# bxh1/VIDO-SLAM

Hardware: AMD Instinct MI355X
Metric: frames/sec end-to-end (flow+depth+track+local-BA) at 640x480; BA iters/sec (higher is better)
Workload: dtype f32

## Files before the change

include/vido_c.h:

```cpp
#ifndef VIDO_C_H
#define VIDO_C_H
#include <stdint.h>
#include <stddef.h>
#ifdef __cplusplus
extern "C" {
#endif

#define VIDO_OK              0
#define VIDO_E_INVALID      -1
#define VIDO_E_NO_DEVICE    -2
#define VIDO_E_HIP          -3
#define VIDO_E_CAPACITY     -4
#define VIDO_E_NOMEM        -5

#define VIDO_MAX_LEVELS 16

typedef struct vido_ctx vido_ctx;

typedef struct vido_keypoint { float x, y, size, angle, response; int32_t octave; } vido_keypoint;

typedef struct vido_config {
    int32_t device;
    int32_t width, height;
    int32_t max_batch;
// ... 44 lines not shown
} vido_track_params;

typedef struct vido_frame_lists {
    int32_t max_stat, max_obj;
    int32_t* n_stat; int32_t* stat_idx; float* stat_corr; float* stat_flow; float* stat_depth;
    int32_t* n_obj; float* obj_keys; float* obj_corr; float* obj_depth; int32_t* obj_label; float* obj_flow;
} vido_frame_lists;

int vido_track_slots(vido_ctx* ctx);
int vido_debug_first_op(vido_ctx* ctx, int rounds);
int vido_frame_upload(vido_ctx* ctx, int slot0, int n_frames, float* depth, const float* flow, const int32_t* mask,
                      int on_device, const vido_track_params* p);
int vido_frame_features(vido_ctx* ctx, int slot0, int n_frames, const vido_keypoint* kps, const int32_t* n_kps, int max_kp,
                        const vido_track_params* p, vido_frame_lists* out);
typedef struct vido_frontend_view {
    int32_t n_frames, kp_pitch, stat_pitch, obj_pitch;
    const vido_keypoint* kps; const uint8_t* desc; const int32_t* frame_beg;
    const int32_t* n_stat; const int32_t* stat_idx; const float* stat_corr; const float* stat_flow; const float* stat_depth;
    const int32_t* n_obj; const float* obj_keys; const float* obj_corr; const float* obj_depth; const int32_t* obj_label; const float* obj_flow;
} vido_frontend_view;
int vido_frontend_batch(vido_ctx* ctx, const uint8_t* imgs, int imgs_on_device, int n_frames, size_t frame_stride, int stride, int width, int height,
                        float* depth, const float* flow, const int32_t* mask, int maps_on_device, int slot0, const vido_track_params* p,
                        vido_frontend_view* view);
int vido_gather_static_depth(vido_ctx* ctx, int slot, const float* keys_xy, int n, float* depth_out);
int vido_gather_object_depth_label(vido_ctx* ctx, int slot, const float* keys_xy, int n, float th_depth_obj,
                                   float* depth_out, int32_t* label_out);
int vido_update_mask(vido_ctx* ctx, int slot_last, int slot_cur, const int32_t* last_label, const float* last_corr_xy, int n,
                     int32_t* recovered_out, int cap, int32_t* n_recovered);
int vido_read_maps(vido_ctx* ctx, int slot, float* depth_out, float* flow_out, int32_t* mask_out);
int vido_mask_propagate(vido_ctx* ctx, const int32_t* mask_prev, const float* flow, const float* depth_prev , int H, int W, int32_t* out,
                        int32_t* stats_out );
int vido_frame_propagate_mask(vido_ctx* ctx, int slot_last, int slot_cur, int32_t* stats_out );
int vido_mask_associate(vido_ctx* ctx, const int32_t* prev , const int32_t* cur, int H, int W, const int64_t* classes , int n, int hold,
                        int32_t* state , int32_t* out, int32_t* lut_out , int32_t* stats_out );
int vido_mask_components(vido_ctx* ctx, const int32_t* mask, int H, int W, int connectivity, int min_area, int id_base, int cap, int32_t* out,
                         int64_t* classes_out , int32_t* area_out , int32_t* stats_out );
int vido_frame_split_mask(vido_ctx* ctx, int slot, int connectivity, int min_area, int id_base, int cap, int32_t* stats_out );
int vido_gather_point_samples(vido_ctx* ctx, int slot, const float* xy, int n, int32_t* mask_out, float* depth_out, float* flow_out);
int vido_unproject_world(vido_ctx* ctx, const float* keys_xy, const float* z, int n, const vido_track_params* p,
                         const float* Tcw, float* xyz_out);
int vido_scene_flow(vido_ctx* ctx, const float* xyz_last, const float* xyz_cur, const int32_t* sem_last, const int32_t* sem_cur,
                    int n, float* flow3d_out, int32_t* obj_label_inout);

typedef struct vido_pose_problem {
    int32_t mode, n;
    const double* Xw;
    const double* obs;
    const double* flow0;
    const double* depth;
    double Twl[16];
    double P[12];
    double fx, fy, cx, cy;
    double T_init[16];
    double info_edge, info_prior, huber_delta;
    int32_t use_huber, rounds, drop_kernel_after_round;
    int32_t iters[4];
    float chi2_th[4];
} vido_pose_problem;

typedef struct vido_pose_result { double T[16]; int32_t n_inliers, lm_iterations; double chi2_final; } vido_pose_result;

int vido_pose_optimize(vido_ctx* ctx, const vido_pose_problem* prob, vido_pose_result* result, uint8_t* outlier_out, double* flow_out);
int vido_pose_optimize_batch(vido_ctx* ctx, const vido_pose_problem* probs, int n_prob, vido_pose_result* results,
                             uint8_t* const* outlier_out, double* const* flow_out);

typedef struct vido_ba_problem {
    int32_t n_cam, n_pt, n_obs, n_odo, prior_cam, use_huber, max_iters, pad;
    double* cam_T; double* pt_xyz;
    const int32_t* obs_cam; const int32_t* obs_pt; const double* obs_meas;
    const int32_t* odo_i; const int32_t* odo_j; const double* odo_T;
    double prior_T[12];
    double info_obs, info_odo, info_prior, huber_obs, huber_odo, gain_threshold;
    int32_t pt_lo, pt_hi;
    int32_t rank, world;
} vido_ba_problem;

typedef struct vido_ba_result { int32_t iterations, lm_trials; double chi2_initial, chi2_final, lambda_final;
                                double ms_setup;
                                double ms_solve_loop;
                                double ms_linearize_kernel;
                                double ms_schur_kernel;
} vido_ba_result;

typedef int (*vido_allreduce_fn)(void* user, void* dev_ptr, size_t count, int op);

int vido_ba_optimize(vido_ctx* ctx, vido_ba_problem* prob, vido_ba_result* result, vido_allreduce_fn allreduce, void* user);
int vido_rccl_unique_id(uint8_t id_out[128]);
int vido_rccl_init(vido_ctx* ctx, const uint8_t id[128], int rank, int world);
int vido_rccl_allreduce(void* user_ctx, void* dev_ptr, size_t count, int op);
int vido_rccl_destroy(vido_ctx* ctx);

typedef struct vido_ba_dynamic {
    int32_t n_H, n_dyn, n_tern, n_smooth;
    double* H_T;
    double* dyn_xyz;
    const int32_t* dyn_cam; const double* dyn_meas;
    const int32_t* tern_prev; const int32_t* tern_cur; const int32_t* tern_H;
    const int32_t* sm_i; const int32_t* sm_j;
    double info_dyn, info_tern, info_smooth, huber_dyn, huber_tern, huber_smooth;
} vido_ba_dynamic;
int vido_ba_optimize_dynamic(vido_ctx* ctx, vido_ba_problem* prob, vido_ba_dynamic* dyn, vido_ba_result* result,
                             vido_allreduce_fn allreduce, void* user);

int vido_correlation(vido_ctx* ctx, const float* first, const float* second, int B, int C, int H, int W, int stride,
                     float* out, int on_device);
int vido_det_order(vido_ctx* ctx, const float* scores, const long long* labels, const int* n_det, float confidence, int cap, long long* order, long long* labels_out, long long* n_live);
int vido_det_order_n(vido_ctx* ctx, const float* scores, const long long* labels, const int* n_det, float confidence, int cap, long long* order, long long* labels_out, long long* n_live,
                     int32_t* n_live32);
int vido_roi_levels(vido_ctx* ctx, const float* boxes, int n, float k_min, float k_max, int* out);
int vido_mask_logit_select(vido_ctx* ctx, const float* feat, const float* w, const float* b, const long long* labels, float* out, int n, int c, int hw, int classes);
int vido_mask_logit_select_n(vido_ctx* ctx, const float* feat, const float* w, const float* b, const long long* labels, float* out, int n, int c, int hw, int classes, const int32_t* n_live);
int vido_bias_act(vido_ctx* ctx, float* x, const float* bias, int N, int C, int H, int W, float slope);
int vido_bias_unary(vido_ctx* ctx, float* x, const float* bias, int N, int C, int H, int W, int kind);
int vido_upcat_reflect(vido_ctx* ctx, const float* x, const float* skip, int C1, int C2, int h, int w, float* out);
int vido_minmax_norm_u16(vido_ctx* ctx, const float* d, const float* mm, int64_t n, int32_t* out);
int vido_bias_res_act(vido_ctx* ctx, float* x, const float* bias, const float* res, int N, int C, int H, int W, float slope);
int vido_area_feed(vido_ctx* ctx, const uint8_t* bgr, int H, int W, float* out, int OH, int OW, float div);
int vido_backwarp(vido_ctx* ctx, const float* x, const float* flow, int B, int C, int H, int W, float* out);
int vido_deconv4s2_depthwise(vido_ctx* ctx, const float* x, const float* weight, int B, int C, int H, int W, float input_slope, float* out);

int vido_conv1x1_supported(int cin, int cout, int hw);
int vido_conv1x1_layout(int cin, int cout, int hw);
int vido_conv1x1_set_arith(int arith);
int vido_conv1x1_range_flag(vido_ctx* ctx, int reset);
int vido_range_latch(vido_ctx* ctx, unsigned* dst);
int vido_conv1x1_bias_act(vido_ctx* ctx, const float* x, const float* w_packed, const float* bias, const float* residual, float* y, int cin, int cout, int hw, float slope);
int vido_deconv2x2_supported(int n, int cin, int cout, int h, int w);
int vido_deconv2x2_bias_act(vido_ctx* ctx, const float* x, const float* w_packed, const float* bias, float* y, int n, int cin, int cout, int h, int w, float slope);
int vido_deconv2x2_bias_act_n(vido_ctx* ctx, const float* x, const float* w_packed, const float* bias, float* y, int n, int cin, int cout, int h, int w, float slope, const int32_t* n_live);
int vido_conv1x1_bias_up2_act(vido_ctx* ctx, const float* x, const float* w_packed, const float* bias, const float* residual_half, float* y, int cin, int cout, int h, int w, float slope);

int vido_conv_kxk_c2(vido_ctx* ctx, const float* x, const float* w, const float* bias, const float* residual, float* y, int cin, int k, int h, int w_);
int vido_conv1x1_skinny(vido_ctx* ctx, const float* x, const float* w_packed, const float* bias, const float* residual, float* y, int cin, int cout, long long hw, float slope);
int vido_stem7x7s2_pool(vido_ctx* ctx, const float* x, const float* w_packed, const float* bias, float* y, int h, int w);

int vido_conv_direct_supported(int cin, int cout, int h, int w, int kh, int kw, int sh, int sw, int ph, int pw);
long long vido_conv_direct_packed_floats(int cin, int cout, int kh, int kw);
int vido_conv_direct_pack(const float* w, int cin, int cout, int kh, int kw, float* w_packed);
int vido_conv_direct_bias_act(vido_ctx* ctx, const float* x, const float* w_packed, const float* bias, float* y, int n, int cin, int cout, int h, int w,
                              int kh, int kw, int sh, int sw, int ph, int pw, float slope);

int vido_wino3x3_supported(int cin, int cout, int h, int w);
int vido_wino3x3_fills_chip(int n, int cout, int h, int w, int min_wgs);
long long vido_wino3x3_packed_floats(int cin, int cout);
int vido_wino3x3_pack(const float* w, int cin, int cout, float* u_packed);
int vido_wino3x3_bias_act(vido_ctx* ctx, const float* x, const float* u_packed, const float* bias, float* y, int n, int cin, int cout, int h, int w, float slope);
int vido_wino3x3_form(int n, int cin, int cout, int h, int w);
int vido_fc_h_splitk(int rows, int k, int outs);
int vido_fc_h(vido_ctx* ctx, const float* x, const void* w_packed, const float* bias, float* part, float* y, int rows, int k, int outs, float slope);
int vido_conv3x3_h_supported(int n, int cin, int cout, int h, int w);
int vido_conv3x3_h_workgroups(int n, int cout, int h, int w);
int vido_conv3x3_h_bias_act(vido_ctx* ctx, const float* x, const void* w_packed, const float* bias, float* y, int n, int cin, int cout, int h, int w, float slope);
int vido_conv3x3_h_bias_act_n(vido_ctx* ctx, const float* x, const void* w_packed, const float* bias, float* y, int n, int cin, int cout, int h, int w, float slope, const int32_t* n_live);
long long vido_wino3x3_packed_floats_form(int cin, int cout, int form);
int vido_wino3x3_pack_form(const float* w, int cin, int cout, int form, float* u_packed);
int vido_wino3x3_bias_act_form(vido_ctx* ctx, const float* x, const float* u_packed, const float* bias, float* y, int n, int cin, int cout, int h, int w, float slope, int form);
int vido_gconv3x3_supported(int H, int W, int cpg_in, int cpg_out);
int64_t vido_gconv3x3_packed_size(int groups, int cpg_in, int cpg_out);
int vido_gconv3x3_bias_act(vido_ctx* ctx, const float* x, const float* in_bias, const float* w_packed, const float* bias, float* y, int groups, int cpg_in, int cpg_out, int H, int W, float slope);
int vido_gconv3x3_s2_supported(int H, int W, int cpg_in, int cpg_out);
int vido_gconv3x3_s2_bias_act(vido_ctx* ctx, const float* x, const float* w_packed, const float* bias, float* y, int groups, int cpg_in, int cpg_out, int H, int W, float slope);
int vido_lfn_reg_front(vido_ctx* ctx, const float* im1, const float* im2, const float* flow, const float* mean, float scale, int B, int C, int H, int W, float* out, int out_channels);
int vido_lfn_reg_tail(vido_ctx* ctx, const float* dist, const float* flow, const float* wx, const float* bx, const float* wy, const float* by, int B, int K, int H, int W, float* out);
int vido_roi_align(vido_ctx* ctx, const float* feat, int B, int C, int H, int W, const float* rois, int n_rois,
                   float spatial_scale, int pooled_h, int pooled_w, int sampling_ratio, float* out, int on_device);
int vido_nms(vido_ctx* ctx, const float* boxes_xyxy, const float* scores, int n, float thresh, int32_t* keep_out,
             int32_t* n_keep, int on_device);
int vido_nms_grouped(vido_ctx* ctx, const float* boxes_xyxy, const float* scores, const int32_t* groups, int n, float thresh,
                     int32_t* keep_out, int32_t* n_keep, int on_device);
int vido_nms_segments(vido_ctx* ctx, const float* boxes_xyxy, const int32_t* groups, const int32_t* seg_off, const int32_t* seg_n, int n_seg, int max_n, int total,
                      float thresh, int32_t* keep_out, int32_t* n_keep);
int vido_roi_align_fpn(vido_ctx* ctx, const float* const feat[4], const int H[4], const int W[4], const float scale[4], int C, const float* boxes, const int32_t* level,
                       int n, int pooled_h, int pooled_w, int sampling_ratio, float* out);
int vido_nchw_to_nhwc(vido_ctx* ctx, const float* src, int B, int C, int H, int W, float* dst);
int vido_roi_align_fpn_nhwc(vido_ctx* ctx, const float* const feat[4], const int H[4], const int W[4], const float scale[4], int C, const float* boxes, const int32_t* level,
                            int n, int pooled_h, int pooled_w, int sampling_ratio, float* out);
int vido_roi_align_fpn_nhwc_n(vido_ctx* ctx, const float* const feat[4], const int H[4], const int W[4], const float scale[4], int C, const float* boxes, const int32_t* level,
                              int n, int pooled_h, int pooled_w, int sampling_ratio, float* out, const int32_t* n_live);
int vido_bawin_create(vido_ctx* ctx, int cap_frames, int cap_features);
int vido_bawin_push_frame(vido_ctx* ctx, int frame, int n, const double* meas, const float* xyz, const int32_t* asso);
int vido_bawin_set_labels(vido_ctx* ctx, int n, const int32_t* quads);
int vido_bawin_solve(vido_ctx* ctx, int start, int N, vido_ba_problem* prob, vido_ba_result* res, int32_t* n_obs_out, int32_t* n_pt_out);
int vido_bawin_read_points(vido_ctx* ctx, int frame, int n, float* xyz_out);
int vido_rpn_select(vido_ctx* ctx, int n_levels, const float* const* logits, const float* const* deltas, const int* h, const int* w, const int* stride, const float* cell_anchors,
                    int A, int K, int img_w, int img_h, float* boxes_out, float* scores_out, int32_t* n_out);
int vido_rpn_merge(vido_ctx* ctx, const float* boxes, const float* scores, const int32_t* keep, const int32_t* cnt, int n_levels, int K, int post_nms_top_n, int n_final,
                   float* out_boxes, float* out_scores, int32_t* n_valid);
int vido_det_class_sort(vido_ctx* ctx, const float* prob, const float* deltas, const float* proposals, const float* objectness, int N, int nc, float thresh, const float weights[4],
                        int img_w, int img_h, float* seg_boxes, int32_t* order, int32_t* seg_n);
int vido_det_select(vido_ctx* ctx, const float* prob, const float* seg_boxes, const int32_t* order, const int32_t* keep, const int32_t* cnt, int N, int nc, int detections_per_img, int cap,
                    int32_t* scratch, float* out_boxes, float* out_scores, int64_t* out_labels, int32_t* n_det);
int vido_mask_label_image(vido_ctx* ctx, const float* masks, const float* boxes, const int64_t* labels, int n, int M, int padding, float thresh, int H, int W, uint8_t* out);
int vido_mask_instance_image(vido_ctx* ctx, const float* masks, const float* boxes, const int64_t* labels, int n, int M, int padding, float thresh, int H, int W,
                             const int32_t* id_base_dev, uint8_t* out, int32_t* area_out);
int vido_box_decode(vido_ctx* ctx, const float* deltas, const float* boxes, int n, int k, const float weights[4],
                    float* out, int on_device);

int vido_pnp_ransac(vido_ctx* ctx, const float* pts3d, const float* pts2d, int n, double fx, double fy, double cx, double cy,
                    int max_iters, double reproj_err, double confidence, uint64_t seed, double T_out[16], uint8_t* inlier_mask,
                    int32_t* n_inliers);

int vido_pnp_ransac_batch(vido_ctx* ctx, int n_prob, const float* const* pts3d, const float* const* pts2d, const int32_t* n, double fx, double fy, double cx, double cy,
                          int max_iters, double reproj_err, double confidence, const uint64_t* seeds, double* T_out, uint8_t* const* inlier_mask, int32_t* n_inliers);

typedef struct vido_host_maps { const int32_t* mask; const float* depth; const float* flow; int32_t width, height; } vido_host_maps;
float vido_depth_noise(float z, unsigned seed);
int vido_undistort_points(const float* xy, int n, const float K[4], const float dist[5], float* xy_out);
int vido_renew_static(const vido_host_maps* maps, const float* stat_xy, int n_stat, const int32_t* TM_sta, int n_tm, const float* sample_xy, int n_sample,
                      int max_num, int32_t* src_out, int32_t* inlier_out, float* flow_out, int cap, int32_t* n_out);
int vido_renew_objects(const vido_host_maps* maps, const float* obj_xy, const int32_t* obj_label, int n_obj_pts,
                       int n_objects, const int32_t* inl_off, const int32_t* inl_ids, const uint8_t* obj_stat, const int32_t* sem_position, const int32_t* mod_label,
                       const float* tmp_xy, const float* tmp_depth, const int32_t* tmp_sem, const float* tmp_flow, const float* tmp_corr, int n_tmp, int max_num_obj,
                       float* keys_out, float* depth_out, int32_t* sem_out, float* flow_out, float* corr_out, int32_t* inlier_out, int32_t* label_out, int cap, int32_t* n_out);
typedef struct vido_point_samples { const int32_t* mask; const float* depth; const float* flow; } vido_point_samples;
int vido_renew_static_sampled(int width, int height, const float* stat_xy, int n_stat, const vido_point_samples* stat_samples, const int32_t* TM_sta, int n_tm,
                              const float* sample_xy, int n_sample, const vido_point_samples* sample_samples, int max_num,
                              int32_t* src_out, int32_t* inlier_out, float* flow_out, int cap, int32_t* n_out);
int vido_renew_objects_sampled(int width, int height, const float* obj_xy, const int32_t* obj_label, int n_obj_pts, const vido_point_samples* obj_samples,
                               int n_objects, const int32_t* inl_off, const int32_t* inl_ids, const uint8_t* obj_stat, const int32_t* sem_position, const int32_t* mod_label,
                               const float* tmp_xy, const float* tmp_depth, const int32_t* tmp_sem, const float* tmp_flow, const float* tmp_corr, int n_tmp, int max_num_obj,
                               float* keys_out, float* depth_out, int32_t* sem_out, float* flow_out, float* corr_out, int32_t* inlier_out, int32_t* label_out, int cap, int32_t* n_out);
int vido_dyn_obj_tracking(const int32_t* sem_label, int32_t* obj_label, const float* obj_xy, const float* obj_depth, const float* flow3d, const int32_t* last_sem_label, int n,
                          const int32_t* last_sem_position, const uint8_t* last_obj_stat, const int32_t* last_mod_label, int n_last, int rows, int cols,
                          float sf_mg_thres, float sf_ds_thres, float th_depth_obj, int f_id, int32_t* max_id,
                          int32_t* obj_off, int32_t* obj_ids, int32_t* mod_label_out, int32_t* sem_position_out, int max_objects, int32_t* n_objects);

int vido_tracklets_incremental(int n_rows, const int32_t* row_off, const int32_t* row_n, const int32_t* TM, const int32_t* labels, int n_feat0,
                               int32_t* trk_off, int32_t* pairs, int32_t* obj_id, int32_t* owner_trk, int32_t* owner_pos, int cap_trk, int cap_pairs, int32_t* n_trk);

typedef struct vido_system vido_system;
typedef struct vido_system_stats {
    int32_t frame_id, n_keypoints, n_static, n_static_inliers, n_objects, n_object_points, ba_window;
    int32_t mask_propagated;
    float ms_total;
    float ms_update_mask, ms_frame;
    float ms_cam_pose, ms_obj_tracking, ms_obj_motion, ms_renew;
    float ms_local_ba;
    float ms_wait_inputs;
    float ms_orb, ms_lists;
} vido_system_stats;
int         vido_system_create(const char* settings_yaml, vido_system** out);
void        vido_system_destroy(vido_system* sys);
const char* vido_system_last_error(const vido_system* sys);
int         vido_system_track_rgbd(vido_system* sys, const uint8_t* im, int channels, int width, int height, float* depth, const float* flow,
                                   const int32_t* mask, double timestamp, int n_image, float Tcw_out[16]);
int         vido_system_set_zero_copy_maps(vido_system* sys, int zero_copy);
int         vido_system_prefetch_image_device(vido_system* sys, const void* im_dev, int channels, int width, int height, void* image_ready_event);
int         vido_system_track_rgbd_device(vido_system* sys, const void* im_dev, int channels, int width, int height, float* depth_dev, const float* flow_dev,
                                          const int32_t* mask_dev, void* ready_event, double timestamp, int n_image, float Tcw_out[16]);
int         vido_system_get_stats(const vido_system* sys, vido_system_stats* out);
int         vido_system_get_verify_stats(const vido_system* sys, int* n_checked, int* n_rejected);
int         vido_system_mask_split_stats(const vido_system* sys, int32_t out[4]);
int         vido_system_get_verify_points(const vido_system* sys, float* xy, float* prev_xy, int32_t* xyl, int32_t* dist, uint8_t* rejected, uint8_t* seed_desc, int cap, int* n_out);
int         vido_system_save_results(vido_system* sys, const char* prefix);
vido_ctx*   vido_system_context(vido_system* sys);
int         vido_system_set_depth_noise_seed(vido_system* sys, unsigned seed);

#ifdef __cplusplus
}
#endif
#endif
```

vido-slam_amd/csrc/conv3x3h.hip:

```cpp
#include "common.hpp"
#include <type_traits>

namespace {
typedef float f32x16 __attribute__((ext_vector_type(16)));
typedef float f32x2 __attribute__((ext_vector_type(2)));
typedef _Float16 f16x8 __attribute__((ext_vector_type(8)));
typedef _Float16 f16x2 __attribute__((ext_vector_type(2)));
typedef unsigned u32x4 __attribute__((ext_vector_type(4)));

#define C3_OOB 0x40000000u
#define C3_WSLOT 24576
#define C3_RBW 3
#define C3_WPIX(BR) (((BR) + 2) * 18)
#define C3_XP(BR) ((16 * C3_WPIX(BR) + 511) / 512)
#define C3_RAW(BR) (C3_XP(BR) * 8 * 256)
#define C3_PLANE(BR) (C3_WPIX(BR) * 32)
#define C3_PBUF(BR) (2 * C3_PLANE(BR))
#define C3_LDS(BR) (C3_RBW * C3_WSLOT + C3_RAW(BR) + 2 * C3_PBUF(BR))

struct C3Args { const float* x; const void* wp; const float* bias; float* y; int N, Cin, Cout, H, W, nby, nbx, mt, total, nchunk; float slope; unsigned wbytes; unsigned* range_flag; const int* n_live; };

template <int RPW, int CG>
__global__ __launch_bounds__(512) void k_conv3x3_h(C3Args A)
{
    constexpr int BR = 16 / CG, MT = 32 * RPW * CG, WPIX = C3_WPIX(BR), XP = C3_XP(BR), RAWB = C3_RAW(BR), PLANE = C3_PLANE(BR), PBUF = C3_PBUF(BR), CK = (WPIX * 8 + 511) / 512, NMM = 9 * RPW, NRD = 2 * RPW + 2;
    extern __shared__ __attribute__((aligned(16))) char c3_lds[];
    char* L = c3_lds;
    const int tid = threadIdx.x, lane = tid & 63, w = __builtin_amdgcn_readfirstlane(tid >> 6);
    int total = A.total, per = gridDim.x >> 3;
    if (A.n_live) { const int nl = min(max(*A.n_live, 0), A.N); total = nl * A.nby * A.nbx * A.mt; per = (total + 7) >> 3; }
    const int q8 = blockIdx.x >> 3, item = (blockIdx.x & 7) * per + q8;
    if (q8 >= per || item >= total) return;
    const int nt = item / A.mt, mtile = item - nt * A.mt, m0 = mtile * MT;
    const int bpi = A.nby * A.nbx, n = nt / bpi, brem = nt - n * bpi, by = brem / A.nbx, bx = brem - by * A.nbx, Y0 = by * BR, X0 = bx * 16;
    const int rp = CG == 1 ? w : (w & 3), rb0 = CG == 1 ? 0 : RPW * (w >> 2);
    const int hw = A.H * A.W, nsteps = A.nchunk * 3;

    const __amdgpu_buffer_rsrc_t wr = __builtin_amdgcn_make_buffer_rsrc((void*)A.wp, 0, A.wbytes, 0x00020000);
    const unsigned avo = 16u * (unsigned)lane;
    unsigned abase[3], avq[3];
#pragma unroll
    for (int q = 0; q < 3; q++) { const int i = w + 8 * q, rb = i / 6, rem = i - 6 * rb; abase[q] = 1024u * (unsigned)(((m0 >> 5) + rb) * A.nchunk * 18 + rem); avq[q] = rb < RPW * CG ? avo : 0x80000000u; }
    unsigned xvo[11];
#pragma unroll
    for (int j = 0; j < XP; j++) {
        const int e = 64 * (8 * j + w) + lane, ch = e / WPIX, rem = e - ch * WPIX, row = rem / 18, col = rem - row * 18, gy = Y0 - 1 + row, gx = X0 - 1 + col;
        xvo[j] = (e < 16 * WPIX && gy >= 0 && gy < A.H && gx >= 0 && gx < A.W) ? 4u * (unsigned)(ch * hw + gy * A.W + gx) : C3_OOB;
    }
    const unsigned ximg = 4u * (unsigned)n * (unsigned)A.Cin * (unsigned)hw, ximg_end = ximg + 4u * (unsigned)A.Cin * (unsigned)hw, xchunk = 64u * (unsigned)hw;
    char* const RAW = L + C3_RBW * C3_WSLOT;
    char* const PL = RAW + RAWB;
    auto issue_w = [&](int s, int slot) {
        char* S = L + slot * C3_WSLOT + w * 1024;
        const unsigned so = 6144u * (unsigned)s;
#pragma unroll
        for (int q = 0; q < 3; q++) __builtin_amdgcn_raw_ptr_buffer_load_lds(wr, (__attribute__((address_space(3))) void*)(S + q * 8192), 16, avq[q], abase[q] + so, 0, 0);
    };
    auto issue_x = [&](int c) {
        const unsigned so = ximg + xchunk * (unsigned)c;
        const __amdgpu_buffer_rsrc_t xc = __builtin_amdgcn_make_buffer_rsrc((void*)((const char*)A.x + so), 0, ximg_end - so, 0x00020000);
#pragma unroll
        for (int j = 0; j < XP; j++) __builtin_amdgcn_raw_ptr_buffer_load_lds(xc, (__attribute__((address_space(3))) void*)(RAW + (8 * j + w) * 256), 4, xvo[j], 0, 0, 0);
    };
    float xmax = 0.f;
    const f32x2 k2048 = {2048.f, 2048.f};
    auto convert = [&](int buf) {
        const float* R = (const float*)RAW;
        unsigned* P = (unsigned*)(PL + buf * PBUF);
#pragma unroll
        for (int k = 0; k < CK; k++) {
            const int idx = tid + 512 * k;
            if (k < CK - 1 || idx < WPIX * 8) {
                const int q = idx / WPIX, pix = idx - q * WPIX;
                const f32x2 v = {R[(2 * q) * WPIX + pix], R[(2 * q + 1) * WPIX + pix]};
                const f16x2 h = __builtin_convertvector(v, f16x2);
                f32x2 vs, r;
                asm("v_pk_mul_f32 %0, %1, %2" : "=v"(vs) : "v"(v), "v"(k2048));
                asm("v_fma_mix_f32 %0, %1, %2, %3 op_sel_hi:[1,0,0]" : "=v"(r.x) : "v"(h), "s"(-2048.f), "v"(vs.x));
                asm("v_fma_mix_f32 %0, %1, %2, %3 op_sel:[1,0,0] op_sel_hi:[1,0,0]" : "=v"(r.y) : "v"(h), "s"(-2048.f), "v"(vs.y));
                const f16x2 l = __builtin_convertvector(r, f16x2);
                P[pix * 8 + q] = __builtin_bit_cast(unsigned, h); P[PLANE / 4 + pix * 8 + q] = __builtin_bit_cast(unsigned, l);
                xmax = __builtin_elementwise_maximum(__builtin_elementwise_maximum(xmax, __builtin_fabsf(v.x)), __builtin_fabsf(v.y));
            }
        }
    };

    f32x16 acc[RPW], acl[RPW];
#pragma unroll
    for (int rb = 0; rb < RPW; rb++)
#pragma unroll
        for (int r = 0; r < 16; r++) { acc[rb][r] = 0.f; acl[rb][r] = 0.f; }
    typedef const __attribute__((address_space(3))) char* lds_c;
    const unsigned a_lane = 16u * (unsigned)lane;
    const unsigned b_lane = (unsigned)(C3_RBW * C3_WSLOT + RAWB) + 32u * (unsigned)((2 * rp + ((lane & 31) >> 4)) * 18 + (lane & 15)) + 16u * (unsigned)(lane >> 5);

    issue_x(0); issue_w(0, 0); issue_w(min(1, nsteps - 1), 1);
    asm volatile("s_waitcnt vmcnt(6) lgkmcnt(0)\n\ts_barrier" ::: "memory");
    convert(0);
    int slot = 0;
    u32x4 a[2][RPW][2], b[2][2];
    auto step = [&](auto dy_c, auto nbuf_c, int pbuf, auto&& copies) {
        constexpr int dy = decltype(dy_c)::value, NBUF = decltype(nbuf_c)::value;
        lds_c Ab = (lds_c)(L + slot * C3_WSLOT) + a_lane;
        lds_c Bb = (lds_c)L + b_lane + pbuf * PBUF + dy * (18 * 32);
        auto ld = [&](int dx, int set) {
#pragma unroll
            for (int rb = 0; rb < RPW; rb++)
#pragma unroll
                for (int pl = 0; pl < 2; pl++) a[set][rb][pl] = *(const __attribute__((address_space(3))) u32x4*)(Ab + (((rb0 + rb) * 3 + dx) * 2 + pl) * 1024);
#pragma unroll
            for (int pl = 0; pl < 2; pl++) b[set][pl] = *(const __attribute__((address_space(3))) u32x4*)(Bb + dx * 32 + pl * PLANE);
        };
        __builtin_amdgcn_sched_barrier(0);
        ld(0, 0);
        copies();
#pragma unroll
        for (int dx = 0; dx < 3; dx++) {
            if (dx < 2) ld(dx + 1, (dx + 1) & 1);
#pragma unroll
            for (int term = 0; term < 3; term++) {
                constexpr int PA[3] = {0, 1, 0}, PB[3] = {1, 0, 0};
#pragma unroll
                for (int rb = 0; rb < RPW; rb++) {
                    f32x16& d = term == 2 ? acc[rb] : acl[rb];
                    d = __builtin_amdgcn_mfma_f32_32x32x16_f16(__builtin_bit_cast(f16x8, a[dx & 1][rb][PA[term]]), __builtin_bit_cast(f16x8, b[dx & 1][PB[term]]), d, 0, 0, 0);
                }
            }
        }
        __builtin_amdgcn_sched_group_barrier(0x100, NRD, 0);
#pragma unroll
        for (int i = 0; i < NMM; i++) {
            __builtin_amdgcn_sched_group_barrier(0x008, 1, 0);
            if (i < 2 * NRD) __builtin_amdgcn_sched_group_barrier(0x100, 1, 0);
            if (i >= 1 && i < 1 + NBUF) __builtin_amdgcn_sched_group_barrier(0x020, 1, 0);
        }
        __builtin_amdgcn_sched_barrier(0);
    };
    for (int c = 0; c < A.nchunk; c++) {
        const int pbuf = c & 1, cn = min(c + 1, A.nchunk - 1);
        asm volatile("s_waitcnt vmcnt(3) lgkmcnt(0)\n\ts_barrier" ::: "memory");
        step(std::integral_constant<int, 0>{}, std::integral_constant<int, 3 + XP>{}, pbuf, [&] { const int sf = slot == 0 ? C3_RBW - 1 : slot - 1; issue_w(min(3 * c + 2, nsteps - 1), sf); issue_x(cn); });
        slot = slot + 1 == C3_RBW ? 0 : slot + 1;
        asm volatile("s_waitcnt vmcnt(%0) lgkmcnt(0)\n\ts_barrier" :: "n"(3 + XP) : "memory");
        step(std::integral_constant<int, 1>{}, std::integral_constant<int, 3>{}, pbuf, [&] { const int sf = slot == 0 ? C3_RBW - 1 : slot - 1; issue_w(min(3 * c + 3, nsteps - 1), sf); });
        slot = slot + 1 == C3_RBW ? 0 : slot + 1;
        asm volatile("s_waitcnt vmcnt(3) lgkmcnt(0)\n\ts_barrier" ::: "memory");
        step(std::integral_constant<int, 2>{}, std::integral_constant<int, 3>{}, pbuf, [&] { const int sf = slot == 0 ? C3_RBW - 1 : slot - 1; issue_w(min(3 * c + 4, nsteps - 1), sf); });
        convert(pbuf ^ 1);
        slot = slot + 1 == C3_RBW ? 0 : slot + 1;
    }
    asm volatile("s_waitcnt vmcnt(0) lgkmcnt(0)" ::: "memory");
#pragma unroll
    for (int rb = 0; rb < RPW; rb++) acc[rb] += acl[rb] * 0x1p-11f;
    if (!(xmax < 65504.f) && A.range_flag) atomicOr(A.range_flag, 1u);

    const float* wsc = (const float*)((const char*)A.wp + (size_t)A.nchunk * 16 * 18 * A.Cout * 2);
    const int p = lane & 31, Y = Y0 + 2 * rp + (p >> 4), X = X0 + (p & 15);
    const bool inside = Y < A.H && X < A.W;
    float* yb = A.y + (size_t)n * A.Cout * hw + (size_t)Y * A.W + X;
#pragma unroll
    for (int rb = 0; rb < RPW; rb++) {
        float bv[16], sv[16];
#pragma unroll
        for (int r = 0; r < 16; r++) { const int co = m0 + 32 * (rb0 + rb) + 8 * (r >> 2) + 4 * (lane >> 5) + (r & 3); bv[r] = A.bias ? A.bias[co] : 0.f; sv[r] = wsc[co]; }
        if (inside) {
#pragma unroll
            for (int r = 0; r < 16; r++) {
                const int co = m0 + 32 * (rb0 + rb) + 8 * (r >> 2) + 4 * (lane >> 5) + (r & 3);
                const float v = acc[rb][r] * sv[r] + bv[r];
                yb[(size_t)co * hw] = fmaxf(v, v * A.slope);
            }
        }
    }
}
}

extern "C" {

int vido_conv3x3_h_supported(int n, int cin, int cout, int h, int w)
{
    const long long cp = (cin + 15) / 16 * 16;
    return n >= 1 && cin >= 1 && (cout == 32 || cout == 64 || (cout >= 128 && cout % 128 == 0)) && h >= 1 && w >= 1 && 4ll * n * cin * h * w < (1ll << 30) && 4ll * n * cout * h * w < (1ll << 30)
           && 36ll * cp * cout < (1ll << 31);
}

#define C3_MIN16 190
static int c3_block_rows(int n, int cout, int h, int w)
{
    static const int force = [] { const char* e = getenv("VIDO_CONV3X3_H_ROWS"); return e ? atoi(e) : 0; }();
    if (cout == 32) return 16;
    if (force == 16 || force == 8) return force;
    const int mt = cout >= 128 ? cout / 128 : 1;
    return n * ((h + 15) / 16) * ((w + 15) / 16) * mt >= C3_MIN16 ? 16 : 8;
}
int vido_conv3x3_h_workgroups(int n, int cout, int h, int w) { const int br = c3_block_rows(n, cout, h, w); return n * ((h + br - 1) / br) * ((w + 15) / 16) * (cout >= 128 ? cout / 128 : 1); }

int vido_conv3x3_h_bias_act(vido_ctx* ctx, const float* x, const void* w_packed, const float* bias, float* y, int n, int cin, int cout, int h, int w, float slope)
{
    return vido_conv3x3_h_bias_act_n(ctx, x, w_packed, bias, y, n, cin, cout, h, w, slope, nullptr);
}

int vido_conv3x3_h_bias_act_n(vido_ctx* ctx, const float* x, const void* w_packed, const float* bias, float* y, int n, int cin, int cout, int h, int w, float slope, const int32_t* n_live)
{
    if (!ctx) return VIDO_E_INVALID;
    if (!x || !w_packed || !y || x == y || !vido_conv3x3_h_supported(n, cin, cout, h, w) || slope < 0.f || slope > 1.f || (((uintptr_t)x | (uintptr_t)y | (uintptr_t)n_live) & 3) || ((uintptr_t)w_packed & 15))
        return vido_set_error(ctx, VIDO_E_INVALID, "conv3x3_h: no kernel for %d x %d -> %d channels at %d x %d (or a pointer is misaligned, or slope outside [0, 1])", n, cin, cout, h, w);
    HIP_TRY(ctx, hipSetDevice(ctx->device));
    hipStream_t st = ctx->has_ext_stream ? ctx->ext_stream : ctx->stream;
    const int br = c3_block_rows(n, cout, h, w);
    const int nby = (h + br - 1) / br, nbx = (w + 15) / 16, mt = cout >= 128 ? cout / 128 : 1, total = n * nby * nbx * mt;
    const int nchunk = (cin + 15) / 16;
    C3Args A{x, w_packed, bias, y, n, cin, cout, h, w, nby, nbx, mt, total, nchunk, slope, (unsigned)(36ll * 16 * nchunk * cout), ctx->c1_range_flag, n_live};
    static bool attr[64] = {};
    if (!attr[ctx->device & 63]) {
#define C3_ATTR(RPW_, CG_) HIP_TRY(ctx, hipFuncSetAttribute((const void*)k_conv3x3_h<RPW_, CG_>, hipFuncAttributeMaxDynamicSharedMemorySize, (int)C3_LDS(16 / CG_)))
        C3_ATTR(4, 1); C3_ATTR(2, 2); C3_ATTR(2, 1); C3_ATTR(1, 2); C3_ATTR(1, 1);
#undef C3_ATTR
        attr[ctx->device & 63] = true;
    }
    const dim3 grid(8 * ((total + 7) / 8));
#define C3_LAUNCH(RPW_, CG_) hipLaunchKernelGGL((k_conv3x3_h<RPW_, CG_>), grid, dim3(512), C3_LDS(16 / CG_), st, A)
    if (cout >= 128) { if (br == 16) C3_LAUNCH(4, 1); else C3_LAUNCH(2, 2); }
    else if (cout == 64) { if (br == 16) C3_LAUNCH(2, 1); else C3_LAUNCH(1, 2); }
    else C3_LAUNCH(1, 1);
#undef C3_LAUNCH
    HIP_TRY(ctx, hipGetLastError());
    return VIDO_OK;
}

}
```

vido-slam_amd/csrc/nets.hip:

```cpp
#include "common.hpp"
#include <numeric>

#define CORR_CH 8
__global__ __launch_bounds__(256) void k_correlation(const float* __restrict__ f1, const float* __restrict__ f2, int C, int H, int W, int s,
                                                     int Ho, int Wo, float* __restrict__ out, int nsplit, int cper)
{
    __shared__ float t2[CORR_CH][22][23];
    const int tx = threadIdx.x & 15, ty = threadIdx.x >> 4, b = blockIdx.z / nsplit, split = blockIdx.z - b * nsplit;
    const int c_lo = split * cper, c_hi = min(C, c_lo + cper);
    const int x = blockIdx.x * 16 + tx, y = blockIdx.y * 16 + ty;
    const bool valid = x < Wo && y < Ho;
    float acc[49];
#pragma unroll
    for (int k = 0; k < 49; k++) acc[k] = 0.f;
    const size_t plane = (size_t)H * W;
    for (int c0 = c_lo; c0 < c_hi; c0 += CORR_CH) {
        const int nc = min(CORR_CH, c_hi - c0);
        for (int i = threadIdx.x; i < nc * 22 * 22; i += 256) {
            const int cc = i / (22 * 22), r = (i / 22) % 22, q = i % 22;
            const int yy = (blockIdx.y * 16 + r - 3), xx = (blockIdx.x * 16 + q - 3);
            float v = 0.f;
            if (yy >= 0 && yy < Ho && xx >= 0 && xx < Wo) v = f2[((size_t)b * C + c0 + cc) * plane + (size_t)(yy * s) * W + xx * s];
            t2[cc][r][q] = v;
        }
        float a[CORR_CH];
#pragma unroll
        for (int cc = 0; cc < CORR_CH; cc++) a[cc] = (valid && cc < nc) ? f1[((size_t)b * C + c0 + cc) * plane + (size_t)(y * s) * W + x * s] : 0.f;
        __syncthreads();
#pragma unroll
        for (int cc = 0; cc < CORR_CH; cc++) {
            if (cc < nc) {
#pragma unroll
                for (int p = 0; p < 7; p++)
#pragma unroll
                    for (int o = 0; o < 7; o++) acc[p * 7 + o] += a[cc] * t2[cc][ty + p][tx + o];
            }
        }
        __syncthreads();
    }
    if (valid) {
        float* o = out + (size_t)split * (gridDim.z / nsplit) * 49 * Ho * Wo;
#pragma unroll
        for (int k = 0; k < 49; k++) o[(((size_t)b * 49 + k) * Ho + y) * Wo + x] = nsplit == 1 ? acc[k] / (float)C : acc[k];
    }
}
__global__ __launch_bounds__(256) void k_correlation_reduce(const float* __restrict__ part, int nsplit, size_t n, float inv_c_dummy, int C, float* __restrict__ out)
{
    const size_t i = blockIdx.x * (size_t)blockDim.x + threadIdx.x;
    if (i >= n) return;
    float sum = 0.f;
    for (int k = 0; k < nsplit; k++) sum += part[(size_t)k * n + i];
    out[i] = sum / (float)C;
}

__global__ __launch_bounds__(1024) void k_det_order(const float* __restrict__ scores, const long long* __restrict__ labels, const int* __restrict__ n_det, float confidence, int cap,
                                                   long long* __restrict__ order, long long* __restrict__ labels_out, long long* __restrict__ n_live, int* __restrict__ n_live32)
{
    __shared__ float key[1024];
    __shared__ int cnt;
    const int i = threadIdx.x;
    if (i == 0) cnt = 0;
    const int nd = *n_det;
    bool live = false;
    if (i < cap) { live = scores[i] > confidence && i < nd; key[i] = live ? scores[i] : -1.0f; }
    __syncthreads();
    if (i < cap) {
        const float k = key[i]; int rank = 0;
        for (int j = 0; j < cap; j++) { const float kj = key[j]; rank += (kj > k) || (kj == k && j < i); }
        order[rank] = i; labels_out[rank] = live ? labels[i] : 0;
        if (live) atomicAdd(&cnt, 1);
    }
    __syncthreads();
    if (i == 0) { *n_live = cnt; if (n_live32) *n_live32 = cnt; }
}

__global__ void k_roi_levels(const float* __restrict__ boxes, int n, float k_min, float k_max, int* __restrict__ out)
{
    const int i = blockIdx.x * blockDim.x + threadIdx.x;
    if (i >= n) return;
    const float x1 = boxes[4 * i], y1 = boxes[4 * i + 1], x2 = boxes[4 * i + 2], y2 = boxes[4 * i + 3];
    const float area = __fmul_rn(__fadd_rn(__fsub_rn(x2, x1), 1.f), __fadd_rn(__fsub_rn(y2, y1), 1.f));
    const float t = __fadd_rn(__fdiv_rn(__fsqrt_rn(area), 224.f), 1e-6f);
    float l = floorf(__fadd_rn(4.f, log2f(t)));
    l = fminf(fmaxf(l, k_min), k_max);
    out[i] = (int)l - (int)k_min;
}

__global__ __launch_bounds__(256) void k_mask_logit_select(const float* __restrict__ feat, const float* __restrict__ w, const float* __restrict__ b, const long long* __restrict__ labels,
                                                           float* __restrict__ out, int c, int hw, int classes, const int* __restrict__ n_live)
{
    __shared__ float wl[1024];
    const int n = blockIdx.y, p = blockIdx.x * 256 + threadIdx.x;
    if (n_live && n >= *n_live) {
        if (p < hw) out[(size_t)n * hw + p] = 0.f;
        return;
    }
    long long lab = labels[n]; lab = lab < 0 ? 0 : (lab >= classes ? classes - 1 : lab);
    for (int i = threadIdx.x; i < c; i += 256) wl[i] = w[(size_t)lab * c + i];
    __syncthreads();
    if (p >= hw) return;
    const float* f = feat + (size_t)n * c * hw + p;
    double a0 = 0, a1 = 0, a2 = 0, a3 = 0;
    int i = 0;
    for (; i + 4 <= c; i += 4) { a0 += (double)wl[i] * f[(size_t)i * hw]; a1 += (double)wl[i + 1] * f[(size_t)(i + 1) * hw]; a2 += (double)wl[i + 2] * f[(size_t)(i + 2) * hw]; a3 += (double)wl[i + 3] * f[(size_t)(i + 3) * hw]; }
    for (; i < c; i++) a0 += (double)wl[i] * f[(size_t)i * hw];
    const float v = (float)((a0 + a1) + (a2 + a3) + (b ? (double)b[lab] : 0.0));
    out[(size_t)n * hw + p] = 1.f / (1.f + expf(-v));
}

__global__ __launch_bounds__(256) void k_bias_act(float* __restrict__ x, const float* __restrict__ bias, int C, size_t hw, size_t total, float slope)
{
    const size_t i = (blockIdx.x * (size_t)blockDim.x + threadIdx.x) * 4;
    if (i >= total) return;
    if ((hw & 3) == 0) {
        const float b = bias[(i / hw) % C];
        float4 v = *(float4*)(x + i);
        v.x += b; v.y += b; v.z += b; v.w += b;
        v.x = v.x > 0.f ? v.x : v.x * slope; v.y = v.y > 0.f ? v.y : v.y * slope; v.z = v.z > 0.f ? v.z : v.z * slope; v.w = v.w > 0.f ? v.w : v.w * slope;
        *(float4*)(x + i) = v;
    } else {
        for (size_t k = i; k < min(i + 4, total); k++) { float v = x[k] + bias[(k / hw) % C]; x[k] = v > 0.f ? v : v * slope; }
    }
}

template <int KIND>
__global__ __launch_bounds__(256) void k_bias_unary(float* __restrict__ x, const float* __restrict__ bias, int C, size_t hw, size_t total)
{
    const size_t i = blockIdx.x * (size_t)blockDim.x + threadIdx.x;
    if (i >= total) return;
    const float v = x[i] + bias[(i / hw) % C];
    x[i] = KIND == 1 ? (v > 0.f ? v : expf(v) - 1.f) : 1.f / (1.f + expf(-v));
}

__global__ __launch_bounds__(256) void k_upcat_reflect(const float* __restrict__ x, const float* __restrict__ skip, int C1, int C2, int h, int w, float* __restrict__ out)
{
    const int H2 = 2 * h, W2 = 2 * w, OW = W2 + 2, OH = H2 + 2;
    const size_t i = blockIdx.x * (size_t)blockDim.x + threadIdx.x, total = (size_t)(C1 + C2) * OH * OW;
    if (i >= total) return;
    const int X = (int)(i % OW), Y = (int)((i / OW) % OH), c = (int)(i / ((size_t)OW * OH));
    int yy = Y - 1, xx = X - 1;
    yy = yy < 0 ? -yy : (yy >= H2 ? 2 * H2 - 2 - yy : yy); xx = xx < 0 ? -xx : (xx >= W2 ? 2 * W2 - 2 - xx : xx);
    out[i] = c < C1 ? x[((size_t)c * h + (yy >> 1)) * w + (xx >> 1)] : skip[((size_t)(c - C1) * H2 + yy) * W2 + xx];
}

__global__ __launch_bounds__(256) void k_minmax_norm_u16(const float* __restrict__ d, const float* __restrict__ mm, size_t n, int* __restrict__ out)
{
    const size_t i = blockIdx.x * (size_t)blockDim.x + threadIdx.x;
    if (i >= n) return;
    const float lo = mm[0], hi = mm[1];
    float v = (d[i] - lo) / (hi - lo + 1e-12f) * 65536.0f;
    v = fminf(fmaxf(v, 0.f), 65535.f);
    out[i] = (int)v;
}

__global__ __launch_bounds__(256) void k_bias_res_act(float* __restrict__ x, const float* __restrict__ bias, const float* __restrict__ res, int C, size_t hw, size_t total, float slope)
{
    const size_t i = (blockIdx.x * (size_t)blockDim.x + threadIdx.x) * 4;
    if (i >= total) return;
    if ((hw & 3) == 0) {
        const float b = bias[(i / hw) % C];
        float4 v = *(float4*)(x + i); const float4 r = *(const float4*)(res + i);
        v.x += b + r.x; v.y += b + r.y; v.z += b + r.z; v.w += b + r.w;
        v.x = v.x > 0.f ? v.x : v.x * slope; v.y = v.y > 0.f ? v.y : v.y * slope; v.z = v.z > 0.f ? v.z : v.z * slope; v.w = v.w > 0.f ? v.w : v.w * slope;
        *(float4*)(x + i) = v;
    } else {
        for (size_t k = i; k < min(i + 4, total); k++) { float v = x[k] + bias[(k / hw) % C] + res[k]; x[k] = v > 0.f ? v : v * slope; }
    }
}

struct RoiLevels { const float* feat[4]; int H[4], W[4]; float scale[4]; };
template <int SR >
__global__ __launch_bounds__(256) void k_roi_align_nhwc(RoiLevels L, int C, const float* __restrict__ rois, int roi_stride ,
                                                        const int* __restrict__ level , int PH, int PW, int sampling, float* __restrict__ out, const int* __restrict__ n_live )
{
    extern __shared__ __attribute__((aligned(16))) float rl_tile[];
    if (n_live && (int)blockIdx.x >= *n_live) return;
    const int i = blockIdx.x, c0 = blockIdx.y * 64, lane = threadIdx.x & 63, wave = threadIdx.x >> 6;
    const int nbin = PH * PW, pitch = nbin | 1;
    const float* r = rois + (size_t)roi_stride * i;
    const int l = level ? level[i] : 0, bi = roi_stride == 5 ? (int)r[0] : 0;
    const float* box = r + (roi_stride == 5 ? 1 : 0);
    const float scale = L.scale[l]; const int H = L.H[l], W = L.W[l];
    const float sw = box[0] * scale, sh = box[1] * scale, ew = box[2] * scale, eh = box[3] * scale;
    const float rw = fmaxf(ew - sw, 1.f), rh = fmaxf(eh - sh, 1.f);
    const float bh = rh / (float)PH, bw = rw / (float)PW;
    const int gh = SR > 0 ? SR : (sampling > 0 ? sampling : (int)ceilf(rh / PH)), gw = SR > 0 ? SR : (sampling > 0 ? sampling : (int)ceilf(rw / PW));
    const float count = (float)(gh * gw);
    const int c = min(c0 + lane, C - 1);
    const float* d = L.feat[l] + (size_t)bi * H * W * C + c;
    auto taps = [&](float y, float x, int& o1, int& o2, int& o3, int& o4, float& w1, float& w2, float& w3, float& w4) {
        const bool out = y < -1.0 || y > H || x < -1.0 || x > W;
        if (y <= 0) y = 0;
        if (x <= 0) x = 0;
        int yl = out ? 0 : (int)y, xl = out ? 0 : (int)x, yh, xh;
        if (yl >= H - 1) { yh = yl = H - 1; y = (float)yl; } else yh = yl + 1;
        if (xl >= W - 1) { xh = xl = W - 1; x = (float)xl; } else xh = xl + 1;
        const float ly = y - yl, lx = x - xl, hy = 1.f - ly, hx = 1.f - lx;
        o1 = yl * W + xl; o2 = yl * W + xh; o3 = yh * W + xl; o4 = yh * W + xh;
        w1 = hy * hx; w2 = hy * lx; w3 = ly * hx; w4 = ly * lx;
        return out;
    };
    for (int bin = wave; bin < nbin; bin += 4) {
        const int ph = bin / PW, pw = bin - ph * PW;
        float acc = 0.f;
        if (SR == 2) {
            int o[4][4]; float w[4][4], v[4][4]; bool out[4];
#pragma unroll
            for (int s2 = 0; s2 < 4; s2++) {
                const int iy = s2 >> 1, ix = s2 & 1;
                const float y = sh + ph * bh + (float)(iy + .5f) * bh / (float)gh, x = sw + pw * bw + (float)(ix + .5f) * bw / (float)gw;
                out[s2] = taps(y, x, o[s2][0], o[s2][1], o[s2][2], o[s2][3], w[s2][0], w[s2][1], w[s2][2], w[s2][3]);
            }
#pragma unroll
            for (int s2 = 0; s2 < 4; s2++)
#pragma unroll
                for (int t = 0; t < 4; t++) v[s2][t] = d[(size_t)o[s2][t] * C];
#pragma unroll
            for (int s2 = 0; s2 < 4; s2++) acc += out[s2] ? 0.f : (w[s2][0] * v[s2][0] + w[s2][1] * v[s2][1] + w[s2][2] * v[s2][2] + w[s2][3] * v[s2][3]);
        } else {
            for (int iy = 0; iy < gh; iy++) {
                const float y = sh + ph * bh + (float)(iy + .5f) * bh / (float)gh;
                for (int ix = 0; ix < gw; ix++) {
                    const float x = sw + pw * bw + (float)(ix + .5f) * bw / (float)gw;
                    int o1, o2, o3, o4; float w1, w2, w3, w4;
                    if (taps(y, x, o1, o2, o3, o4, w1, w2, w3, w4)) { acc += 0.f; continue; }
                    const float v1 = d[(size_t)o1 * C], v2 = d[(size_t)o2 * C], v3 = d[(size_t)o3 * C], v4 = d[(size_t)o4 * C];
                    acc += (w1 * v1 + w2 * v2 + w3 * v3 + w4 * v4);
                }
            }
        }
        rl_tile[lane * pitch + bin] = acc / count;
    }
    __syncthreads();
    const int nc = min(64, C - c0), total = nc * nbin;
    float* o = out + ((size_t)i * C + c0) * nbin;
    for (int e = threadIdx.x; e < total; e += 256) { const int cc = e / nbin; o[e] = rl_tile[cc * pitch + (e - cc * nbin)]; }
}
__global__ __launch_bounds__(256) void k_nchw_to_nhwc(const float* __restrict__ src, int C, int HW, float* __restrict__ dst)
{
    __shared__ float t[64][65];
    const int p0 = blockIdx.x * 64, c0 = blockIdx.y * 64, b = blockIdx.z, lane = threadIdx.x & 63, q = threadIdx.x >> 6;
    const float* s = src + (size_t)b * C * HW; float* d = dst + (size_t)b * HW * C;
    for (int k = q; k < 64; k += 4) if (c0 + k < C && p0 + lane < HW) t[k][lane] = s[(size_t)(c0 + k) * HW + p0 + lane];
    __syncthreads();
    for (int k = q; k < 64; k += 4) if (p0 + k < HW && c0 + lane < C) d[(size_t)(p0 + k) * C + c0 + lane] = t[lane][k];
}

__device__ __forceinline__ void tile_of(int t, int nb, int& rb, int& cb)
{
    int r = (int)((2.0f * nb + 1.0f - sqrtf((2.0f * nb + 1.0f) * (2.0f * nb + 1.0f) - 8.0f * (float)t)) * 0.5f);
    r = max(0, min(r, nb - 1));
    while (r > 0 && r * nb - r * (r - 1) / 2 > t) r--;
    while ((r + 1) * nb - (r + 1) * r / 2 <= t) r++;
    rb = r; cb = r + (t - (r * nb - r * (r - 1) / 2));
}
__device__ __forceinline__ void nms_tile(const float* __restrict__ boxes, const int* __restrict__ group, int n, float thresh, unsigned long long* __restrict__ mask, int col_blocks, int rb, int cb, int lane)
{
    const int col = cb * 64 + lane; const bool cv = col < n;
    const float4 b = cv ? *(const float4*)(boxes + 4 * (size_t)col) : make_float4(0.f, 0.f, 0.f, 0.f);
    const float Sb = (b.z - b.x + 1) * (b.w - b.y + 1);
    const int gb = (group && cv) ? group[col] : 0;
    const int rows = min(n - rb * 64, 64);
    unsigned long long mine = 0;
    for (int i = 0; i < rows; i++) {
        const float* a = boxes + 4 * (size_t)(rb * 64 + i);
        const float a0 = a[0], a1 = a[1], a2 = a[2], a3 = a[3];
        const int ga = group ? group[rb * 64 + i] : 0;
        const float left = fmaxf(a0, b.x), right = fminf(a2, b.z), top = fmaxf(a1, b.y), bottom = fminf(a3, b.w);
        const float w = fmaxf(right - left + 1, 0.f), h = fmaxf(bottom - top + 1, 0.f), inter = w * h;
        const float Sa = (a2 - a0 + 1) * (a3 - a1 + 1);
        const bool hit = cv && ga == gb && inter / (Sa + Sb - inter) > thresh;
        unsigned long long word = __ballot(hit);
        if (rb == cb) word &= i >= 63 ? 0ull : ~((2ull << i) - 1ull);
        if (lane == i) mine = word;
    }
    if (lane < rows) mask[(size_t)(rb * 64 + lane) * col_blocks + cb] = mine;
}
__global__ __launch_bounds__(256) void k_nms_mask(const float* __restrict__ boxes, const int* __restrict__ group , int n, float thresh,
                                                 unsigned long long* __restrict__ mask, int col_blocks)
{
    const int t = __builtin_amdgcn_readfirstlane(blockIdx.x * 4 + (threadIdx.x >> 6)), nb = col_blocks;
    if (t >= nb * (nb + 1) / 2) return;
    int rb, cb; tile_of(t, nb, rb, cb);
    nms_tile(boxes, group, n, thresh, mask, col_blocks, rb, cb, threadIdx.x & 63);
}
__global__ __launch_bounds__(64) void k_nms_sweep(const unsigned long long* __restrict__ mask, int n, int col_blocks, int* __restrict__ keep, int* __restrict__ n_keep)
{
    const int lane = threadIdx.x;
    int cnt = 0;
    unsigned long long remv[16];
    const int wpl = (col_blocks + 63) / 64;
    for (int k = 0; k < 16; k++) remv[k] = 0;
    for (int i = 0; i < n; i++) {
        const int nblock = i >> 6, inblock = i & 63;
        const int owner = nblock & 63, slot = nblock >> 6;
        unsigned long long word = 0;
#pragma unroll
        for (int k = 0; k < 16; k++) if (k == slot) word = remv[k];
        word = __shfl(word, owner, 64);
        if (!(word & (1ULL << inblock))) {
            if (lane == 0) keep[cnt] = i;
            cnt++;
            const unsigned long long* p = mask + (size_t)i * col_blocks;
#pragma unroll
            for (int k = 0; k < 16; k++) if (k < wpl) { const int w = k * 64 + lane; if (w >= nblock && w < col_blocks) remv[k] |= p[w]; }
        }
    }
    if (lane == 0) *n_keep = cnt;
}

__global__ __launch_bounds__(64) void k_nms_sweep_seg(const unsigned long long* __restrict__ mask, const int* __restrict__ seg_off, const int* __restrict__ seg_n, int col_blocks,
                                                      int* __restrict__ keep, int* __restrict__ n_keep, int keep_stride)
{
    const int g = blockIdx.x, lane = threadIdx.x;
    const int n = seg_n[g];
    const unsigned long long* M = mask + (size_t)seg_off[g] * col_blocks;
    int* kp = keep + (size_t)g * keep_stride;
    const int cb = (n + 63) >> 6;
    unsigned long long remv[16];
#pragma unroll
    for (int k = 0; k < 16; k++) remv[k] = 0;
    int cnt = 0;
    for (int blk = 0; blk < cb; blk++) {
        const int owner = blk & 63, slot = blk >> 6, rows = min(n - blk * 64, 64);
        unsigned long long word = 0;
#pragma unroll
        for (int k = 0; k < 16; k++) if (k == slot) word = remv[k];
        word = __shfl(word, owner, 64);
        const unsigned long long diag = lane < rows ? M[(size_t)(blk * 64 + lane) * col_blocks + blk] : 0ull;
        const uint32_t dlo = (uint32_t)diag, dhi = (uint32_t)(diag >> 32);
        unsigned long long alive = ~word;
        if (rows < 64) alive &= (1ull << rows) - 1ull;
        unsigned long long keepmask = 0;
        while (alive) {
            const int j = __builtin_ctzll(alive);
            keepmask |= 1ull << j;
            const unsigned long long dj = (unsigned long long)(uint32_t)__builtin_amdgcn_readlane((int)dlo, j) | ((unsigned long long)(uint32_t)__builtin_amdgcn_readlane((int)dhi, j) << 32);
            alive &= ~dj; alive &= ~(1ull << j);
        }
        if ((keepmask >> lane) & 1ull) kp[cnt + __popcll(keepmask & ((1ull << lane) - 1ull))] = blk * 64 + lane;
        cnt += __popcll(keepmask);
        const bool mine = (keepmask >> lane) & 1ull;
        const unsigned long long* prow = M + (size_t)(blk * 64 + lane) * col_blocks;
        for (int w0 = blk + 1; w0 < cb; w0 += 4) {
            unsigned long long v[4];
#pragma unroll
            for (int u = 0; u < 4; u++) v[u] = (mine && w0 + u < cb) ? prow[w0 + u] : 0ull;
#pragma unroll
            for (int u = 0; u < 4; u++) {
                uint32_t lo = (uint32_t)v[u], hi = (uint32_t)(v[u] >> 32);
#pragma unroll
                for (int o = 32; o >= 1; o >>= 1) { lo |= (uint32_t)__shfl_xor((int)lo, o, 64); hi |= (uint32_t)__shfl_xor((int)hi, o, 64); }
                const int w = w0 + u;
                if (w < cb && lane == (w & 63)) {
                    const unsigned long long r = (unsigned long long)lo | ((unsigned long long)hi << 32);
#pragma unroll
                    for (int k = 0; k < 16; k++) if (k == (w >> 6)) remv[k] |= r;
                }
            }
        }
    }
    for (int i = cnt + lane; i < keep_stride; i += 64) kp[i] = -1;
    if (lane == 0) n_keep[g] = cnt;
}
__global__ __launch_bounds__(256) void k_nms_mask_seg(const float* __restrict__ boxes, const int* __restrict__ group, const int* __restrict__ seg_off, const int* __restrict__ seg_n,
                                                     float thresh, unsigned long long* __restrict__ mask, int col_blocks)
{
    const int g = blockIdx.y, n = seg_n[g], off = seg_off[g];
    const int nb = (n + 63) >> 6, t = __builtin_amdgcn_readfirstlane(blockIdx.x * 4 + (threadIdx.x >> 6));
    if (t >= nb * (nb + 1) / 2) return;
    int rb, cb; tile_of(t, nb, rb, cb);
    nms_tile(boxes + 4 * (size_t)off, group ? group + off : nullptr, n, thresh, mask + (size_t)off * col_blocks, col_blocks, rb, cb, threadIdx.x & 63);
}

struct PasteDet { int x0, y0, w, h, label; float rw, rh; };
__global__ __launch_bounds__(256) void k_paste_prepare(const float* __restrict__ boxes, const int64_t* __restrict__ labels, int n, int M, int padding, PasteDet* __restrict__ det)
{
    const int i = blockIdx.x * blockDim.x + threadIdx.x;
    if (i >= n) return;
    const float scale = (float)((double)(M + 2 * padding) / (double)M);
    const float* b = boxes + 4 * (size_t)i;
    const float wh = (b[2] - b[0]) * 0.5f * scale, hh = (b[3] - b[1]) * 0.5f * scale;
    const float xc = (b[2] + b[0]) * 0.5f, yc = (b[3] + b[1]) * 0.5f;
    const int x0 = (int)(xc - wh), y0 = (int)(yc - hh), x1 = (int)(xc + wh), y1 = (int)(yc + hh);
    PasteDet d; d.x0 = x0; d.y0 = y0; d.w = max(x1 - x0 + 1, 1); d.h = max(y1 - y0 + 1, 1); d.label = (int)labels[i];
    const int Mp = M + 2 * padding;
    d.rw = (float)Mp / (float)d.w; d.rh = (float)Mp / (float)d.h;
    det[i] = d;
}
__global__ __launch_bounds__(256) void k_paste_label(const float* __restrict__ masks , const PasteDet* __restrict__ det, int n, int M, int padding, float thresh,
                                                     int H, int W, uint8_t* __restrict__ out)
{
    __shared__ PasteDet sd[128];
    const int x = blockIdx.x * 32 + (threadIdx.x & 31), y = blockIdx.y * 8 + (threadIdx.x >> 5);
    const int Mp = M + 2 * padding;
    unsigned acc = 0;
    for (int d0 = 0; d0 < n; d0 += 128) {
        __syncthreads();
        if ((int)threadIdx.x < min(128, n - d0)) sd[threadIdx.x] = det[d0 + threadIdx.x];
        __syncthreads();
        if (x < W && y < H) {
            for (int k = 0; k < min(128, n - d0); k++) {
                const PasteDet d = sd[k];
                const int u = x - d.x0, v = y - d.y0;
                if (u < 0 || v < 0 || u >= d.w || v >= d.h) continue;
                float sy = d.rh * ((float)v + 0.5f) - 0.5f; if (sy < 0.f) sy = 0.f;
                float sx = d.rw * ((float)u + 0.5f) - 0.5f; if (sx < 0.f) sx = 0.f;
                const int iy = (int)sy, ix = (int)sx; const int iyp = iy < Mp - 1 ? 1 : 0, ixp = ix < Mp - 1 ? 1 : 0;
                const float ly = sy - (float)iy, lx = sx - (float)ix, hy = 1.f - ly, hx = 1.f - lx;
                const float* m = masks + (size_t)(d0 + k) * M * M;
                auto at = [&](int yy, int xx) -> float { yy -= padding; xx -= padding; return (yy < 0 || xx < 0 || yy >= M || xx >= M) ? 0.f : m[yy * M + xx]; };
                const float val = hy * (hx * at(iy, ix) + lx * at(iy, ix + ixp)) + ly * (hx * at(iy + iyp, ix) + lx * at(iy + iyp, ix + ixp));
                if (val > thresh) acc += (unsigned)d.label;
            }
        }
    }
    if (x < W && y < H) out[(size_t)y * W + x] = (uint8_t)acc;
}

__global__ void k_zero_i32(int32_t* __restrict__ p, int n)
{
    const int i = blockIdx.x * blockDim.x + threadIdx.x;
    if (i < n) p[i] = 0;
}
__global__ __launch_bounds__(256) void k_paste_instance(const float* __restrict__ masks , const PasteDet* __restrict__ det, int n, int M, int padding, float thresh,
                                                        int H, int W, const int32_t* __restrict__ id_base, uint8_t* __restrict__ out, int32_t* __restrict__ area)
{
    __shared__ PasteDet sd[128];
    __shared__ unsigned char slot[128];
    __shared__ int cnt[256], nlive[2];
    const int t = threadIdx.x, bx0 = blockIdx.x * 32, by0 = blockIdx.y * 8;
    const int x = bx0 + (t & 31), y = by0 + (t >> 5);
    const int Mp = M + 2 * padding;
    const bool inside = x < W && y < H;
    if (area) cnt[t] = 0;
    int hit = -1;
    for (int d0 = 0; d0 < n; d0 += 128) {
        PasteDet mine; bool live = false; int pos = 0;
        if (t < 128) {
            if (t < n - d0) {
                mine = det[d0 + t];
                const int u_lo = (int)((unsigned)bx0 - (unsigned)mine.x0), u_hi = (int)((unsigned)(bx0 + 31) - (unsigned)mine.x0);
                const int v_lo = (int)((unsigned)by0 - (unsigned)mine.y0), v_hi = (int)((unsigned)(by0 + 7) - (unsigned)mine.y0);
                live = mine.label != 0 && (u_lo > u_hi || (u_hi >= 0 && u_lo < mine.w)) && (v_lo > v_hi || (v_hi >= 0 && v_lo < mine.h));
            }
            const unsigned long long b = __ballot(live);
            pos = __popcll(b & ((1ull << (t & 63)) - 1ull));
            if ((t & 63) == 0) nlive[t >> 6] = __popcll(b);
        }
        __syncthreads();
        if (live) { const int p = pos + (t >= 64 ? nlive[0] : 0); sd[p] = mine; slot[p] = (unsigned char)t; }
        __syncthreads();
        const int m = nlive[0] + nlive[1];
        if (inside && hit < 0) {
            for (int k = 0; k < m; k++) {
                const PasteDet d = sd[k];
                const int u = x - d.x0, v = y - d.y0;
                if (u < 0 || v < 0 || u >= d.w || v >= d.h) continue;
                float sy = d.rh * ((float)v + 0.5f) - 0.5f; if (sy < 0.f) sy = 0.f;
                float sx = d.rw * ((float)u + 0.5f) - 0.5f; if (sx < 0.f) sx = 0.f;
                const int iy = (int)sy, ix = (int)sx; const int iyp = iy < Mp - 1 ? 1 : 0, ixp = ix < Mp - 1 ? 1 : 0;
                const float ly = sy - (float)iy, lx = sx - (float)ix, hy = 1.f - ly, hx = 1.f - lx;
                const float* m_ = masks + (size_t)(d0 + slot[k]) * M * M;
                auto at = [&](int yy, int xx) -> float { yy -= padding; xx -= padding; return (yy < 0 || xx < 0 || yy >= M || xx >= M) ? 0.f : m_[yy * M + xx]; };
                const float val = hy * (hx * at(iy, ix) + lx * at(iy, ix + ixp)) + ly * (hx * at(iy + iyp, ix) + lx * at(iy + iyp, ix + ixp));
                if (val > thresh) { hit = d0 + slot[k]; break; }
            }
        }
        __syncthreads();
    }
    if (inside) out[(size_t)y * W + x] = hit < 0 ? (uint8_t)0 : (uint8_t)((id_base ? *id_base : 0) + 1 + hit);
    if (area) {
        if (hit >= 0) atomicAdd(&cnt[hit], 1);
        __syncthreads();
        if (t < n && cnt[t]) atomicAdd(&area[t], cnt[t]);
    }
}

__global__ void k_box_decode(const float* __restrict__ deltas, const float* __restrict__ boxes, int n, int k, float wx, float wy, float ww, float wh, float* __restrict__ out)
{
    const int t = blockIdx.x * blockDim.x + threadIdx.x;
    if (t >= n * k) return;
    const int i = t / k;
    const float clip = (float)log(1000. / 16);
    const float* b = boxes + 4 * (size_t)i; const float* d = deltas + 4 * (size_t)t; float* o = out + 4 * (size_t)t;
    const float w = b[2] - b[0] + 1, h = b[3] - b[1] + 1, cx = b[0] + 0.5f * w, cy = b[1] + 0.5f * h;
    float dx = d[0] / wx, dy = d[1] / wy, dw = d[2] / ww, dh = d[3] / wh;
    if (dw > clip) dw = clip;
    if (dh > clip) dh = clip;
    const float pcx = dx * w + cx, pcy = dy * h + cy, pw = expf(dw) * w, phh = expf(dh) * h;
    o[0] = pcx - 0.5f * pw; o[1] = pcy - 0.5f * phh; o[2] = pcx + 0.5f * pw - 1; o[3] = pcy + 0.5f * phh - 1;
}

struct NetState { char* d = nullptr; char* h = nullptr; size_t cap = 0; };
void net_state_destroy(vido_ctx* ctx)
{
    NetState* S = ctx->net; if (!S) return;
    hipFree(S->d); hipHostFree(S->h); delete S; ctx->net = nullptr;
}
static int net_scratch(vido_ctx* ctx, size_t bytes, NetState** out)
{
    if (!ctx->net) ctx->net = new NetState();
    NetState* S = ctx->net;
    if (bytes > S->cap) {
        HIP_TRY(ctx, hipStreamSynchronize(ctx->stream));
        if (S->d) { hipFree(S->d); hipHostFree(S->h); S->d = nullptr; S->h = nullptr; }
        S->cap = bytes + bytes / 4 + 4096;
        HIP_TRY(ctx, hipMalloc((void**)&S->d, S->cap)); HIP_TRY(ctx, hipHostMalloc((void**)&S->h, S->cap));
    }
    *out = S;
    return VIDO_OK;
}
static inline size_t al256(size_t x) { return (x + 255) & ~(size_t)255; }

__global__ __launch_bounds__(256) void k_area_feed(const uint8_t* __restrict__ src, int H, int W, float* __restrict__ dst, int OH, int OW, float div)
{
    const int ow = blockIdx.x * 64 + (threadIdx.x & 63), oh = blockIdx.y * 4 + (threadIdx.x >> 6);
    if (ow >= OW || oh >= OH) return;
    const int h0 = (int)floorf((float)(oh * H) / OH), h1 = (int)ceilf((float)((oh + 1) * H) / OH);
    const int w0 = (int)floorf((float)(ow * W) / OW), w1 = (int)ceilf((float)((ow + 1) * W) / OW);
    float s0 = 0.f, s1 = 0.f, s2 = 0.f;
    for (int ih = h0; ih < h1; ih++) {
        const uint8_t* row = src + ((size_t)ih * W + w0) * 3;
        for (int iw = w0; iw < w1; iw++, row += 3) { s0 += (float)row[2]; s1 += (float)row[1]; s2 += (float)row[0]; }
    }
    const float kh = (float)(h1 - h0), kw = (float)(w1 - w0);
    float o0 = s0 / kh / kw, o1 = s1 / kh / kw, o2 = s2 / kh / kw;
    if (div != 1.0f) { const float inv = 1.0f / div; o0 *= inv; o1 *= inv; o2 *= inv; }
    const size_t plane = (size_t)OH * OW, o = (size_t)oh * OW + ow;
    dst[o] = o0; dst[plane + o] = o1; dst[2 * plane + o] = o2;
}
#define BW_CG 8
__global__ __launch_bounds__(256) void k_backwarp(const float* __restrict__ x, const float* __restrict__ flow, int B, int C, int H, int W, float* __restrict__ out)
{
    const int w = blockIdx.x * 64 + (threadIdx.x & 63), h = blockIdx.y * 4 + (threadIdx.x >> 6);
    const int ncg = (C + BW_CG - 1) / BW_CG, b = blockIdx.z / ncg, c0 = (blockIdx.z - b * ncg) * BW_CG, c1 = min(C, c0 + BW_CG);
    if (w >= W || h >= H) return;
    const size_t hw = (size_t)H * W, o = (size_t)h * W + w;
    const float u = flow[(size_t)b * 2 * hw + o], v = flow[(size_t)b * 2 * hw + hw + o];
    const float stepx = ((1.0f - 1.0f / W) - (-1.0f + 1.0f / W)) / (float)(W - 1), stepy = ((1.0f - 1.0f / H) - (-1.0f + 1.0f / H)) / (float)(H - 1);
    const float gx = ((-1.0f + 1.0f / W) + stepx * (float)w) + u / (((float)W - 1.0f) / 2.0f);
    const float gy = ((-1.0f + 1.0f / H) + stepy * (float)h) + v / (((float)H - 1.0f) / 2.0f);
    const float ix = ((gx + 1.0f) * (float)W - 1.0f) / 2.0f, iy = ((gy + 1.0f) * (float)H - 1.0f) / 2.0f;
    const float fx = floorf(ix), fy = floorf(iy);
    const int x0 = (int)fx, y0 = (int)fy, x1 = x0 + 1, y1 = y0 + 1;
    const float ax = ix - fx, ay = iy - fy;
    const float wnw = (1.0f - ax) * (1.0f - ay), wne = ax * (1.0f - ay), wsw = (1.0f - ax) * ay, wse = ax * ay;
    const bool vx0 = x0 >= 0 && x0 < W, vx1 = x1 >= 0 && x1 < W, vy0 = y0 >= 0 && y0 < H, vy1 = y1 >= 0 && y1 < H;
    const float* xb = x + (size_t)b * C * hw; float* ob = out + (size_t)b * C * hw + o;
    const size_t inw = (size_t)(vy0 ? y0 : 0) * W + (vx0 ? x0 : 0), ine = (size_t)(vy0 ? y0 : 0) * W + (vx1 ? x1 : 0);
    const size_t isw = (size_t)(vy1 ? y1 : 0) * W + (vx0 ? x0 : 0), ise = (size_t)(vy1 ? y1 : 0) * W + (vx1 ? x1 : 0);
    const float mnw = (vy0 && vx0) ? wnw : 0.f, mne = (vy0 && vx1) ? wne : 0.f, msw = (vy1 && vx0) ? wsw : 0.f, mse = (vy1 && vx1) ? wse : 0.f;
#pragma unroll 4
    for (int c = c0; c < c1; c++) {
        const float* xc = xb + (size_t)c * hw;
        float acc = 0.f;
        acc += xc[inw] * mnw; acc += xc[ine] * mne; acc += xc[isw] * msw; acc += xc[ise] * mse;
        ob[(size_t)c * hw] = acc;
    }
}

__global__ __launch_bounds__(256) void k_lfn_reg_front(const float* __restrict__ im1, const float* __restrict__ im2, const float* __restrict__ flow, const float* __restrict__ mean ,
                                                       float scale, int B, int C, int H, int W, float* __restrict__ out, int out_ch)
{
    const int w = blockIdx.x * 64 + (threadIdx.x & 63), h = blockIdx.y * 4 + (threadIdx.x >> 6), b = blockIdx.z;
    if (w >= W || h >= H) return;
    const size_t hw = (size_t)H * W, o = (size_t)h * W + w;
    const float fu = flow[(size_t)b * 2 * hw + o], fv = flow[(size_t)b * 2 * hw + hw + o];
    const float u = fu * scale, v = fv * scale;
    const float stepx = ((1.0f - 1.0f / W) - (-1.0f + 1.0f / W)) / (float)(W - 1), stepy = ((1.0f - 1.0f / H) - (-1.0f + 1.0f / H)) / (float)(H - 1);
    const float gx = ((-1.0f + 1.0f / W) + stepx * (float)w) + u / (((float)W - 1.0f) / 2.0f);
    const float gy = ((-1.0f + 1.0f / H) + stepy * (float)h) + v / (((float)H - 1.0f) / 2.0f);
    const float ix = ((gx + 1.0f) * (float)W - 1.0f) / 2.0f, iy = ((gy + 1.0f) * (float)H - 1.0f) / 2.0f;
    const float fx = floorf(ix), fy = floorf(iy);
    const int x0 = (int)fx, y0 = (int)fy, x1 = x0 + 1, y1 = y0 + 1;
    const float ax = ix - fx, ay = iy - fy;
    const float wnw = (1.0f - ax) * (1.0f - ay), wne = ax * (1.0f - ay), wsw = (1.0f - ax) * ay, wse = ax * ay;
    const bool vx0 = x0 >= 0 && x0 < W, vx1 = x1 >= 0 && x1 < W, vy0 = y0 >= 0 && y0 < H, vy1 = y1 >= 0 && y1 < H;
    const size_t inw = (size_t)(vy0 ? y0 : 0) * W + (vx0 ? x0 : 0), ine = (size_t)(vy0 ? y0 : 0) * W + (vx1 ? x1 : 0);
    const size_t isw = (size_t)(vy1 ? y1 : 0) * W + (vx0 ? x0 : 0), ise = (size_t)(vy1 ? y1 : 0) * W + (vx1 ? x1 : 0);
    const float mnw = (vy0 && vx0) ? wnw : 0.f, mne = (vy0 && vx1) ? wne : 0.f, msw = (vy1 && vx0) ? wsw : 0.f, mse = (vy1 && vx1) ? wse : 0.f;
    float acc2 = 0.f;
    for (int c = 0; c < C; c++) {
        const float* xc = im2 + ((size_t)b * C + c) * hw;
        float wv = 0.f;
        wv += xc[inw] * mnw; wv += xc[ine] * mne; wv += xc[isw] * msw; wv += xc[ise] * mse;
        const float dlt = im1[((size_t)b * C + c) * hw + o] - wv;
        acc2 += dlt * dlt;
    }
    float* ob = out + (size_t)b * out_ch * hw + o;
    ob[0] = sqrtf(acc2); ob[hw] = fu - mean[2 * b]; ob[2 * hw] = fv - mean[2 * b + 1];
}
template <int K>
__global__ __launch_bounds__(256) void k_lfn_reg_tail(const float* __restrict__ dist, const float* __restrict__ flow, const float* __restrict__ wx, const float* __restrict__ bx,
                                                      const float* __restrict__ wy, const float* __restrict__ by, int B, int H, int W, float* __restrict__ out)
{
    constexpr int ND = K * K, PAD = (K - 1) / 2;
    const int w = blockIdx.x * 64 + (threadIdx.x & 63), h = blockIdx.y * 4 + (threadIdx.x >> 6), b = blockIdx.z;
    if (w >= W || h >= H) return;
    const size_t hw = (size_t)H * W, o = (size_t)h * W + w;
    const float* dp = dist + (size_t)b * ND * hw + o;
    float e[ND]; float m = -INFINITY;
#pragma unroll
    for (int c = 0; c < ND; c++) { const float v = dp[(size_t)c * hw]; e[c] = -(v * v); m = fmaxf(m, e[c]); }
    const float* fxp = flow + (size_t)b * 2 * hw; const float* fyp = fxp + hw;
    float s = 0.f, ax = 0.f, ay = 0.f;
#pragma unroll
    for (int c = 0; c < ND; c++) {
        const float p = expf(e[c] - m);
        s += p;
        const int yy = h + c / K - PAD, xx = w + c % K - PAD;
        const bool in = yy >= 0 && yy < H && xx >= 0 && xx < W;
        const size_t q = in ? (size_t)yy * W + xx : 0;
        const float ux = in ? fxp[q] : 0.f, uy = in ? fyp[q] : 0.f;
        ax += wx[c] * (p * ux); ay += wy[c] * (p * uy);
    }
    const float div = 1.0f / s;
    out[(size_t)b * 2 * hw + o] = (ax + bx[0]) * div;
    out[(size_t)b * 2 * hw + hw + o] = (ay + by[0]) * div;
}

__global__ __launch_bounds__(256) void k_deconv4s2_dw(const float* __restrict__ in, const float* __restrict__ wgt , int C, int H, int W, float slope, float* __restrict__ out)
{
    const int OW = 2 * W, OH = 2 * H;
    const int ox = blockIdx.x * 64 + (threadIdx.x & 63), oy = blockIdx.y * 4 + (threadIdx.x >> 6), bc = blockIdx.z, c = bc % C;
    if (ox >= OW || oy >= OH) return;
    const float* ip = in + (size_t)bc * H * W; const float* wp = wgt + 16 * c;
    const int ky0 = (oy + 1) & 1, kx0 = (ox + 1) & 1, iy0 = (oy + 1 - ky0) >> 1, ix0 = (ox + 1 - kx0) >> 1;
    float acc = 0.f;
#pragma unroll
    for (int a = 0; a < 2; a++) {
        const int iy = iy0 - a, ky = ky0 + 2 * a;
#pragma unroll
        for (int b = 0; b < 2; b++) {
            const int ix = ix0 - b, kx = kx0 + 2 * b;
            if (iy >= 0 && iy < H && ix >= 0 && ix < W) { float v = ip[(size_t)iy * W + ix]; v = v > 0.f ? v : v * slope; acc += v * wp[ky * 4 + kx]; }
        }
    }
    out[((size_t)bc * OH + oy) * OW + ox] = acc;
}

static int roi_lds_limit(vido_ctx* ctx, size_t lds)
{
    static size_t have = 48 * 1024;
    if (lds <= have) return VIDO_OK;
    HIP_TRY(ctx, hipFuncSetAttribute((const void*)k_roi_align_nhwc<2>, hipFuncAttributeMaxDynamicSharedMemorySize, (int)lds));
    HIP_TRY(ctx, hipFuncSetAttribute((const void*)k_roi_align_nhwc<0>, hipFuncAttributeMaxDynamicSharedMemorySize, (int)lds));
    have = lds;
    return VIDO_OK;
}

extern "C" {

int vido_correlation(vido_ctx* ctx, const float* first, const float* second, int B, int C, int H, int W, int stride, float* out, int on_device)
{
    if (!ctx) return VIDO_E_INVALID;
    if (!first || !second || !out || B < 1 || C < 1 || H < 1 || W < 1 || (stride != 1 && stride != 2)) return vido_set_error(ctx, VIDO_E_INVALID, "correlation: bad arguments");
    HIP_TRY(ctx, hipSetDevice(ctx->device));
    hipStream_t st = (on_device && ctx->has_ext_stream) ? ctx->ext_stream : ctx->stream;
    const int Ho = (H + stride - 1) / stride, Wo = (W + stride - 1) / stride;
    const size_t nin = (size_t)B * C * H * W * 4, nout = (size_t)B * 49 * Ho * Wo * 4;
    const float *d1 = first, *d2 = second; float* dout = out;
    const int tiles = ((Wo + 15) / 16) * ((Ho + 15) / 16) * B, nchunk = (C + CORR_CH - 1) / CORR_CH;
    int nsplit = std::max(1, std::min(nchunk, 512 / std::max(tiles, 1)));
    const int cper = ((nchunk + nsplit - 1) / nsplit) * CORR_CH; nsplit = (C + cper - 1) / cper;
    const size_t nel = (size_t)B * 49 * Ho * Wo, io_bytes = on_device ? 0 : 2 * al256(nin) + al256(nout), pbytes = nsplit > 1 ? al256(nel * 4 * nsplit) : 0;
    NetState* S = nullptr;
    if (io_bytes + pbytes) { int rc = net_scratch(ctx, io_bytes + pbytes, &S); if (rc) return rc; }
    if (!on_device) {
        memcpy(S->h, first, nin); memcpy(S->h + al256(nin), second, nin);
        HIP_TRY(ctx, hipMemcpyAsync(S->d, S->h, 2 * al256(nin), hipMemcpyHostToDevice, st));
        d1 = (float*)S->d; d2 = (float*)(S->d + al256(nin)); dout = (float*)(S->d + 2 * al256(nin));
    }
    if (nsplit == 1) hipLaunchKernelGGL(k_correlation, dim3((Wo + 15) / 16, (Ho + 15) / 16, B), dim3(256), 0, st, d1, d2, C, H, W, stride, Ho, Wo, dout, 1, C);
    else {
        float* part = (float*)(S->d + io_bytes);
        hipLaunchKernelGGL(k_correlation, dim3((Wo + 15) / 16, (Ho + 15) / 16, B * nsplit), dim3(256), 0, st, d1, d2, C, H, W, stride, Ho, Wo, part, nsplit, cper);
        hipLaunchKernelGGL(k_correlation_reduce, dim3((unsigned)((nel + 255) / 256)), dim3(256), 0, st, (const float*)part, nsplit, nel, 0.f, C, dout);
    }
    HIP_TRY(ctx, hipGetLastError());
    if (!on_device) {
        HIP_TRY(ctx, hipStreamSynchronize(st));
        HIP_TRY(ctx, hipMemcpyAsync(S->h, dout, nout, hipMemcpyDeviceToHost, st)); HIP_TRY(ctx, hipStreamSynchronize(st));
        memcpy(out, S->h, nout);
    }
    return VIDO_OK;
}

int vido_det_order(vido_ctx* ctx, const float* scores, const long long* labels, const int* n_det, float confidence, int cap, long long* order, long long* labels_out, long long* n_live)
{
    return vido_det_order_n(ctx, scores, labels, n_det, confidence, cap, order, labels_out, n_live, nullptr);
}
int vido_det_order_n(vido_ctx* ctx, const float* scores, const long long* labels, const int* n_det, float confidence, int cap, long long* order, long long* labels_out, long long* n_live,
                     int32_t* n_live32)
{
    if (!ctx) return VIDO_E_INVALID;
    if (!scores || !labels || !n_det || !order || !labels_out || !n_live || cap < 1 || cap > 1024) return vido_set_error(ctx, VIDO_E_INVALID, "det_order: bad arguments (cap 1 .. 1024)");
    HIP_TRY(ctx, hipSetDevice(ctx->device));
    hipStream_t st = ctx->has_ext_stream ? ctx->ext_stream : ctx->stream;
    hipLaunchKernelGGL(k_det_order, dim3(1), dim3(1024), 0, st, scores, labels, n_det, confidence, cap, order, labels_out, n_live, n_live32);
    HIP_TRY(ctx, hipGetLastError());
    return VIDO_OK;
}

int vido_roi_levels(vido_ctx* ctx, const float* boxes, int n, float k_min, float k_max, int* out)
{
    if (!ctx) return VIDO_E_INVALID;
    if (!boxes || !out || n < 0 || !(k_min <= k_max)) return vido_set_error(ctx, VIDO_E_INVALID, "roi_levels: bad arguments");
    if (n == 0) return VIDO_OK;
    HIP_TRY(ctx, hipSetDevice(ctx->device));
    hipStream_t st = ctx->has_ext_stream ? ctx->ext_stream : ctx->stream;
    hipLaunchKernelGGL(k_roi_levels, dim3((unsigned)((n + 255) / 256)), dim3(256), 0, st, boxes, n, k_min, k_max, out);
    HIP_TRY(ctx, hipGetLastError());
    return VIDO_OK;
}

int vido_mask_logit_select(vido_ctx* ctx, const float* feat, const float* w, const float* b, const long long* labels, float* out, int n, int c, int hw, int classes)
{
    return vido_mask_logit_select_n(ctx, feat, w, b, labels, out, n, c, hw, classes, nullptr);
}
int vido_mask_logit_select_n(vido_ctx* ctx, const float* feat, const float* w, const float* b, const long long* labels, float* out, int n, int c, int hw, int classes, const int32_t* n_live)
{
    if (!ctx) return VIDO_E_INVALID;
    if (!feat || !w || !labels || !out || n < 1 || c < 1 || c > 1024 || hw < 1 || classes < 1) return vido_set_error(ctx, VIDO_E_INVALID, "mask_logit_select: bad arguments");
    HIP_TRY(ctx, hipSetDevice(ctx->device));
    hipStream_t st = ctx->has_ext_stream ? ctx->ext_stream : ctx->stream;
    hipLaunchKernelGGL(k_mask_logit_select, dim3((unsigned)((hw + 255) / 256), (unsigned)n), dim3(256), 0, st, feat, w, b, labels, out, c, hw, classes, n_live);
    HIP_TRY(ctx, hipGetLastError());
    return VIDO_OK;
}

int vido_bias_act(vido_ctx* ctx, float* x, const float* bias, int N, int C, int H, int W, float slope)
{
    if (!ctx) return VIDO_E_INVALID;
    if (!x || !bias || N < 1 || C < 1 || H < 1 || W < 1) return vido_set_error(ctx, VIDO_E_INVALID, "bias_act: bad arguments");
    HIP_TRY(ctx, hipSetDevice(ctx->device));
    hipStream_t st = ctx->has_ext_stream ? ctx->ext_stream : ctx->stream;
    const size_t hw = (size_t)H * W, total = (size_t)N * C * hw;
    hipLaunchKernelGGL(k_bias_act, dim3((unsigned)((total / 4 + 256) / 256)), dim3(256), 0, st, x, bias, C, hw, total, slope);
    HIP_TRY(ctx, hipGetLastError());
    return VIDO_OK;
}

int vido_bias_unary(vido_ctx* ctx, float* x, const float* bias, int N, int C, int H, int W, int kind)
{
    if (!ctx) return VIDO_E_INVALID;
    if (!x || !bias || N < 1 || C < 1 || H < 1 || W < 1 || (kind != 1 && kind != 2)) return vido_set_error(ctx, VIDO_E_INVALID, "bias_unary: bad arguments");
    HIP_TRY(ctx, hipSetDevice(ctx->device));
    hipStream_t st = ctx->has_ext_stream ? ctx->ext_stream : ctx->stream;
    const size_t hw = (size_t)H * W, total = (size_t)N * C * hw;
    if (kind == 1) hipLaunchKernelGGL(k_bias_unary<1>, dim3((unsigned)((total + 255) / 256)), dim3(256), 0, st, x, bias, C, hw, total);
    else hipLaunchKernelGGL(k_bias_unary<2>, dim3((unsigned)((total + 255) / 256)), dim3(256), 0, st, x, bias, C, hw, total);
    HIP_TRY(ctx, hipGetLastError());
    return VIDO_OK;
}

int vido_upcat_reflect(vido_ctx* ctx, const float* x, const float* skip, int C1, int C2, int h, int w, float* out)
{
    if (!ctx) return VIDO_E_INVALID;
    if (!x || !out || C1 < 1 || C2 < 0 || (C2 && !skip) || h < 1 || w < 1) return vido_set_error(ctx, VIDO_E_INVALID, "upcat_reflect: bad arguments");
    HIP_TRY(ctx, hipSetDevice(ctx->device));
    hipStream_t st = ctx->has_ext_stream ? ctx->ext_stream : ctx->stream;
    const size_t total = (size_t)(C1 + C2) * (2 * h + 2) * (2 * w + 2);
    hipLaunchKernelGGL(k_upcat_reflect, dim3((unsigned)((total + 255) / 256)), dim3(256), 0, st, x, skip, C1, C2, h, w, out);
    HIP_TRY(ctx, hipGetLastError());
    return VIDO_OK;
}

int vido_minmax_norm_u16(vido_ctx* ctx, const float* d, const float* mm, int64_t n, int32_t* out)
{
    if (!ctx) return VIDO_E_INVALID;
    if (!d || !mm || !out || n < 1) return vido_set_error(ctx, VIDO_E_INVALID, "minmax_norm_u16: bad arguments");
    HIP_TRY(ctx, hipSetDevice(ctx->device));
    hipStream_t st = ctx->has_ext_stream ? ctx->ext_stream : ctx->stream;
    hipLaunchKernelGGL(k_minmax_norm_u16, dim3((unsigned)((n + 255) / 256)), dim3(256), 0, st, d, mm, (size_t)n, (int*)out);
    HIP_TRY(ctx, hipGetLastError());
    return VIDO_OK;
}

int vido_area_feed(vido_ctx* ctx, const uint8_t* bgr, int H, int W, float* out, int OH, int OW, float div)
{
    if (!ctx) return VIDO_E_INVALID;
    if (!bgr || !out || H < 1 || W < 1 || OH < 1 || OW < 1 || !(div > 0)) return vido_set_error(ctx, VIDO_E_INVALID, "area_feed: bad arguments");
    HIP_TRY(ctx, hipSetDevice(ctx->device));
    hipStream_t st = ctx->has_ext_stream ? ctx->ext_stream : ctx->stream;
    hipLaunchKernelGGL(k_area_feed, dim3((OW + 63) / 64, (OH + 3) / 4), dim3(256), 0, st, bgr, H, W, out, OH, OW, div);
    HIP_TRY(ctx, hipGetLastError());
    return VIDO_OK;
}

int vido_backwarp(vido_ctx* ctx, const float* x, const float* flow, int B, int C, int H, int W, float* out)
{
    if (!ctx) return VIDO_E_INVALID;
    if (!x || !flow || !out || B < 1 || C < 1 || H < 2 || W < 2 || (long long)B * ((C + 7) / 8) > 65535) return vido_set_error(ctx, VIDO_E_INVALID, "backwarp: bad arguments");
    HIP_TRY(ctx, hipSetDevice(ctx->device));
    hipStream_t st = ctx->has_ext_stream ? ctx->ext_stream : ctx->stream;
    hipLaunchKernelGGL(k_backwarp, dim3((W + 63) / 64, (H + 3) / 4, B * ((C + BW_CG - 1) / BW_CG)), dim3(256), 0, st, x, flow, B, C, H, W, out);
    HIP_TRY(ctx, hipGetLastError());
    return VIDO_OK;
}

int vido_deconv4s2_depthwise(vido_ctx* ctx, const float* x, const float* weight, int B, int C, int H, int W, float input_slope, float* out)
{
    if (!ctx) return VIDO_E_INVALID;
    if (!x || !weight || !out || B < 1 || C < 1 || H < 1 || W < 1 || (long long)B * C > 65535) return vido_set_error(ctx, VIDO_E_INVALID, "deconv4s2_depthwise: bad arguments");
    HIP_TRY(ctx, hipSetDevice(ctx->device));
    hipStream_t st = ctx->has_ext_stream ? ctx->ext_stream : ctx->stream;
    hipLaunchKernelGGL(k_deconv4s2_dw, dim3((2 * W + 63) / 64, (2 * H + 3) / 4, B * C), dim3(256), 0, st, x, weight, C, H, W, input_slope, out);
    HIP_TRY(ctx, hipGetLastError());
    return VIDO_OK;
}

int vido_lfn_reg_front(vido_ctx* ctx, const float* im1, const float* im2, const float* flow, const float* mean, float scale, int B, int C, int H, int W, float* out, int out_channels)
{
    if (!ctx) return VIDO_E_INVALID;
    if (!im1 || !im2 || !flow || !mean || !out || B < 1 || B > 65535 || C < 1 || H < 2 || W < 2 || out_channels < 3) return vido_set_error(ctx, VIDO_E_INVALID, "lfn_reg_front: bad arguments");
    HIP_TRY(ctx, hipSetDevice(ctx->device));
    hipStream_t st = ctx->has_ext_stream ? ctx->ext_stream : ctx->stream;
    hipLaunchKernelGGL(k_lfn_reg_front, dim3((W + 63) / 64, (H + 3) / 4, B), dim3(256), 0, st, im1, im2, flow, mean, scale, B, C, H, W, out, out_channels);
    HIP_TRY(ctx, hipGetLastError());
    return VIDO_OK;
}

int vido_lfn_reg_tail(vido_ctx* ctx, const float* dist, const float* flow, const float* wx, const float* bx, const float* wy, const float* by, int B, int K, int H, int W, float* out)
{
    if (!ctx) return VIDO_E_INVALID;
    if (!dist || !flow || !wx || !bx || !wy || !by || !out || B < 1 || B > 65535 || H < 1 || W < 1 || (K != 3 && K != 5 && K != 7)) return vido_set_error(ctx, VIDO_E_INVALID, "lfn_reg_tail: bad arguments (K must be 3, 5 or 7)");
    HIP_TRY(ctx, hipSetDevice(ctx->device));
    hipStream_t st = ctx->has_ext_stream ? ctx->ext_stream : ctx->stream;
    const dim3 grid((W + 63) / 64, (H + 3) / 4, B);
    if (K == 3) hipLaunchKernelGGL(k_lfn_reg_tail<3>, grid, dim3(256), 0, st, dist, flow, wx, bx, wy, by, B, H, W, out);
    else if (K == 5) hipLaunchKernelGGL(k_lfn_reg_tail<5>, grid, dim3(256), 0, st, dist, flow, wx, bx, wy, by, B, H, W, out);
    else hipLaunchKernelGGL(k_lfn_reg_tail<7>, grid, dim3(256), 0, st, dist, flow, wx, bx, wy, by, B, H, W, out);
    HIP_TRY(ctx, hipGetLastError());
    return VIDO_OK;
}

int vido_bias_res_act(vido_ctx* ctx, float* x, const float* bias, const float* res, int N, int C, int H, int W, float slope)
{
    if (!ctx) return VIDO_E_INVALID;
    if (!res) return vido_bias_act(ctx, x, bias, N, C, H, W, slope);
    if (!x || !bias || N < 1 || C < 1 || H < 1 || W < 1) return vido_set_error(ctx, VIDO_E_INVALID, "bias_res_act: bad arguments");
    HIP_TRY(ctx, hipSetDevice(ctx->device));
    hipStream_t st = ctx->has_ext_stream ? ctx->ext_stream : ctx->stream;
    const size_t hw = (size_t)H * W, total = (size_t)N * C * hw;
    hipLaunchKernelGGL(k_bias_res_act, dim3((unsigned)((total / 4 + 256) / 256)), dim3(256), 0, st, x, bias, res, C, hw, total, slope);
    HIP_TRY(ctx, hipGetLastError());
    return VIDO_OK;
}

int vido_nchw_to_nhwc(vido_ctx* ctx, const float* src, int B, int C, int H, int W, float* dst)
{
    if (!ctx) return VIDO_E_INVALID;
    if (!src || !dst || B < 1 || C < 1 || H < 1 || W < 1 || B > 65535) return vido_set_error(ctx, VIDO_E_INVALID, "nchw_to_nhwc: bad arguments");
    HIP_TRY(ctx, hipSetDevice(ctx->device));
    hipStream_t st = ctx->has_ext_stream ? ctx->ext_stream : ctx->stream;
    hipLaunchKernelGGL(k_nchw_to_nhwc, dim3((H * W + 63) / 64, (C + 63) / 64, B), dim3(256), 0, st, src, C, H * W, dst);
    HIP_TRY(ctx, hipGetLastError());
    return VIDO_OK;
}

int vido_roi_align(vido_ctx* ctx, const float* feat, int B, int C, int H, int W, const float* rois, int n_rois, float spatial_scale,
                   int pooled_h, int pooled_w, int sampling_ratio, float* out, int on_device)
{
    if (!ctx) return VIDO_E_INVALID;
    if (!feat || (n_rois && (!rois || !out)) || B < 1 || C < 1 || H < 1 || W < 1 || n_rois < 0 || pooled_h < 1 || pooled_w < 1) return vido_set_error(ctx, VIDO_E_INVALID, "roi_align: bad arguments");
    if (n_rois == 0) return VIDO_OK;
    HIP_TRY(ctx, hipSetDevice(ctx->device));
    hipStream_t st = (on_device && ctx->has_ext_stream) ? ctx->ext_stream : ctx->stream;
    const size_t nf = (size_t)B * C * H * W * 4, nr = (size_t)n_rois * 5 * 4, nout = (size_t)n_rois * C * pooled_h * pooled_w * 4;
    const float *df = feat, *dr = rois; float* dout = out; NetState* S = nullptr;
    const size_t base = on_device ? 0 : al256(nf) + al256(nr) + al256(nout);
    { int rc = net_scratch(ctx, base + al256(nf), &S); if (rc) return rc; }
    if (!on_device) {
        for (int i = 0; i < n_rois; i++) if (!(rois[5 * i] >= 0 && rois[5 * i] < B)) return vido_set_error(ctx, VIDO_E_INVALID, "roi_align: roi %d has batch index %g", i, rois[5 * i]);
        memcpy(S->h, feat, nf); memcpy(S->h + al256(nf), rois, nr);
        HIP_TRY(ctx, hipMemcpyAsync(S->d, S->h, al256(nf) + al256(nr), hipMemcpyHostToDevice, st));
        df = (float*)S->d; dr = (float*)(S->d + al256(nf)); dout = (float*)(S->d + al256(nf) + al256(nr));
    }
    float* nhwc = (float*)(S->d + base);
    hipLaunchKernelGGL(k_nchw_to_nhwc, dim3((H * W + 63) / 64, (C + 63) / 64, B), dim3(256), 0, st, df, C, H * W, nhwc);
    RoiLevels L{}; L.feat[0] = nhwc; L.H[0] = H; L.W[0] = W; L.scale[0] = spatial_scale;
    const size_t lds = (size_t)64 * ((pooled_h * pooled_w) | 1) * sizeof(float);
    if (lds > 150 * 1024) return vido_set_error(ctx, VIDO_E_CAPACITY, "roi_align: pooled size %d x %d too large", pooled_h, pooled_w);
    { int rc = roi_lds_limit(ctx, lds); if (rc) return rc; }
    if (sampling_ratio == 2) hipLaunchKernelGGL(k_roi_align_nhwc<2>, dim3(n_rois, (C + 63) / 64), dim3(256), lds, st, L, C, dr, 5, (const int*)nullptr, pooled_h, pooled_w, sampling_ratio, dout, (const int*)nullptr);
    else hipLaunchKernelGGL(k_roi_align_nhwc<0>, dim3(n_rois, (C + 63) / 64), dim3(256), lds, st, L, C, dr, 5, (const int*)nullptr, pooled_h, pooled_w, sampling_ratio, dout, (const int*)nullptr);
    HIP_TRY(ctx, hipGetLastError());
    if (!on_device) {
        HIP_TRY(ctx, hipStreamSynchronize(st));
        HIP_TRY(ctx, hipMemcpyAsync(S->h, dout, nout, hipMemcpyDeviceToHost, st)); HIP_TRY(ctx, hipStreamSynchronize(st));
        memcpy(out, S->h, nout);
    }
    return VIDO_OK;
}

static int nms_impl(vido_ctx* ctx, const float* boxes_xyxy, const float* scores, const int32_t* groups, int n, float thresh, int32_t* keep_out, int32_t* n_keep, int on_device)
{
    if (!ctx) return VIDO_E_INVALID;
    if (n < 0 || !n_keep || (n && (!boxes_xyxy || !keep_out)) || (!on_device && n && !scores)) return vido_set_error(ctx, VIDO_E_INVALID, "nms: bad arguments");
    if (n > 65536) return vido_set_error(ctx, VIDO_E_CAPACITY, "nms: %d boxes > 65536", n);
    HIP_TRY(ctx, hipSetDevice(ctx->device));
    hipStream_t st = (on_device && ctx->has_ext_stream) ? ctx->ext_stream : ctx->stream;
    if (n == 0) { if (on_device) HIP_TRY(ctx, hipMemsetAsync(n_keep, 0, 4, st)); else *n_keep = 0; return VIDO_OK; }
    const int cb = (n + 63) / 64;
    const size_t nb = (size_t)n * 16, nm = (size_t)n * cb * 8, nk = (size_t)n * 4 + 256, ng = (size_t)n * 4;
    NetState* S = nullptr;
    int rc = net_scratch(ctx, al256(nb) + al256(nm) + al256(nk) + al256(ng), &S); if (rc) return rc;
    const int* dgroups = groups;
    const float* dboxes = boxes_xyxy; unsigned long long* dmask = (unsigned long long*)(S->d + al256(nb));
    int* dkeep = keep_out; int* dn = n_keep;
    std::vector<int> order;
    if (!on_device) {
        order.resize(n); std::iota(order.begin(), order.end(), 0);
        std::stable_sort(order.begin(), order.end(), [&](int a, int b) { return scores[a] > scores[b]; });
        float* hb = (float*)S->h;
        for (int i = 0; i < n; i++) memcpy(hb + 4 * (size_t)i, boxes_xyxy + 4 * (size_t)order[i], 16);
        HIP_TRY(ctx, hipMemcpyAsync(S->d, S->h, nb, hipMemcpyHostToDevice, st));
        dboxes = (float*)S->d; dkeep = (int*)(S->d + al256(nb) + al256(nm)); dn = dkeep + n;
        if (groups) {
            int* hg = (int*)(S->h + al256(nb)); for (int i = 0; i < n; i++) hg[i] = groups[order[i]];
            int* dg = (int*)(S->d + al256(nb) + al256(nm) + al256(nk));
            HIP_TRY(ctx, hipMemcpyAsync(dg, hg, ng, hipMemcpyHostToDevice, st)); dgroups = dg;
        }
    }
    hipLaunchKernelGGL(k_nms_mask, dim3((cb * (cb + 1) / 2 + 3) / 4), dim3(256), 0, st, dboxes, dgroups, n, thresh, dmask, cb);
    hipLaunchKernelGGL(k_nms_sweep, dim3(1), dim3(64), 0, st, dmask, n, cb, dkeep, dn);
    HIP_TRY(ctx, hipGetLastError());
    if (!on_device) {
        HIP_TRY(ctx, hipStreamSynchronize(st));
        HIP_TRY(ctx, hipMemcpyAsync(S->h, dkeep, nk, hipMemcpyDeviceToHost, st)); HIP_TRY(ctx, hipStreamSynchronize(st));
        const int* hk = (const int*)S->h; const int m = hk[n];
        for (int i = 0; i < m; i++) keep_out[i] = order[hk[i]];
        std::sort(keep_out, keep_out + m);
        *n_keep = m;
    }
    return VIDO_OK;
}

int vido_nms(vido_ctx* ctx, const float* boxes_xyxy, const float* scores, int n, float thresh, int32_t* keep_out, int32_t* n_keep, int on_device)
{
    return nms_impl(ctx, boxes_xyxy, scores, nullptr, n, thresh, keep_out, n_keep, on_device);
}
int vido_nms_grouped(vido_ctx* ctx, const float* boxes_xyxy, const float* scores, const int32_t* groups, int n, float thresh,
                     int32_t* keep_out, int32_t* n_keep, int on_device)
{
    if (n > 0 && !groups) return ctx ? vido_set_error(ctx, VIDO_E_INVALID, "nms_grouped: null groups") : VIDO_E_INVALID;
    return nms_impl(ctx, boxes_xyxy, scores, groups, n, thresh, keep_out, n_keep, on_device);
}

int vido_nms_segments(vido_ctx* ctx, const float* boxes_xyxy, const int32_t* groups, const int32_t* seg_off, const int32_t* seg_n, int n_seg, int max_n, int total,
                      float thresh, int32_t* keep_out, int32_t* n_keep)
{
    if (!ctx) return VIDO_E_INVALID;
    if (!boxes_xyxy || !seg_off || !seg_n || !keep_out || !n_keep || n_seg < 1 || max_n < 1 || total < 1) return vido_set_error(ctx, VIDO_E_INVALID, "nms_segments: bad arguments");
    if (max_n > 65536) return vido_set_error(ctx, VIDO_E_CAPACITY, "nms_segments: %d boxes per segment > 65536", max_n);
    HIP_TRY(ctx, hipSetDevice(ctx->device));
    hipStream_t st = ctx->has_ext_stream ? ctx->ext_stream : ctx->stream;
    const int cb = (max_n + 63) / 64;
    NetState* S = nullptr;
    int rc = net_scratch(ctx, al256((size_t)total * cb * 8), &S); if (rc) return rc;
    unsigned long long* dmask = (unsigned long long*)S->d;
    hipLaunchKernelGGL(k_nms_mask_seg, dim3((cb * (cb + 1) / 2 + 3) / 4, n_seg), dim3(256), 0, st, boxes_xyxy, groups, seg_off, seg_n, thresh, dmask, cb);
    hipLaunchKernelGGL(k_nms_sweep_seg, dim3(n_seg), dim3(64), 0, st, dmask, seg_off, seg_n, cb, keep_out, n_keep, max_n);
    HIP_TRY(ctx, hipGetLastError());
    return VIDO_OK;
}

int vido_roi_align_fpn(vido_ctx* ctx, const float* const feat[4], const int H[4], const int W[4], const float scale[4], int C, const float* boxes, const int32_t* level,
                       int n, int pooled_h, int pooled_w, int sampling_ratio, float* out)
{
    if (!ctx) return VIDO_E_INVALID;
    if (!feat || !H || !W || !scale || C < 1 || n < 0 || pooled_h < 1 || pooled_w < 1 || (n && (!boxes || !level || !out))) return vido_set_error(ctx, VIDO_E_INVALID, "roi_align_fpn: bad arguments");
    if (n == 0) return VIDO_OK;
    HIP_TRY(ctx, hipSetDevice(ctx->device));
    hipStream_t st = ctx->has_ext_stream ? ctx->ext_stream : ctx->stream;
    size_t off[5] = {0, 0, 0, 0, 0};
    for (int l = 0; l < 4; l++) off[l + 1] = off[l] + al256((size_t)C * H[l] * W[l] * 4);
    NetState* S = nullptr;
    { int rc = net_scratch(ctx, off[4], &S); if (rc) return rc; }
    const float* nh[4];
    for (int l = 0; l < 4; l++) {
        hipLaunchKernelGGL(k_nchw_to_nhwc, dim3((H[l] * W[l] + 63) / 64, (C + 63) / 64, 1), dim3(256), 0, st, feat[l], C, H[l] * W[l], (float*)(S->d + off[l]));
        nh[l] = (const float*)(S->d + off[l]);
    }
    return vido_roi_align_fpn_nhwc(ctx, nh, H, W, scale, C, boxes, level, n, pooled_h, pooled_w, sampling_ratio, out);
}

int vido_roi_align_fpn_nhwc(vido_ctx* ctx, const float* const feat[4], const int H[4], const int W[4], const float scale[4], int C, const float* boxes, const int32_t* level,
                            int n, int pooled_h, int pooled_w, int sampling_ratio, float* out)
{
    return vido_roi_align_fpn_nhwc_n(ctx, feat, H, W, scale, C, boxes, level, n, pooled_h, pooled_w, sampling_ratio, out, nullptr);
}
int vido_roi_align_fpn_nhwc_n(vido_ctx* ctx, const float* const feat[4], const int H[4], const int W[4], const float scale[4], int C, const float* boxes, const int32_t* level,
                              int n, int pooled_h, int pooled_w, int sampling_ratio, float* out, const int32_t* n_live)
{
    if (!ctx) return VIDO_E_INVALID;
    if (!feat || !H || !W || !scale || C < 1 || n < 0 || pooled_h < 1 || pooled_w < 1 || (n && (!boxes || !level || !out))) return vido_set_error(ctx, VIDO_E_INVALID, "roi_align_fpn_nhwc: bad arguments");
    if (n == 0) return VIDO_OK;
    HIP_TRY(ctx, hipSetDevice(ctx->device));
    hipStream_t st = ctx->has_ext_stream ? ctx->ext_stream : ctx->stream;
    RoiLevels L;
    for (int l = 0; l < 4; l++) { L.feat[l] = feat[l]; L.H[l] = H[l]; L.W[l] = W[l]; L.scale[l] = scale[l]; }
    const size_t lds = (size_t)64 * ((pooled_h * pooled_w) | 1) * sizeof(float);
    if (lds > 150 * 1024) return vido_set_error(ctx, VIDO_E_CAPACITY, "roi_align_fpn: pooled size %d x %d too large", pooled_h, pooled_w);
    { int rc = roi_lds_limit(ctx, lds); if (rc) return rc; }
    if (sampling_ratio == 2) hipLaunchKernelGGL(k_roi_align_nhwc<2>, dim3(n, (C + 63) / 64), dim3(256), lds, st, L, C, boxes, 4, level, pooled_h, pooled_w, sampling_ratio, out, n_live);
    else hipLaunchKernelGGL(k_roi_align_nhwc<0>, dim3(n, (C + 63) / 64), dim3(256), lds, st, L, C, boxes, 4, level, pooled_h, pooled_w, sampling_ratio, out, n_live);
    HIP_TRY(ctx, hipGetLastError());
    return VIDO_OK;
}

int vido_mask_label_image(vido_ctx* ctx, const float* masks, const float* boxes, const int64_t* labels, int n, int M, int padding, float thresh, int H, int W, uint8_t* out)
{
    if (!ctx) return VIDO_E_INVALID;
    if (!out || H < 1 || W < 1 || n < 0 || M < 1 || padding < 0 || (n && (!masks || !boxes || !labels))) return vido_set_error(ctx, VIDO_E_INVALID, "mask_label_image: bad arguments");
    HIP_TRY(ctx, hipSetDevice(ctx->device));
    hipStream_t st = ctx->has_ext_stream ? ctx->ext_stream : ctx->stream;
    if (n == 0) { HIP_TRY(ctx, hipMemsetAsync(out, 0, (size_t)H * W, st)); return VIDO_OK; }
    NetState* S = nullptr;
    int rc = net_scratch(ctx, al256((size_t)n * sizeof(PasteDet)), &S); if (rc) return rc;
    PasteDet* det = (PasteDet*)S->d;
    hipLaunchKernelGGL(k_paste_prepare, dim3((n + 255) / 256), dim3(256), 0, st, boxes, labels, n, M, padding, det);
    hipLaunchKernelGGL(k_paste_label, dim3((W + 31) / 32, (H + 7) / 8), dim3(256), 0, st, masks, det, n, M, padding, thresh, H, W, out);
    HIP_TRY(ctx, hipGetLastError());
    return VIDO_OK;
}

int vido_mask_instance_image(vido_ctx* ctx, const float* masks, const float* boxes, const int64_t* labels, int n, int M, int padding, float thresh, int H, int W,
                             const int32_t* id_base_dev, uint8_t* out, int32_t* area_out)
{
    if (!ctx) return VIDO_E_INVALID;
    if (!out || H < 1 || W < 1 || n < 0 || M < 1 || padding < 0 || (n && (!masks || !boxes || !labels))) return vido_set_error(ctx, VIDO_E_INVALID, "mask_instance_image: bad arguments");
    if (n > 255) return vido_set_error(ctx, VIDO_E_CAPACITY, "mask_instance_image: %d detections, ids are u8 (n + id_base <= 255)", n);
    HIP_TRY(ctx, hipSetDevice(ctx->device));
    hipStream_t st = ctx->has_ext_stream ? ctx->ext_stream : ctx->stream;
    PasteDet* det = nullptr;
    if (n) {
        NetState* S = nullptr;
        int rc = net_scratch(ctx, al256((size_t)n * sizeof(PasteDet)), &S); if (rc) return rc;
        det = (PasteDet*)S->d;
        if (area_out) hipLaunchKernelGGL(k_zero_i32, dim3((n + 255) / 256), dim3(256), 0, st, area_out, n);
        hipLaunchKernelGGL(k_paste_prepare, dim3((n + 255) / 256), dim3(256), 0, st, boxes, labels, n, M, padding, det);
    }
    hipLaunchKernelGGL(k_paste_instance, dim3((W + 31) / 32, (H + 7) / 8), dim3(256), 0, st, masks, det, n, M, padding, thresh, H, W, id_base_dev, out, area_out);
    HIP_TRY(ctx, hipGetLastError());
    return VIDO_OK;
}

int vido_box_decode(vido_ctx* ctx, const float* deltas, const float* boxes, int n, int k, const float weights[4], float* out, int on_device)
{
    if (!ctx) return VIDO_E_INVALID;
    if (n < 0 || k < 1 || !weights || (n && (!deltas || !boxes || !out))) return vido_set_error(ctx, VIDO_E_INVALID, "box_decode: bad arguments");
    if (n == 0) return VIDO_OK;
    HIP_TRY(ctx, hipSetDevice(ctx->device));
    hipStream_t st = (on_device && ctx->has_ext_stream) ? ctx->ext_stream : ctx->stream;
    const size_t nd = (size_t)n * k * 16, nb = (size_t)n * 16;
    const float *dd = deltas, *db = boxes; float* dout = out; NetState* S = nullptr;
    if (!on_device) {
        int rc = net_scratch(ctx, 2 * al256(nd) + al256(nb), &S); if (rc) return rc;
        memcpy(S->h, deltas, nd); memcpy(S->h + al256(nd), boxes, nb);
        HIP_TRY(ctx, hipMemcpyAsync(S->d, S->h, al256(nd) + al256(nb), hipMemcpyHostToDevice, st));
        dd = (float*)S->d; db = (float*)(S->d + al256(nd)); dout = (float*)(S->d + al256(nd) + al256(nb));
    }
    hipLaunchKernelGGL(k_box_decode, dim3((n * k + 255) / 256), dim3(256), 0, st, dd, db, n, k, weights[0], weights[1], weights[2], weights[3], dout);
    HIP_TRY(ctx, hipGetLastError());
    if (!on_device) {
        HIP_TRY(ctx, hipStreamSynchronize(st));
        HIP_TRY(ctx, hipMemcpyAsync(S->h, dout, nd, hipMemcpyDeviceToHost, st)); HIP_TRY(ctx, hipStreamSynchronize(st));
        memcpy(out, S->h, nd);
    }
    return VIDO_OK;
}

}
```

vido-slam_amd/nets/maskrcnn.py:

```python
import math
import os
from collections import OrderedDict
from dataclasses import dataclass
import numpy as np
import torch
import torch.nn as nn
import torch.nn.functional as F


@dataclass
class MaskRCNNConfig:
    blocks: tuple = (3, 4, 23, 3)
    groups: int = 32
    width_per_group: int = 8
    stride_in_1x1: bool = False
    stem_out: int = 64
    res2_out: int = 256
    fpn_out: int = 256
    anchor_sizes: tuple = (32, 64, 128, 256, 512)
    aspect_ratios: tuple = (0.5, 1.0, 2.0)
    anchor_strides: tuple = (4, 8, 16, 32, 64)
    pre_nms_top_n: int = 1000
    post_nms_top_n: int = 1000
    fpn_post_nms_top_n: int = 1000
# ... 477 lines not shown

class _MaskFeatures(nn.Module):
    def __init__(self, c, ops):
        super().__init__()
        self.pooler = _Pooler(c.mask_resolution, c.pool_scales, c.sampling_ratio, ops)
        cin = c.fpn_out; self.names = []
        for i, ch in enumerate(c.mask_layers, 1):
            setattr(self, "mask_fcn%d" % i, nn.Conv2d(cin, ch, 3, 1, 1)); self.names.append("mask_fcn%d" % i); cin = ch

    def forward(self, feats, boxes, n_live=None):
        x = self.pooler(feats, boxes, n_live) if n_live is not None else self.pooler(feats, boxes)
        for n in self.names:
            x = _conv_bias_relu(getattr(self, n), x, self.pooler.ops if hasattr(self.pooler.ops, "bias_act_") else None, n_live)
        return x


class _MaskPredictor(nn.Module):
    def __init__(self, c):
        super().__init__()
        self.conv5_mask = nn.ConvTranspose2d(c.mask_layers[-1], c.mask_layers[-1], 2, 2, 0)
        self.mask_fcn_logits = nn.Conv2d(c.mask_layers[-1], c.num_classes, 1)

    _ops = None

    def forward(self, x):
        return self.mask_fcn_logits(_conv_bias_relu(self.conv5_mask, x, self._ops))

    def selected(self, x, labels, n_live=None):
        y = _conv_bias_relu(self.conv5_mask, x, self._ops, n_live)
        if self._ops is not None and y.is_cuda and hasattr(self._ops, "mask_logit_select") and not os.environ.get("VIDO_NO_MASK_SELECT") and labels.dtype == torch.int64:
            return self._ops.mask_logit_select(y.contiguous(), self.mask_fcn_logits, labels.contiguous(), n_live)
        return self.mask_fcn_logits(y).sigmoid()[torch.arange(x.shape[0], device=labels.device), labels][:, None]


class _MaskHead(nn.Module):
    buckets = (4, 8, 16, 32, 64, 100)

    def __init__(self, c, ops):
        super().__init__()
        self.feature_extractor = _MaskFeatures(c, ops); self.predictor = _MaskPredictor(c)

    def forward(self, feats, boxes, labels):
        if not len(boxes):
            return feats[0].new_zeros((0, 1, 2 * self.feature_extractor.pooler.res, 2 * self.feature_extractor.pooler.res))
        n = len(boxes); self.last_n = n
        idx = torch.arange(n, device=labels.device)
        if not (boxes.is_cuda and self.buckets):
            return self.predictor(self.feature_extractor(feats, boxes)).sigmoid()[idx, labels][:, None]
        out = []; big = self.buckets[-1]
        for a in range(0, n, big):
            bx, lb = boxes[a:a + big], labels[a:a + big]; k = len(bx)
            m = next(b for b in self.buckets if b >= k)
            if m > k:
                bx = torch.cat([bx, bx.new_zeros((m - k, 4))]); lb = torch.cat([lb, lb.new_zeros((m - k,))])
            g = self.graphed.get(m) if self.graphed and feats[0].data_ptr() == self._graph_feat_ptr else None
            logits = g(bx) if g is not None else self.chunk_logits(feats, bx)
            out.append(logits.sigmoid()[torch.arange(m, device=lb.device), lb][:k, None])
        return torch.cat(out)

    graphed = None; _graph_feat_ptr = 0; last_n = 0

    def chunk_logits(self, feats, bx):
        return self.predictor(self.feature_extractor(feats, bx))

    def capture_buckets(self, feats, graphed_cls):
        feats = list(feats)
        self.graphed = {}
        for b in self.buckets:
            ex = torch.tensor([[10.0, 10.0, 200.0, 300.0]], device=feats[0].device).repeat(b, 1)
            self.graphed[b] = graphed_cls(lambda bx, _f=feats: self.chunk_logits(_f, bx), [ex])
        self._graph_feat_ptr = feats[0].data_ptr()


class _RoiHeads(nn.Module):
    def __init__(self, c, ops):
        super().__init__()
        self.box = _BoxHead(c, ops); self.mask = _MaskHead(c, ops)


def paste_masks(masks, boxes, im_h, im_w, thresh=0.5, padding=1):
    n, M = masks.shape[0], masks.shape[-1]
    out = torch.zeros((n, im_h, im_w), dtype=torch.bool, device=masks.device)
    if n == 0:
        return out
    scale = float(M + 2 * padding) / M
    padded = F.pad(masks.float(), (padding,) * 4)
    b = boxes.float()
    wh, hh = (b[:, 2] - b[:, 0]) * 0.5 * scale, (b[:, 3] - b[:, 1]) * 0.5 * scale
    xc, yc = (b[:, 2] + b[:, 0]) * 0.5, (b[:, 3] + b[:, 1]) * 0.5
    ib = torch.stack([xc - wh, yc - hh, xc + wh, yc + hh], 1).to(torch.int32).cpu().tolist()
    for i, (x0, y0, x1, y1) in enumerate(ib):
        w, h = max(x1 - x0 + 1, 1), max(y1 - y0 + 1, 1)
        m = F.interpolate(padded[i:i + 1], size=(h, w), mode="bilinear", align_corners=False)[0, 0] > thresh
        xa, xb, ya, yb = max(x0, 0), min(x1 + 1, im_w), max(y0, 0), min(y1 + 1, im_h)
        if xb > xa and yb > ya:
            out[i, ya:yb, xa:xb] = m[ya - y0:yb - y0, xa - x0:xb - x0]
    return out


class MaskRCNN(nn.Module):

    def __init__(self, ops, config=None):
        super().__init__()
        self.config = c = config or MaskRCNNConfig()
        self.backbone = nn.Sequential(OrderedDict([("body", _Body(c)), ("fpn", _FPN(c))]))
        self.rpn = _RPN(c, ops)
        self.roi_heads = _RoiHeads(c, ops)
        for m in self.modules():
            if isinstance(m, (_RPNHead, _MaskPredictor, _FPN)):
                m._ops = ops if hasattr(ops, "bias_act_") else None

    @torch.no_grad()
    def forward(self, image):
        feats, logits, deltas = self.trunk(image)
        return self.heads(feats, logits, deltas, image.shape[-2:])

    @torch.no_grad()
    def trunk(self, image):
        feats = self.backbone(image)
        logits, deltas = self.rpn.head(feats)
        return feats, logits, deltas

    @torch.no_grad()
    def heads(self, feats, logits, deltas, image_hw):
        H, W = image_hw
        proposals, objectness = self.rpn.proposals(feats, logits, deltas, (W, H))
        maps = self.fpn_maps(feats)
        boxes, scores, labels = self.roi_heads.box(maps, proposals, (W, H), objectness)
        masks = self.roi_heads.mask(maps, boxes, labels)
        return dict(boxes=boxes, scores=scores, labels=labels, masks=masks, proposals=proposals, objectness=objectness, n_proposals=(objectness >= 0).sum())


def _fpn_maps(self, feats):
    ops = self.rpn.ops; lv = tuple(feats[:len(self.config.pool_scales)])
    if not (hasattr(ops, "to_nhwc") and lv[0].is_cuda and len(lv) == 4):
        return lv
    m = FpnMaps(lv); m.nhwc = tuple(ops.to_nhwc(f) for f in lv)
    return m


@torch.no_grad()
def _heads_static(self, feats, logits, deltas, image_hw, cap=None, confidence=None):
    H, W = image_hw; c = self.config; cap = cap or c.detections_per_img
    fused = self.fused_post and hasattr(self.rpn.ops, "det_select") and c.pre_nms_top_n <= 1024 and c.rpn_min_size <= 0
    proposals, objectness = (self.rpn.proposals_fused if fused else self.rpn.proposals_device)(feats, logits, deltas, (W, H))
    maps = self.fpn_maps(feats)
    bh = self.roi_heads.box
    lg, dl = bh.predictor(bh.feature_extractor(maps, proposals))
    boxes, scores, labels, n_det = (bh.postprocess_fused if fused else bh.postprocess_static)(lg, dl, proposals, (W, H), objectness, cap)
    mh = self.roi_heads.mask
    out = dict(boxes=boxes, scores=scores, labels=labels, n_det=n_det, proposals=proposals, objectness=objectness, n_proposals=(objectness >= 0).sum())
    if confidence is not None:
        order, lab, n_live, n32 = self.rpn.ops.det_order(scores.contiguous(), labels.contiguous(), n_det.reshape(1), confidence, count32=True)
        out.update(order=order, labels_ordered=lab, n_live=n_live,
                   masks=mh.predictor.selected(mh.feature_extractor(maps, boxes[order], n32), lab, n32))
        return out
    out["masks"] = mh.predictor.selected(mh.feature_extractor(maps, boxes), labels)
    return out


MaskRCNN.fused_post = True
MaskRCNN.fpn_maps = _fpn_maps
MaskRCNN.heads_static = _heads_static


LABEL_MODES = ("class", "instance")


def _check_label_mode(label_mode):
    if label_mode not in LABEL_MODES:
        raise ValueError("label_mode: one of %s, not %r" % (LABEL_MODES, label_mode))


def label_image_torch(masks, boxes, scores, labels, H, W, confidence=0.8, label_mode="class", id_base=0, max_instances=None):
    _check_label_mode(label_mode)
    keep = torch.nonzero(scores > confidence).squeeze(1)
    keep = keep[scores[keep].sort(0, descending=True)[1]]
    if label_mode == "instance" and max_instances is not None:
        keep = keep[:max_instances]
    labels = labels[keep]
    n = int(keep.numel())
    if n == 0:
        return torch.zeros((H, W), dtype=torch.uint8, device=masks.device), labels
    pasted = paste_masks(masks[keep], boxes[keep], H, W)
    if label_mode == "class":
        return (pasted.to(torch.int32) * labels.view(-1, 1, 1).to(torch.int32)).sum(0).remainder(256).to(torch.uint8), labels
    if not torch.is_tensor(id_base) and n + int(id_base) > 255:
        raise ValueError("label_mode='instance': %d detections above id base %d, ids are u8 (n + id_base <= 255)" % (n, id_base))
    slot = torch.arange(1, n + 1, dtype=torch.int32, device=masks.device).view(-1, 1, 1)
    first = torch.where(pasted & (labels != 0).view(-1, 1, 1), slot, slot.new_full((), n + 1)).min(0)[0]
    base = id_base.reshape(()).to(torch.int32) if torch.is_tensor(id_base) else int(id_base)
    return torch.where(first <= n, first + base, torch.zeros_like(first)).to(torch.uint8), labels


@torch.no_grad()
def analyse_image_static(net, feats, logits, deltas, out_hw, feed=(1088, 800), confidence=0.8, cap=None, label_mode="class", id_base=None):
    _check_label_mode(label_mode)
    H, W = out_hw
    ops = net.rpn.ops
    c = net.config; ncap = cap or c.detections_per_img
    fused = net.fused_post and hasattr(ops, "det_select") and c.pre_nms_top_n <= 1024 and c.rpn_min_size <= 0
    live_first = (hasattr(ops, "det_order") and fused and ncap <= 1024 and feats[0].is_cuda and not os.environ.get("VIDO_NO_DET_ORDER") and not os.environ.get("VIDO_MASK_HEAD_ALL"))
    out = net.heads_static(feats, logits, deltas, feed, cap, confidence) if live_first else net.heads_static(feats, logits, deltas, feed, cap)
    cap = out["boxes"].shape[0]
    rw, rh = float(W) / feed[1], float(H) / feed[0]
    cache = net.__dict__.setdefault("_const_cache", {})
    key = ("box_scale", rw, rh, str(out["boxes"].device))
    if key not in cache:
        cache[key] = out["boxes"].new_tensor([rw, rh, rw, rh])
    boxes = out["boxes"] * cache[key]
    nd = out["n_det"]
    if "order" in out:
        order, labels, n_live = out["order"], out["labels_ordered"], out["n_live"]
        masks = out["masks"]
    elif hasattr(ops, "det_order") and cap <= 1024 and nd.dtype == torch.int32 and out["labels"].dtype == torch.int64 and not os.environ.get("VIDO_NO_DET_ORDER"):
        order, labels, n_live = ops.det_order(out["scores"].contiguous(), out["labels"].contiguous(), nd.reshape(1), confidence)
    else:
        live = (out["scores"] > confidence) & (torch.arange(cap, device=boxes.device) < nd)
        order = torch.sort(torch.where(live, out["scores"], out["scores"].new_full((), -1.0)), descending=True, stable=True)[1]
        labels = torch.where(live, out["labels"], torch.zeros_like(out["labels"]))[order]
        n_live = live.sum()
    if "order" not in out:
        masks = out["masks"][order]
    if label_mode == "instance":
        if cap > 255:
            raise ValueError("label_mode='instance': %d slots, ids are u8" % cap)
        img = ops.mask_instance_image(masks, boxes[order], labels, H, W, id_base=id_base)
    else:
        img = ops.mask_label_image(masks, boxes[order], labels, H, W)
    return img, labels, n_live, out["n_det"]


def image_to_feed(bgr, dev, feed=(1088, 800), ops=None):
    if ops is not None and torch.is_tensor(bgr) and bgr.is_cuda and bgr.dtype == torch.uint8:
        return ops.area_feed(bgr.contiguous(), feed)
    t = (bgr.to(dev).flip(-1) if torch.is_tensor(bgr) else torch.as_tensor(bgr[:, :, ::-1].copy(), device=dev)).permute(2, 0, 1).float().unsqueeze(0)
    return F.interpolate(t, size=feed, mode="area")


@torch.no_grad()
def analyse_image(net, bgr, feed=(1088, 800), confidence=0.8, trunk=None, on_range=None, label_mode="class", id_base=None, max_instances=None):
    _check_label_mode(label_mode)
    if on_range is not None:
        from .ops import range_checked
        return range_checked(lambda safe: analyse_image(net, bgr, feed, confidence, None if safe else trunk, None, label_mode, id_base, max_instances), (net,), on_range, "the detector")
    dev = next(net.parameters()).device
    H, W = bgr.shape[:2]
    if trunk is not None:
        feats, logits, deltas = trunk(bgr)
        out = net.heads(feats, logits, deltas, feed)
    else:
        out = net(image_to_feed(bgr, dev, feed))
    rw, rh = float(W) / feed[1], float(H) / feed[0]
    boxes = out["boxes"] * out["boxes"].new_tensor([rw, rh, rw, rh]) if rw != rh else out["boxes"] * rw
    ops = getattr(net.rpn, "ops", None)
    if hasattr(ops, "mask_label_image") and out["masks"].is_cuda:
        keep = torch.nonzero(out["scores"] > confidence).squeeze(1)
        keep = keep[out["scores"][keep].sort(0, descending=True)[1]]
        if label_mode == "instance" and max_instances is not None:
            keep = keep[:max_instances]
        labels = out["labels"][keep]
        if label_mode == "instance":
            return ops.mask_instance_image(out["masks"][keep], boxes[keep], labels, H, W, id_base=id_base), labels
        return ops.mask_label_image(out["masks"][keep], boxes[keep], labels, H, W), labels
    return label_image_torch(out["masks"], boxes, out["scores"], out["labels"], H, W, confidence, label_mode, 0 if id_base is None else id_base, max_instances)
```

vido-slam_amd/nets/ops.py:

```python
import contextlib
import ctypes as C
import os
import torch

_WINO_MIN_WGS = int(os.environ.get("VIDO_WINO_MIN_WGS", "0"))
_CONV3X3_H_MIN_WGS = 0 if os.environ.get("VIDO_CONV3X3_H") == "0" else int(os.environ.get("VIDO_CONV3X3_H_MIN_WGS", "128"))
_CONVDIRECT_SET = os.environ.get("VIDO_CONVDIRECT_SET", "novalu")


def correlation_torch_reference(first, second, stride):
    a, b = first[:, :, ::stride, ::stride], second[:, :, ::stride, ::stride]
    pad = torch.nn.functional.pad(b, (3, 3, 3, 3))
    H, W = a.shape[2], a.shape[3]
    return torch.stack([(a * pad[:, :, p:p + H, o:o + W]).mean(1) for p in range(7) for o in range(7)], 1)


class HipOps:

    _range_safe = 0

    def __init__(self, ctx):
        self.ctx = ctx

    @property
# ... 181 lines not shown

    def conv1x1_range_flag(self, reset=True):
        return int(self.ctx.lib.vido_conv1x1_range_flag(self.ctx.h, int(bool(reset))))

    def conv1x1_layout(self, cin, cout, hw):
        return int(self.ctx.lib.vido_conv1x1_layout(int(cin), int(cout), int(hw)))

    def conv1x1_bias_act(self, x, w_packed, bias=None, residual=None, slope=1.0, residual_up2=None):
        assert x.is_cuda and x.is_contiguous() and x.dtype == torch.float32 and x.shape[0] == 1
        _, cin, H, W = x.shape
        if isinstance(w_packed, PackedConv1x1):
            w_packed = w_packed.get(self.conv1x1_layout(cin, w_packed.cout, H * W), x.device)
        cout = (w_packed.numel() // (2 * (cin + 1)) if w_packed.dim() == 1 else w_packed.numel() // cin // 3) if w_packed.dtype == torch.int16 else w_packed.numel() // cin
        layout = self.conv1x1_layout(cin, cout, H * W)
        assert not self.conv1x1_supported(cin, cout, H * W) or tuple(w_packed.shape) == {0: (cout // 32, cin // 8, 64, 4), 1: (cout // 16, cin // 16, 64, 4), 2: (cout // 32, cin // 16, 3, 64, 8),
                                                                                         3: (2 * cout * (cin + 1),)}[layout], \
            "conv1x1: weight packed for another form (pack_conv1x1(w, layout))"
        assert 0.0 <= slope <= 1.0 and (residual is None or residual_up2 is None)
        out = torch.empty((1, cout, H, W), device=x.device, dtype=torch.float32)
        self.gconv_flops = getattr(self, "gconv_flops", 0.0) + 2.0 * cout * cin * H * W
        self._adopt_stream()
        pb = C.c_void_p(bias.data_ptr()) if bias is not None else None
        if residual_up2 is not None:
            residual_up2 = residual_up2.contiguous(); assert tuple(residual_up2.shape) == (1, cout, H // 2, W // 2) and H % 2 == 0 and W % 2 == 0
            self.ctx._check(self.ctx.lib.vido_conv1x1_bias_up2_act(self.ctx.h, C.c_void_p(x.data_ptr()), C.c_void_p(w_packed.data_ptr()), pb, C.c_void_p(residual_up2.data_ptr()),
                                                                   C.c_void_p(out.data_ptr()), int(cin), int(cout), int(H), int(W), C.c_float(slope)))
            return out
        if residual is not None:
            residual = residual.contiguous(); assert residual.shape == out.shape
        self.ctx._check(self.ctx.lib.vido_conv1x1_bias_act(self.ctx.h, C.c_void_p(x.data_ptr()), C.c_void_p(w_packed.data_ptr()), pb,
                                                           C.c_void_p(residual.data_ptr()) if residual is not None else None, C.c_void_p(out.data_ptr()), int(cin), int(cout), int(H * W), C.c_float(slope)))
        return out

    def conv1x1_conv(self, conv, x, slope=1.0, residual=None, residual_up2=None):
        w = conv.weight
        if (tuple(w.shape[2:]) != (1, 1) or tuple(conv.stride) != (1, 1) or tuple(conv.padding) != (0, 0) or conv.groups != 1 or not x.is_cuda or x.shape[0] != 1
                or self._range_safe or not self.conv1x1_supported(w.shape[1], w.shape[0], x.shape[2] * x.shape[3])):
            return None
        if not conv1x1_fills_chip(w.shape[0], x.shape[2] * x.shape[3]):
            return None
        layout = self.conv1x1_layout(w.shape[1], w.shape[0], x.shape[2] * x.shape[3])
        key = (w.data_ptr(), w._version, str(x.device), layout)
        if getattr(conv, "_c1_key", None) != key:
            conv._c1_w = pack_conv1x1(w, layout).to(x.device); conv._c1_key = key
        return self.conv1x1_bias_act(x.contiguous(), conv._c1_w, conv.bias, residual, slope, residual_up2)

    def conv_kxk_c2(self, conv, x, residual=None):
        w = conv.weight
        k = int(w.shape[2])
        if (w.shape[0] != 2 or w.shape[2] != w.shape[3] or k not in (3, 5, 7) or tuple(conv.stride) != (1, 1) or tuple(conv.padding) != (k // 2, k // 2) or tuple(conv.dilation) != (1, 1)
                or conv.groups != 1 or not x.is_cuda or x.shape[0] != 1 or x.dtype != torch.float32):
            return None
        x = x.contiguous(); wc = w.contiguous()
        _, cin, H, W = x.shape
        out = torch.empty((1, 2, H, W), device=x.device, dtype=torch.float32)
        if residual is not None:
            residual = residual.contiguous(); assert residual.shape == out.shape
        self.gconv_flops = getattr(self, "gconv_flops", 0.0) + 2.0 * 2 * cin * k * k * H * W
        self._adopt_stream()
        self.ctx._check(self.ctx.lib.vido_conv_kxk_c2(self.ctx.h, C.c_void_p(x.data_ptr()), C.c_void_p(wc.data_ptr()), C.c_void_p(conv.bias.data_ptr()) if conv.bias is not None else None,
                                                      C.c_void_p(residual.data_ptr()) if residual is not None else None, C.c_void_p(out.data_ptr()), int(cin), k, int(H), int(W)))
        return out

    def conv1x1_skinny(self, x, w_packed, bias, cout, slope=1.0, residual=None):
        assert x.is_cuda and x.dtype == torch.float32 and x.shape[0] == 1
        x = x.contiguous(); cin, H, W = int(x.shape[1]), int(x.shape[2]), int(x.shape[3])
        out = torch.empty((1, cout, H, W), device=x.device, dtype=torch.float32)
        if residual is not None:
            residual = residual.contiguous(); assert residual.shape == out.shape
        self.gconv_flops = getattr(self, "gconv_flops", 0.0) + 2.0 * cout * cin * H * W
        self._adopt_stream()
        self.ctx._check(self.ctx.lib.vido_conv1x1_skinny(self.ctx.h, C.c_void_p(x.data_ptr()), C.c_void_p(w_packed.data_ptr()), C.c_void_p(bias.data_ptr()) if bias is not None else None,
                                                         C.c_void_p(residual.data_ptr()) if residual is not None else None, C.c_void_p(out.data_ptr()), cin, int(cout), C.c_longlong(H * W), C.c_float(slope)))
        return out

    def conv1x1_skinny_conv(self, conv, x, slope=1.0):
        w = conv.weight
        cout, cin = int(w.shape[0]), int(w.shape[1])
        if (tuple(w.shape[2:]) != (1, 1) or tuple(conv.stride) != (1, 1) or tuple(conv.padding) != (0, 0) or conv.groups != 1 or cin % 2 or cin > 256 or cout > 256
                or not x.is_cuda or x.shape[0] != 1 or x.dtype != torch.float32):
            return None
        key = (w.data_ptr(), w._version, str(x.device))
        if getattr(conv, "_c1s_key", None) != key:
            conv._c1s_w = pack_conv1x1_skinny(w).to(x.device); conv._c1s_key = key
        return self.conv1x1_skinny(x, conv._c1s_w, conv.bias, cout, slope)

    def stem7x7s2_pool(self, x, w_packed, bias):
        assert x.is_cuda and x.dtype == torch.float32 and x.dim() == 4 and x.shape[0] == 1 and x.shape[1] == 3 and tuple(w_packed.shape) == (2, 84, 64) and bias.numel() == 64
        x = x.contiguous(); H, W = int(x.shape[2]), int(x.shape[3])
        Hc, Wc = (H - 1) // 2 + 1, (W - 1) // 2 + 1
        out = torch.empty((1, 64, (Hc - 1) // 2 + 1, (Wc - 1) // 2 + 1), device=x.device, dtype=torch.float32)
        self.gconv_flops = getattr(self, "gconv_flops", 0.0) + 2.0 * 64 * 147 * Hc * Wc
        self._adopt_stream()
        self.ctx._check(self.ctx.lib.vido_stem7x7s2_pool(self.ctx.h, C.c_void_p(x.data_ptr()), C.c_void_p(w_packed.data_ptr()), C.c_void_p(bias.data_ptr()), C.c_void_p(out.data_ptr()), H, W))
        return out

    def stem7x7s2_pool_conv(self, mod, w, bias, x):
        if tuple(w.shape) != (64, 3, 7, 7) or bias is None or bias.numel() != 64 or not x.is_cuda or x.shape[0] != 1 or x.shape[1] != 3 or x.dtype != torch.float32 or w.dtype != torch.float32:
            return None
        key = (w.data_ptr(), w._version, str(x.device))
        if getattr(mod, "_stem_key", None) != key:
            mod._stem_w = pack_stem7x7(w).to(x.device); mod._stem_b = bias.detach().to(x.device).contiguous(); mod._stem_key = key
        return self.stem7x7s2_pool(x, mod._stem_w, mod._stem_b)

    def wino3x3_supported(self, cin, cout, H, W):
        return bool(self.ctx.lib.vido_wino3x3_supported(int(cin), int(cout), int(H), int(W)))

    def wino3x3_form(self, N, cin, cout, H, W):
        return int(self.ctx.lib.vido_wino3x3_form(int(N), int(cin), int(cout), int(H), int(W)))

    def wino3x3_bias_act(self, x, u_packed, bias, cout, slope=1.0, form=0):
        assert x.is_cuda and x.is_contiguous() and x.dtype == torch.float32 and u_packed.is_cuda
        N, cin, H, W = x.shape
        out = torch.empty((N, cout, H, W), device=x.device, dtype=torch.float32)
        self.gconv_flops = getattr(self, "gconv_flops", 0.0) + 2.0 * N * cout * cin * 9 * H * W
        self._adopt_stream()
        self.ctx._check(self.ctx.lib.vido_wino3x3_bias_act_form(self.ctx.h, C.c_void_p(x.data_ptr()), C.c_void_p(u_packed.data_ptr()), C.c_void_p(bias.data_ptr()) if bias is not None else None,
                                                                C.c_void_p(out.data_ptr()), int(N), int(cin), int(cout), int(H), int(W), C.c_float(slope), int(form)))
        return out

    def wino3x3_conv(self, conv, x, slope, weight=None, bias=None, n_live=None):
        w = conv.weight if weight is None else weight
        b = conv.bias if bias is None and weight is None else bias
        if (tuple(w.shape[2:]) != (3, 3) or tuple(conv.stride) != (1, 1) or tuple(conv.padding) != (1, 1) or tuple(conv.dilation) != (1, 1) or conv.groups != 1
                or getattr(conv, "padding_mode", "zeros") != "zeros" or not x.is_cuda or not self.wino3x3_supported(w.shape[1], w.shape[0], x.shape[2], x.shape[3])
                or 4 * x.numel() >= 1 << 30 or 4 * x.shape[0] * w.shape[0] * x.shape[2] * x.shape[3] >= 1 << 30):
            return None
        if _WINO_MIN_WGS > 0 and not self.ctx.lib.vido_wino3x3_fills_chip(int(x.shape[0]), int(w.shape[0]), int(x.shape[2]), int(x.shape[3]), _WINO_MIN_WGS):
            return None
        if (_CONV3X3_H_MIN_WGS > 0 and x.dtype == torch.float32 and not self._range_safe and self.ctx.lib.vido_conv3x3_h_supported(int(x.shape[0]), int(w.shape[1]), int(w.shape[0]), int(x.shape[2]), int(x.shape[3]))
                and self.ctx.lib.vido_conv3x3_h_workgroups(int(x.shape[0]), int(w.shape[0]), int(x.shape[2]), int(x.shape[3])) >= (1 if int(w.shape[0]) == 64 else _CONV3X3_H_MIN_WGS)):
            key = (w.data_ptr(), w._version, str(x.device))
            if getattr(conv, "_c3h_key", None) != key:
                conv._c3h_w = pack_conv3x3_h(w).to(x.device); conv._c3h_key = key
            return self.conv3x3_h_bias_act(x.contiguous(), conv._c3h_w, b, int(w.shape[0]), slope, n_live)
        form = self.wino3x3_form(x.shape[0], w.shape[1], w.shape[0], x.shape[2], x.shape[3])
        key = (w.data_ptr(), w._version, str(x.device))
        if getattr(conv, "_wino_key", None) != key:
            conv._wino_u = {}; conv._wino_key = key
        if form not in conv._wino_u:
            conv._wino_u[form] = pack_wino3x3(w, form).to(x.device)
        return self.wino3x3_bias_act(x.contiguous(), conv._wino_u[form], b, int(w.shape[0]), slope, form)

    def conv3x3_h_bias_act(self, x, w_packed, bias, cout, slope, n_live=None):
        assert x.is_cuda and x.is_contiguous() and x.dtype == torch.float32
        N, cin, H, W = x.shape
        assert w_packed.dtype == torch.int16 and w_packed.numel() == 2 * cout * ((cin + 15) // 16 * 16 * 9 + 1), "conv3x3_h: weight not packed by pack_conv3x3_h for this layer"
        out = torch.empty((N, cout, H, W), device=x.device, dtype=torch.float32)
        self.gconv_flops = getattr(self, "gconv_flops", 0.0) + 2.0 * N * cout * cin * 9 * H * W
        self._adopt_stream()
        self.ctx._check(self.ctx.lib.vido_conv3x3_h_bias_act_n(self.ctx.h, C.c_void_p(x.data_ptr()), C.c_void_p(w_packed.data_ptr()), C.c_void_p(bias.data_ptr()) if bias is not None else None,
                                                               C.c_void_p(out.data_ptr()), int(N), int(cin), int(cout), int(H), int(W), C.c_float(slope), self._live_ptr(n_live)))
        return out

    def fc_h(self, x, w_packed, bias, outs, slope=1.0):
        assert x.is_cuda and x.is_contiguous() and x.dtype == torch.float32 and x.dim() == 2
        rows, k = int(x.shape[0]), int(x.shape[1])
        S = int(self.ctx.lib.vido_fc_h_splitk(rows, k, int(outs)))
        if S <= 0:
            return None
        assert w_packed.dtype == torch.int16 and w_packed.numel() == 2 * outs * (k + 1), "fc_h: weight not packed (pack_conv1x1(w[:, :, None, None], 3))"
        part = torch.empty((S, rows, outs), device=x.device, dtype=torch.float32); y = torch.empty((rows, outs), device=x.device, dtype=torch.float32)
        self.gconv_flops = getattr(self, "gconv_flops", 0.0) + 2.0 * rows * k * outs
        self._adopt_stream()
        self.ctx._check(self.ctx.lib.vido_fc_h(self.ctx.h, C.c_void_p(x.data_ptr()), C.c_void_p(w_packed.data_ptr()), C.c_void_p(bias.data_ptr()) if bias is not None else None,
                                               C.c_void_p(part.data_ptr()), C.c_void_p(y.data_ptr()), rows, k, int(outs), C.c_float(slope)))
        return y

    def fc_h_linear(self, lin, x, slope=1.0):
        w = lin.weight
        if not x.is_cuda or x.dtype != torch.float32 or x.dim() != 2 or os.environ.get("VIDO_NO_FC_H") or self._range_safe or int(self.ctx.lib.vido_fc_h_splitk(int(x.shape[0]), int(w.shape[1]), int(w.shape[0]))) <= 0:
            return None
        key = (w.data_ptr(), w._version, str(x.device))
        if getattr(lin, "_fch_key", None) != key:
            lin._fch_w = pack_conv1x1(w.detach().reshape(int(w.shape[0]), int(w.shape[1]), 1, 1), 3).to(x.device); lin._fch_key = key
        return self.fc_h(x.contiguous(), lin._fch_w, lin.bias, int(w.shape[0]), slope)

    def conv_direct_conv(self, conv, x, slope):
        w = conv.weight
        kh, kw = int(w.shape[2]), int(w.shape[3]); sh, sw = (int(v) for v in conv.stride); ph, pw = (int(v) for v in conv.padding)
        if _CONVDIRECT_SET == "novalu" and (kh, kw) in ((3, 3), (7, 7)) and int(w.shape[0]) >= 32:
            return None
        if (tuple(conv.dilation) != (1, 1) or conv.groups != 1 or getattr(conv, "padding_mode", "zeros") != "zeros" or not x.is_cuda or x.dtype != torch.float32
                or not self.ctx.lib.vido_conv_direct_supported(int(w.shape[1]), int(w.shape[0]), int(x.shape[2]), int(x.shape[3]), kh, kw, sh, sw, ph, pw)
                or 4 * x.numel() >= 1 << 30):
            return None
        N, cin, H, W = x.shape; cout = int(w.shape[0])
        Ho, Wo = (H + 2 * ph - kh) // sh + 1, (W + 2 * pw - kw) // sw + 1
        if 4 * N * cout * Ho * Wo >= 1 << 30:
            return None
        key = (w.data_ptr(), w._version, str(x.device))
        if getattr(conv, "_cd_key", None) != key:
            conv._cd_w = pack_conv_direct(w).to(x.device); conv._cd_key = key
        x = x.contiguous()
        out = torch.empty((N, cout, Ho, Wo), device=x.device, dtype=torch.float32)
        self.gconv_flops = getattr(self, "gconv_flops", 0.0) + 2.0 * N * cout * cin * kh * kw * Ho * Wo
        self._adopt_stream()
        b = conv.bias
        self.ctx._check(self.ctx.lib.vido_conv_direct_bias_act(self.ctx.h, C.c_void_p(x.data_ptr()), C.c_void_p(conv._cd_w.data_ptr()), C.c_void_p(b.data_ptr()) if b is not None else None,
                                                               C.c_void_p(out.data_ptr()), int(N), int(cin), cout, int(H), int(W), kh, kw, sh, sw, ph, pw, C.c_float(slope)))
        return out

    def lfn_reg_front(self, im1, im2, flow, scale, feat):
        im1 = im1.contiguous(); im2 = im2.contiguous(); flow = flow.contiguous()
        B, Cc, H, W = im1.shape
        out = torch.empty((B, 3 + feat.shape[1], H, W), device=im1.device, dtype=torch.float32)
        mean = flow.flatten(2).mean(2).contiguous()
        self._adopt_stream()
        self.ctx._check(self.ctx.lib.vido_lfn_reg_front(self.ctx.h, C.c_void_p(im1.data_ptr()), C.c_void_p(im2.data_ptr()), C.c_void_p(flow.data_ptr()), C.c_void_p(mean.data_ptr()),
                                                        C.c_float(scale), B, Cc, H, W, C.c_void_p(out.data_ptr()), out.shape[1]))
        out[:, 3:] = feat
        return out

    def lfn_reg_tail(self, dist, flow, scale_x, scale_y, k):
        dist = dist.contiguous(); flow = flow.contiguous()
        B, nd, H, W = dist.shape
        assert nd == k * k
        out = torch.empty((B, 2, H, W), device=dist.device, dtype=torch.float32)
        self._adopt_stream()
        self.ctx._check(self.ctx.lib.vido_lfn_reg_tail(self.ctx.h, C.c_void_p(dist.data_ptr()), C.c_void_p(flow.data_ptr()), C.c_void_p(scale_x.weight.data_ptr()), C.c_void_p(scale_x.bias.data_ptr()),
                                                       C.c_void_p(scale_y.weight.data_ptr()), C.c_void_p(scale_y.bias.data_ptr()), B, int(k), H, W, C.c_void_p(out.data_ptr())))
        return out

    def roi_align(self, feat, rois, output_size, spatial_scale, sampling_ratio):
        if not feat.is_cuda:
            raise RuntimeError("HipOps.roi_align needs CUDA(HIP) tensors; there is no CPU fallback")
        feat = feat.contiguous().float(); rois = rois.contiguous().float()
        B, Cc, H, W = feat.shape; ph, pw = output_size
        out = torch.empty((rois.shape[0], Cc, ph, pw), device=feat.device, dtype=torch.float32)
        self._adopt_stream()
        self.ctx._check(self.ctx.lib.vido_roi_align(self.ctx.h, C.c_void_p(feat.data_ptr()), B, Cc, H, W, C.c_void_p(rois.data_ptr()), rois.shape[0],
                                                    C.c_float(spatial_scale), ph, pw, sampling_ratio, C.c_void_p(out.data_ptr()), 1))
        return out

    def box_decode(self, deltas, boxes, weights):
        deltas = deltas.contiguous().float(); boxes = boxes.contiguous().float(); n = deltas.shape[0]
        out = torch.empty_like(deltas)
        if n:
            w = (C.c_float * 4)(*[float(x) for x in weights])
            self._adopt_stream()
            self.ctx._check(self.ctx.lib.vido_box_decode(self.ctx.h, C.c_void_p(deltas.data_ptr()), C.c_void_p(boxes.data_ptr()), n, deltas.shape[1] // 4, w,
                                                         C.c_void_p(out.data_ptr()), 1))
        return out

    def nms_grouped(self, boxes, scores, groups, thresh):
        if not boxes.is_cuda:
            raise RuntimeError("HipOps.nms_grouped needs CUDA(HIP) tensors; there is no CPU fallback")
        if boxes.shape[0] == 0:
            return torch.zeros((0,), dtype=torch.int64, device=boxes.device)
        order = torch.sort(scores, descending=True, stable=True)[1]
        n = boxes.shape[0]
        if n <= 65536:
            order = order[torch.sort(groups[order], stable=True)[1]]
            cnts = torch.bincount(groups, minlength=1).to(torch.int32)
            seg_off = (torch.cumsum(cnts, 0) - cnts).to(torch.int32)
            max_n = int(cnts.max().item())
            keep, cnt = self.nms_segments(boxes[order], seg_off, cnts, max_n, thresh)
            flat = (keep.long() + seg_off.long()[:, None])[keep >= 0]
            return torch.sort(order[flat])[0]
        sb = boxes[order].contiguous().float(); sg = groups[order].to(torch.int32).contiguous()
        keep = torch.empty(n, device=boxes.device, dtype=torch.int32); cnt = torch.zeros(1, device=boxes.device, dtype=torch.int32)
        self._adopt_stream()
        self.ctx._check(self.ctx.lib.vido_nms_grouped(self.ctx.h, C.c_void_p(sb.data_ptr()), None, C.c_void_p(sg.data_ptr()), n, C.c_float(thresh),
                                                      C.c_void_p(keep.data_ptr()), C.c_void_p(cnt.data_ptr()), 1))
        m = int(cnt.item())
        return torch.sort(order[keep[:m].long()])[0]

    def nms(self, boxes, scores, thresh):
        if not boxes.is_cuda:
            raise RuntimeError("HipOps.nms needs CUDA(HIP) tensors; there is no CPU fallback")
        if boxes.shape[0] == 0:
            return torch.zeros((0,), dtype=torch.int64, device=boxes.device)
        order = torch.sort(scores, descending=True, stable=True)[1]
        sb = boxes[order].contiguous().float(); n = sb.shape[0]
        keep = torch.empty(max(n, 1), device=boxes.device, dtype=torch.int32); cnt = torch.zeros(1, device=boxes.device, dtype=torch.int32)
        self._adopt_stream()
        self.ctx._check(self.ctx.lib.vido_nms(self.ctx.h, C.c_void_p(sb.data_ptr()), None, n, C.c_float(thresh), C.c_void_p(keep.data_ptr()), C.c_void_p(cnt.data_ptr()), 1))
        m = int(cnt.item())
        return torch.sort(order[keep[:m].long()])[0]

    def nms_segments(self, boxes, seg_off, seg_n, max_n, thresh, groups=None):
        boxes = boxes.contiguous().float(); n_seg = seg_n.shape[0]
        keep = torch.empty((n_seg, max_n), device=boxes.device, dtype=torch.int32); cnt = torch.empty(n_seg, device=boxes.device, dtype=torch.int32)
        self._adopt_stream()
        self.ctx._check(self.ctx.lib.vido_nms_segments(self.ctx.h, C.c_void_p(boxes.data_ptr()), C.c_void_p(groups.data_ptr()) if groups is not None else None,
                                                       C.c_void_p(seg_off.data_ptr()), C.c_void_p(seg_n.data_ptr()), n_seg, int(max_n), boxes.shape[0], C.c_float(thresh),
                                                       C.c_void_p(keep.data_ptr()), C.c_void_p(cnt.data_ptr())))
        return keep, cnt

    def roi_align_fpn(self, feats, boxes, level, output_size, scales, sampling_ratio):
        n = boxes.shape[0]; ph, pw = output_size; Cc = feats[0].shape[1]
        out = torch.empty((n, Cc, ph, pw), device=boxes.device, dtype=torch.float32)
        if n == 0:
            return out
        feats = [f.contiguous().float() for f in feats]; boxes = boxes.contiguous().float(); level = level.to(torch.int32).contiguous()
        fp = (C.c_void_p * 4)(*[f.data_ptr() for f in feats]); Hs = (C.c_int * 4)(*[f.shape[2] for f in feats]); Ws = (C.c_int * 4)(*[f.shape[3] for f in feats])
        sc = (C.c_float * 4)(*[float(x) for x in scales])
        self._adopt_stream()
        self.ctx._check(self.ctx.lib.vido_roi_align_fpn(self.ctx.h, fp, Hs, Ws, sc, Cc, C.c_void_p(boxes.data_ptr()), C.c_void_p(level.data_ptr()), n, ph, pw, sampling_ratio,
                                                        C.c_void_p(out.data_ptr())))
        return out

    def rpn_select(self, logits, deltas, cell_anchors, strides, K, image_wh):
        L = len(logits); A = logits[0].shape[1]; dev = logits[0].device
        logits = [t.contiguous() for t in logits]; deltas = [t.contiguous() for t in deltas]
        boxes = torch.empty((L * K, 4), device=dev, dtype=torch.float32); scores = torch.empty((L * K,), device=dev, dtype=torch.float32); n = torch.empty((L,), device=dev, dtype=torch.int32)
        lp = (C.c_void_p * L)(*[t.data_ptr() for t in logits]); dp = (C.c_void_p * L)(*[t.data_ptr() for t in deltas])
        hs = (C.c_int * L)(*[t.shape[2] for t in logits]); ws = (C.c_int * L)(*[t.shape[3] for t in logits]); st = (C.c_int * L)(*[int(s) for s in strides])
        key = ("anch", L, A)
        if getattr(self, "_anch_key", None) != key:
            self._anch = (C.c_float * (L * A * 4))(*[float(v) for a in cell_anchors for v in a.detach().cpu().reshape(-1).tolist()]); self._anch_key = key
        self._adopt_stream()
        self.ctx._check(self.ctx.lib.vido_rpn_select(self.ctx.h, L, lp, dp, hs, ws, st, self._anch, A, int(K), int(image_wh[0]), int(image_wh[1]),
                                                     C.c_void_p(boxes.data_ptr()), C.c_void_p(scores.data_ptr()), C.c_void_p(n.data_ptr())))
        return boxes, scores, n

    def rpn_merge(self, boxes, scores, keep, cnt, K, post_nms_top_n, n_final):
        L = cnt.shape[0]; dev = boxes.device
        ob = torch.empty((n_final, 4), device=dev, dtype=torch.float32); osc = torch.empty((n_final,), device=dev, dtype=torch.float32); nv = torch.empty((1,), device=dev, dtype=torch.int32)
        self._adopt_stream()
        self.ctx._check(self.ctx.lib.vido_rpn_merge(self.ctx.h, C.c_void_p(boxes.data_ptr()), C.c_void_p(scores.data_ptr()), C.c_void_p(keep.data_ptr()), C.c_void_p(cnt.data_ptr()),
                                                    L, int(K), int(post_nms_top_n), int(n_final), C.c_void_p(ob.data_ptr()), C.c_void_p(osc.data_ptr()), C.c_void_p(nv.data_ptr())))
        return ob, osc, nv

    def det_class_sort(self, prob, deltas, proposals, objectness, thresh, weights, image_wh):
        prob = prob.contiguous(); deltas = deltas.contiguous(); proposals = proposals.contiguous()
        N, nc = prob.shape; dev = prob.device
        seg = torch.empty(((nc - 1) * N, 4), device=dev, dtype=torch.float32); order = torch.empty((nc - 1, N), device=dev, dtype=torch.int32); seg_n = torch.empty((nc - 1,), device=dev, dtype=torch.int32)
        wv = (C.c_float * 4)(*[float(x) for x in weights])
        self._adopt_stream()
        self.ctx._check(self.ctx.lib.vido_det_class_sort(self.ctx.h, C.c_void_p(prob.data_ptr()), C.c_void_p(deltas.data_ptr()), C.c_void_p(proposals.data_ptr()),
                                                         C.c_void_p(objectness.data_ptr()) if objectness is not None else None, N, nc, C.c_float(thresh), wv, int(image_wh[0]), int(image_wh[1]),
                                                         C.c_void_p(seg.data_ptr()), C.c_void_p(order.data_ptr()), C.c_void_p(seg_n.data_ptr())))
        return seg, order, seg_n

    def det_select(self, prob, seg_boxes, order, keep, cnt, detections_per_img, cap):
        N, nc = prob.shape; dev = prob.device
        ob = torch.empty((cap, 4), device=dev, dtype=torch.float32); osc = torch.empty((cap,), device=dev, dtype=torch.float32); ol = torch.empty((cap,), device=dev, dtype=torch.int64)
        nd = torch.empty((1,), device=dev, dtype=torch.int32); scratch = torch.empty((nc + 3,), device=dev, dtype=torch.int32)
        self._adopt_stream()
        self.ctx._check(self.ctx.lib.vido_det_select(self.ctx.h, C.c_void_p(prob.data_ptr()), C.c_void_p(seg_boxes.data_ptr()), C.c_void_p(order.data_ptr()), C.c_void_p(keep.data_ptr()),
                                                     C.c_void_p(cnt.data_ptr()), N, nc, int(detections_per_img), int(cap), C.c_void_p(scratch.data_ptr()),
                                                     C.c_void_p(ob.data_ptr()), C.c_void_p(osc.data_ptr()), C.c_void_p(ol.data_ptr()), C.c_void_p(nd.data_ptr())))
        return ob, osc, ol, nd

    def to_nhwc(self, x):
        assert x.is_cuda and x.dtype == torch.float32 and x.dim() == 4
        x = x.contiguous(); B, Cc, H, W = x.shape
        out = torch.empty((B, H, W, Cc), device=x.device, dtype=torch.float32)
        self._adopt_stream()
        self.ctx._check(self.ctx.lib.vido_nchw_to_nhwc(self.ctx.h, C.c_void_p(x.data_ptr()), B, Cc, H, W, C.c_void_p(out.data_ptr())))
        return out

    def roi_align_fpn_nhwc(self, feats_nhwc, boxes, level, output_size, scales, sampling_ratio, n_live=None):
        n = boxes.shape[0]; ph, pw = output_size; Cc = feats_nhwc[0].shape[3]
        out = torch.empty((n, Cc, ph, pw), device=boxes.device, dtype=torch.float32)
        if n == 0:
            return out
        boxes = boxes.contiguous().float(); level = level.to(torch.int32).contiguous()
        fp = (C.c_void_p * 4)(*[f.data_ptr() for f in feats_nhwc]); Hs = (C.c_int * 4)(*[f.shape[1] for f in feats_nhwc]); Ws = (C.c_int * 4)(*[f.shape[2] for f in feats_nhwc])
        sc = (C.c_float * 4)(*[float(x) for x in scales])
        self._adopt_stream()
        self.ctx._check(self.ctx.lib.vido_roi_align_fpn_nhwc_n(self.ctx.h, fp, Hs, Ws, sc, Cc, C.c_void_p(boxes.data_ptr()), C.c_void_p(level.data_ptr()), n, ph, pw, sampling_ratio,
                                                               C.c_void_p(out.data_ptr()), self._live_ptr(n_live)))
        return out

    def mask_label_image(self, masks, boxes, labels, H, W, thresh=0.5, padding=1):
        out = torch.empty((H, W), device=masks.device, dtype=torch.uint8)
        n = masks.shape[0]
        masks = masks.contiguous().float(); boxes = boxes.contiguous().float(); labels = labels.contiguous().to(torch.int64)
        self._adopt_stream()
        self.ctx._check(self.ctx.lib.vido_mask_label_image(self.ctx.h, C.c_void_p(masks.data_ptr()) if n else None, C.c_void_p(boxes.data_ptr()) if n else None,
                                                           C.c_void_p(labels.data_ptr()) if n else None, n, masks.shape[-1] if n else 28, padding, C.c_float(thresh), H, W,
                                                           C.c_void_p(out.data_ptr())))
        return out

    def mask_propagate(self, mask, flow, depth=None, out=None, stats=None):
        from ..host import VidoError
        def bad(why):
            raise VidoError(-1, "mask_propagate: " + why)
        for name, t, dt in (("mask", mask, torch.int32), ("flow", flow, torch.float32), ("depth", depth, torch.float32), ("out", out, torch.int32), ("stats", stats, torch.int32)):
            if t is None:
                continue
            if not torch.is_tensor(t) or not t.is_cuda:
                bad("%s must be a device tensor; there is no CPU fallback" % name)
            if t.dtype != dt:
                bad("%s must be %s, got %s" % (name, dt, t.dtype))
            if not t.is_contiguous():
                bad("%s must be contiguous" % name)
            if t.device != mask.device:
                bad("%s is on another device than mask" % name)
        if mask.dim() != 2:
            bad("mask must be [H, W]")
        H, W = int(mask.shape[0]), int(mask.shape[1])
        if tuple(flow.shape) != (H, W, 2):
            bad("flow must be [%d, %d, 2], got %s" % (H, W, tuple(flow.shape)))
        if depth is not None and tuple(depth.shape) != (H, W):
            bad("depth must be [%d, %d], got %s" % (H, W, tuple(depth.shape)))
        if out is None:
            out = torch.empty((H, W), device=mask.device, dtype=torch.int32)
        elif tuple(out.shape) != (H, W):
            bad("out must be [%d, %d], got %s" % (H, W, tuple(out.shape)))
        if out.data_ptr() < mask.data_ptr() + 4 * H * W and mask.data_ptr() < out.data_ptr() + 4 * H * W:
            bad("out aliases mask")
        if stats is not None and stats.numel() < 3:
            bad("stats needs 3 elements")
        self._adopt_stream()
        self.ctx._check(self.ctx.lib.vido_mask_propagate(self.ctx.h, C.c_void_p(mask.data_ptr()), C.c_void_p(flow.data_ptr()), C.c_void_p(depth.data_ptr()) if depth is not None else None,
                                                         H, W, C.c_void_p(out.data_ptr()), C.c_void_p(stats.data_ptr()) if stats is not None else None))
        return out

    def mask_associate(self, prev, cur, state, classes=None, n=None, hold=0, out=None, lut=None, stats=None):
        from ..host import VidoError
        def bad(why):
            raise VidoError(-1, "mask_associate: " + why)
        for name, t, dt in (("cur", cur, torch.int32), ("prev", prev, torch.int32), ("state", state, torch.int32), ("classes", classes, torch.int64), ("out", out, torch.int32),
                            ("lut", lut, torch.int32), ("stats", stats, torch.int32)):
            if t is None:
                if name in ("cur", "state"):
                    bad("%s is required" % name)
                continue
            if not torch.is_tensor(t) or not t.is_cuda:
                bad("%s must be a device tensor; there is no CPU fallback" % name)
            if t.dtype != dt:
                bad("%s must be %s, got %s" % (name, dt, t.dtype))
            if not t.is_contiguous():
                bad("%s must be contiguous" % name)
            if t.device != cur.device:
                bad("%s is on another device than cur" % name)
        if cur.dim() != 2:
            bad("cur must be [H, W]")
        H, W = int(cur.shape[0]), int(cur.shape[1])
        if prev is not None and tuple(prev.shape) != (H, W):
            bad("prev must be [%d, %d], got %s" % (H, W, tuple(prev.shape)))
        if state.numel() != 768:
            bad("state needs 768 elements")
        if n is None:
            n = int(classes.numel()) if classes is not None else 127
        n = int(n)
        if classes is not None and classes.numel() < n:
            bad("classes holds %d elements, n = %d" % (classes.numel(), n))
        if out is None:
            out = torch.empty((H, W), device=cur.device, dtype=torch.int32)
        elif tuple(out.shape) != (H, W):
            bad("out must be [%d, %d], got %s" % (H, W, tuple(out.shape)))
        for name, t in (("prev", prev), ("cur", cur)):
            if t is not None and out.data_ptr() < t.data_ptr() + 4 * H * W and t.data_ptr() < out.data_ptr() + 4 * H * W and not (name == "cur" and out.data_ptr() == t.data_ptr()):
                bad("out aliases %s" % name)
        if lut is not None and lut.numel() < 256:
            bad("lut needs 256 elements")
        if stats is not None and stats.numel() < 4:
            bad("stats needs 4 elements")
        ptr = lambda t: C.c_void_p(t.data_ptr()) if t is not None else None
        self._adopt_stream()
        self.ctx._check(self.ctx.lib.vido_mask_associate(self.ctx.h, ptr(prev), ptr(cur), H, W, ptr(classes), n, int(hold), ptr(state), ptr(out), ptr(lut), ptr(stats)))
        return out

    def mask_components(self, mask, connectivity=8, min_area=1, id_base=0, cap=127, out=None, classes=None, areas=None, stats=None):
        from ..host import VidoError
        def bad(why):
            raise VidoError(-1, "mask_components: " + why)
        for name, t, dt in (("mask", mask, torch.int32), ("out", out, torch.int32), ("classes", classes, torch.int64), ("areas", areas, torch.int32), ("stats", stats, torch.int32)):
            if t is None:
                if name == "mask":
                    bad("mask is required")
                continue
            if not torch.is_tensor(t) or not t.is_cuda:
                bad("%s must be a device tensor; there is no CPU fallback" % name)
            if t.dtype != dt:
                bad("%s must be %s, got %s" % (name, dt, t.dtype))
            if not t.is_contiguous():
                bad("%s must be contiguous" % name)
            if t.device != mask.device:
                bad("%s is on another device than mask" % name)
        if mask.dim() != 2:
            bad("mask must be [H, W]")
        H, W = int(mask.shape[0]), int(mask.shape[1])
        if out is None:
            out = torch.empty((H, W), device=mask.device, dtype=torch.int32)
        elif tuple(out.shape) != (H, W):
            bad("out must be [%d, %d], got %s" % (H, W, tuple(out.shape)))
        if out.data_ptr() != mask.data_ptr() and out.data_ptr() < mask.data_ptr() + 4 * H * W and mask.data_ptr() < out.data_ptr() + 4 * H * W:
            bad("out aliases mask")
        cap = int(cap)
        for name, t in (("classes", classes), ("areas", areas)):
            if t is not None and t.numel() < cap:
                bad("%s holds %d elements, cap = %d" % (name, t.numel(), cap))
        if stats is not None and stats.numel() < 4:
            bad("stats needs 4 elements")
        ptr = lambda t: C.c_void_p(t.data_ptr()) if t is not None else None
        self._adopt_stream()
        self.ctx._check(self.ctx.lib.vido_mask_components(self.ctx.h, ptr(mask), H, W, int(connectivity), int(min_area), int(id_base), cap, ptr(out), ptr(classes), ptr(areas),
                                                          ptr(stats)))
        return out

    def mask_instance_image(self, masks, boxes, labels, H, W, thresh=0.5, padding=1, id_base=None, areas=False):
        from ..host import VidoError
        out = torch.empty((H, W), device=masks.device, dtype=torch.uint8)
        n = masks.shape[0]
        masks = masks.contiguous().float(); boxes = boxes.contiguous().float(); labels = labels.contiguous().to(torch.int64)
        if id_base is not None and not torch.is_tensor(id_base):
            if id_base < 0 or n + int(id_base) > 255:
                raise VidoError(-4, "mask_instance_image: %d detections above id base %d, ids are u8 (n + id_base <= 255)" % (n, id_base))
            id_base = torch.full((1,), int(id_base), dtype=torch.int32, device=masks.device) if id_base else None
        if id_base is not None:
            assert id_base.is_cuda and id_base.dtype == torch.int32 and id_base.numel() == 1
        area = torch.empty((n,), device=masks.device, dtype=torch.int32) if areas else None
        self._adopt_stream()
        self.ctx._check(self.ctx.lib.vido_mask_instance_image(self.ctx.h, C.c_void_p(masks.data_ptr()) if n else None, C.c_void_p(boxes.data_ptr()) if n else None,
                                                              C.c_void_p(labels.data_ptr()) if n else None, n, masks.shape[-1] if n else 28, padding, C.c_float(thresh), H, W,
                                                              C.c_void_p(id_base.data_ptr()) if id_base is not None else None, C.c_void_p(out.data_ptr()),
                                                              C.c_void_p(area.data_ptr()) if areas and n else None))
        return (out, area) if areas else out


def _ops_of(obj, out):
    if isinstance(obj, HipOps):
        out.setdefault(id(obj), obj)
    elif isinstance(obj, torch.nn.Module):
        for m in obj.modules():
            for v in vars(m).values():
                v = getattr(v, "__self__", v)
                if isinstance(v, HipOps):
                    out.setdefault(id(v), v)
    else:
        raise TypeError("range_safe: a HipOps or an nn.Module, not %s" % type(obj).__name__)
    return out
# ... 187 lines not shown
```

Before: 134.5.

## Adapt mask-head kernels to live detection count with finer tiling and bin splits

Measured after the change: 136.0, median of 6. 1.1% higher.

```diff
diff --git a/include/vido_c.h b/include/vido_c.h
--- a/include/vido_c.h
+++ b/include/vido_c.h
@@ -220,6 +220,9 @@
 int vido_conv3x3_h_workgroups(int n, int cout, int h, int w);
 int vido_conv3x3_h_bias_act(vido_ctx* ctx, const float* x, const void* w_packed, const float* bias, float* y, int n, int cin, int cout, int h, int w, float slope);
 int vido_conv3x3_h_bias_act_n(vido_ctx* ctx, const float* x, const void* w_packed, const float* bias, float* y, int n, int cin, int cout, int h, int w, float slope, const int32_t* n_live);
+int vido_conv3x3_h_live_form(int n, int cout, int h, int w, int live, int* channels, int* block_rows);
+int vido_mask_head_coarse(void);
+int vido_conv3x3_h_bias_act_form(vido_ctx* ctx, const float* x, const void* w_packed, const float* bias, float* y, int n, int cin, int cout, int h, int w, float slope, int rpw, int cg);
 long long vido_wino3x3_packed_floats_form(int cin, int cout, int form);
 int vido_wino3x3_pack_form(const float* w, int cin, int cout, int form, float* u_packed);
 int vido_wino3x3_bias_act_form(vido_ctx* ctx, const float* x, const float* u_packed, const float* bias, float* y, int n, int cin, int cout, int h, int w, float slope, int form);
@@ -259,6 +262,8 @@
 int vido_det_select(vido_ctx* ctx, const float* prob, const float* seg_boxes, const int32_t* order, const int32_t* keep, const int32_t* cnt, int N, int nc, int detections_per_img, int cap,
                     int32_t* scratch, float* out_boxes, float* out_scores, int64_t* out_labels, int32_t* n_det);
 int vido_mask_label_image(vido_ctx* ctx, const float* masks, const float* boxes, const int64_t* labels, int n, int M, int padding, float thresh, int H, int W, uint8_t* out);
+int vido_mask_label_image_n(vido_ctx* ctx, const float* masks, const float* boxes, const int64_t* labels, int n, int M, int padding, float thresh, int H, int W, uint8_t* out,
+                            const int32_t* n_live);
 int vido_mask_instance_image(vido_ctx* ctx, const float* masks, const float* boxes, const int64_t* labels, int n, int M, int padding, float thresh, int H, int W,
                              const int32_t* id_base_dev, uint8_t* out, int32_t* area_out);
 int vido_box_decode(vido_ctx* ctx, const float* deltas, const float* boxes, int n, int k, const float weights[4],
diff --git a/vido-slam_amd/csrc/conv3x3h.hip b/vido-slam_amd/csrc/conv3x3h.hip
--- a/vido-slam_amd/csrc/conv3x3h.hip
+++ b/vido-slam_amd/csrc/conv3x3h.hip
@@ -21,18 +21,16 @@
 struct C3Args { const float* x; const void* wp; const float* bias; float* y; int N, Cin, Cout, H, W, nby, nbx, mt, total, nchunk; float slope; unsigned wbytes; unsigned* range_flag; const int* n_live; };
 
 template <int RPW, int CG>
-__global__ __launch_bounds__(512) void k_conv3x3_h(C3Args A)
+__device__ __forceinline__ void c3_body(const C3Args& A, const int nby, const int nbx, const int mt, const int total, const int per)
 {
     constexpr int BR = 16 / CG, MT = 32 * RPW * CG, WPIX = C3_WPIX(BR), XP = C3_XP(BR), RAWB = C3_RAW(BR), PLANE = C3_PLANE(BR), PBUF = C3_PBUF(BR), CK = (WPIX * 8 + 511) / 512, NMM = 9 * RPW, NRD = 2 * RPW + 2;
     extern __shared__ __attribute__((aligned(16))) char c3_lds[];
     char* L = c3_lds;
     const int tid = threadIdx.x, lane = tid & 63, w = __builtin_amdgcn_readfirstlane(tid >> 6);
-    int total = A.total, per = gridDim.x >> 3;
-    if (A.n_live) { const int nl = min(max(*A.n_live, 0), A.N); total = nl * A.nby * A.nbx * A.mt; per = (total + 7) >> 3; }
     const int q8 = blockIdx.x >> 3, item = (blockIdx.x & 7) * per + q8;
     if (q8 >= per || item >= total) return;
-    const int nt = item / A.mt, mtile = item - nt * A.mt, m0 = mtile * MT;
-    const int bpi = A.nby * A.nbx, n = nt / bpi, brem = nt - n * bpi, by = brem / A.nbx, bx = brem - by * A.nbx, Y0 = by * BR, X0 = bx * 16;
+    const int nt = item / mt, mtile = item - nt * mt, m0 = mtile * MT;
+    const int bpi = nby * nbx, n = nt / bpi, brem = nt - n * bpi, by = brem / nbx, bx = brem - by * nbx, Y0 = by * BR, X0 = bx * 16;
     const int rp = CG == 1 ? w : (w & 3), rb0 = CG == 1 ? 0 : RPW * (w >> 2);
     const int hw = A.H * A.W, nsteps = A.nchunk * 3;
 
@@ -173,6 +171,26 @@
         }
     }
 }
+
+template <int RPW, int CG>
+__global__ __launch_bounds__(512) void k_conv3x3_h(C3Args A)
+{
+    int total = A.total, per = gridDim.x >> 3;
+    if (A.n_live) { const int nl = min(max(*A.n_live, 0), A.N); total = nl * A.nby * A.nbx * A.mt; per = (total + 7) >> 3; }
+    c3_body<RPW, CG>(A, A.nby, A.nbx, A.mt, total, per);
+}
+
+#define C3_FINE_RPW 1
+#define C3_FINE_CG 2
+template <int RPWC, int CGC>
+__global__ __launch_bounds__(512) void k_conv3x3_h_live(C3Args A, int fine_max)
+{
+    constexpr int BRF = 16 / C3_FINE_CG, MTF = 32 * C3_FINE_RPW * C3_FINE_CG, BRC = 16 / CGC, MTC = 32 * RPWC * CGC;
+    const int nl = min(max(*A.n_live, 0), A.N), nbx = (A.W + 15) >> 4;
+    const int nbyf = (A.H + BRF - 1) / BRF, mtf = A.Cout / MTF, tf = nl * nbyf * nbx * mtf;
+    if (tf <= fine_max) c3_body<C3_FINE_RPW, C3_FINE_CG>(A, nbyf, nbx, mtf, tf, (tf + 7) >> 3);
+    else { const int nbyc = (A.H + BRC - 1) / BRC, mtc = A.Cout / MTC, tc = nl * nbyc * nbx * mtc; c3_body<RPWC, CGC>(A, nbyc, nbx, mtc, tc, (tc + 7) >> 3); }
+}
 }
 
 extern "C" {
@@ -194,6 +212,38 @@
     return n * ((h + 15) / 16) * ((w + 15) / 16) * mt >= C3_MIN16 ? 16 : 8;
 }
 int vido_conv3x3_h_workgroups(int n, int cout, int h, int w) { const int br = c3_block_rows(n, cout, h, w); return n * ((h + br - 1) / br) * ((w + 15) / 16) * (cout >= 128 ? cout / 128 : 1); }
+
+int vido_mask_head_coarse(void)
+{
+    static const int v = [] { const char* e = getenv("VIDO_MASK_HEAD_COARSE"); return e && atoi(e) != 0 ? 1 : 0; }();
+    return v;
+}
+
+#define C3_FINE_MAX 512
+static bool c3_live_has_fine(int cout) { return cout >= 128 && !vido_mask_head_coarse(); }
+int vido_conv3x3_h_live_form(int n, int cout, int h, int w, int live, int* channels, int* block_rows)
+{
+    const int nl = live < 0 ? 0 : (live > n ? n : live);
+    constexpr int BRF = 16 / C3_FINE_CG, MTF = 32 * C3_FINE_RPW * C3_FINE_CG;
+    const bool fine = c3_live_has_fine(cout) && (long long)nl * ((h + BRF - 1) / BRF) * ((w + 15) / 16) * (cout / MTF) <= C3_FINE_MAX;
+    if (channels) *channels = fine ? MTF : (cout >= 128 ? 128 : cout);
+    if (block_rows) *block_rows = fine ? BRF : c3_block_rows(n, cout, h, w);
+    return fine ? 1 : 0;
+}
+
+static int c3_set_attrs(vido_ctx* ctx)
+{
+    static bool attr[64] = {};
+    if (!attr[ctx->device & 63]) {
+#define C3_ATTR(RPW_, CG_) HIP_TRY(ctx, hipFuncSetAttribute((const void*)k_conv3x3_h<RPW_, CG_>, hipFuncAttributeMaxDynamicSharedMemorySize, (int)C3_LDS(16 / CG_)))
+        C3_ATTR(4, 1); C3_ATTR(2, 2); C3_ATTR(2, 1); C3_ATTR(1, 2); C3_ATTR(1, 1);
+#undef C3_ATTR
+        HIP_TRY(ctx, hipFuncSetAttribute((const void*)k_conv3x3_h_live<4, 1>, hipFuncAttributeMaxDynamicSharedMemorySize, (int)std::max(C3_LDS(16), C3_LDS(16 / C3_FINE_CG))));
+        HIP_TRY(ctx, hipFuncSetAttribute((const void*)k_conv3x3_h_live<2, 2>, hipFuncAttributeMaxDynamicSharedMemorySize, (int)std::max(C3_LDS(8), C3_LDS(16 / C3_FINE_CG))));
+        attr[ctx->device & 63] = true;
+    }
+    return VIDO_OK;
+}
 
 int vido_conv3x3_h_bias_act(vido_ctx* ctx, const float* x, const void* w_packed, const float* bias, float* y, int n, int cin, int cout, int h, int w, float slope)
 {
@@ -211,12 +261,17 @@
     const int nby = (h + br - 1) / br, nbx = (w + 15) / 16, mt = cout >= 128 ? cout / 128 : 1, total = n * nby * nbx * mt;
     const int nchunk = (cin + 15) / 16;
     C3Args A{x, w_packed, bias, y, n, cin, cout, h, w, nby, nbx, mt, total, nchunk, slope, (unsigned)(36ll * 16 * nchunk * cout), ctx->c1_range_flag, n_live};
-    static bool attr[64] = {};
-    if (!attr[ctx->device & 63]) {
-#define C3_ATTR(RPW_, CG_) HIP_TRY(ctx, hipFuncSetAttribute((const void*)k_conv3x3_h<RPW_, CG_>, hipFuncAttributeMaxDynamicSharedMemorySize, (int)C3_LDS(16 / CG_)))
-        C3_ATTR(4, 1); C3_ATTR(2, 2); C3_ATTR(2, 1); C3_ATTR(1, 2); C3_ATTR(1, 1);
-#undef C3_ATTR
-        attr[ctx->device & 63] = true;
+    { int rc = c3_set_attrs(ctx); if (rc) return rc; }
+    if (n_live && c3_live_has_fine(cout)) {
+        constexpr int BRF = 16 / C3_FINE_CG, MTF = 32 * C3_FINE_RPW * C3_FINE_CG;
+        static_assert(MTF <= 128 && 128 % MTF == 0, "the fine form's channels divide the coarse form's 128");
+        const long long fpi = (long long)((h + BRF - 1) / BRF) * nbx * (cout / MTF);
+        const long long tfine = std::min<long long>(n, C3_FINE_MAX / fpi) * fpi;
+        const dim3 grid((unsigned)(8 * ((std::max<long long>(total, tfine) + 7) / 8)));
+        if (br == 16) hipLaunchKernelGGL((k_conv3x3_h_live<4, 1>), grid, dim3(512), std::max(C3_LDS(16), C3_LDS(BRF)), st, A, (int)C3_FINE_MAX);
+        else hipLaunchKernelGGL((k_conv3x3_h_live<2, 2>), grid, dim3(512), std::max(C3_LDS(8), C3_LDS(BRF)), st, A, (int)C3_FINE_MAX);
+        HIP_TRY(ctx, hipGetLastError());
+        return VIDO_OK;
     }
     const dim3 grid(8 * ((total + 7) / 8));
 #define C3_LAUNCH(RPW_, CG_) hipLaunchKernelGGL((k_conv3x3_h<RPW_, CG_>), grid, dim3(512), C3_LDS(16 / CG_), st, A)
@@ -228,4 +283,24 @@
     return VIDO_OK;
 }
 
-}
+int vido_conv3x3_h_bias_act_form(vido_ctx* ctx, const float* x, const void* w_packed, const float* bias, float* y, int n, int cin, int cout, int h, int w, float slope, int rpw, int cg)
+{
+    if (!ctx) return VIDO_E_INVALID;
+    const int MT = 32 * rpw * cg, form = rpw * 10 + cg;
+    if (!x || !w_packed || !y || x == y || !vido_conv3x3_h_supported(n, cin, cout, h, w) || slope < 0.f || slope > 1.f || (((uintptr_t)x | (uintptr_t)y) & 3) || ((uintptr_t)w_packed & 15)
+        || (form != 41 && form != 22 && form != 21 && form != 12 && form != 11) || cout % MT)
+        return vido_set_error(ctx, VIDO_E_INVALID, "conv3x3_h_form: no kernel <%d, %d> for %d x %d -> %d channels at %d x %d", rpw, cg, n, cin, cout, h, w);
+    HIP_TRY(ctx, hipSetDevice(ctx->device));
+    { int rc = c3_set_attrs(ctx); if (rc) return rc; }
+    hipStream_t st = ctx->has_ext_stream ? ctx->ext_stream : ctx->stream;
+    const int br = 16 / cg, nby = (h + br - 1) / br, nbx = (w + 15) / 16, mt = cout / MT, total = n * nby * nbx * mt, nchunk = (cin + 15) / 16;
+    C3Args A{x, w_packed, bias, y, n, cin, cout, h, w, nby, nbx, mt, total, nchunk, slope, (unsigned)(36ll * 16 * nchunk * cout), ctx->c1_range_flag, nullptr};
+    const dim3 grid(8 * ((total + 7) / 8));
+#define C3_LAUNCH(RPW_, CG_) hipLaunchKernelGGL((k_conv3x3_h<RPW_, CG_>), grid, dim3(512), C3_LDS(16 / CG_), st, A)
+    if (form == 41) C3_LAUNCH(4, 1); else if (form == 22) C3_LAUNCH(2, 2); else if (form == 21) C3_LAUNCH(2, 1); else if (form == 12) C3_LAUNCH(1, 2); else C3_LAUNCH(1, 1);
+#undef C3_LAUNCH
+    HIP_TRY(ctx, hipGetLastError());
+    return VIDO_OK;
+}
+
+}
diff --git a/vido-slam_amd/csrc/nets.hip b/vido-slam_amd/csrc/nets.hip
--- a/vido-slam_amd/csrc/nets.hip
+++ b/vido-slam_amd/csrc/nets.hip
@@ -87,7 +87,7 @@
 }
 
 __global__ __launch_bounds__(256) void k_mask_logit_select(const float* __restrict__ feat, const float* __restrict__ w, const float* __restrict__ b, const long long* __restrict__ labels,
-                                                           float* __restrict__ out, int c, int hw, int classes, const int* __restrict__ n_live)
+                                                           float* __restrict__ out, int c, int hw, int classes, const int* __restrict__ n_live, int batch)
 {
     __shared__ float wl[1024];
     const int n = blockIdx.y, p = blockIdx.x * 256 + threadIdx.x;
@@ -102,6 +102,15 @@
     const float* f = feat + (size_t)n * c * hw + p;
     double a0 = 0, a1 = 0, a2 = 0, a3 = 0;
     int i = 0;
+    if (batch) {
+        for (; i + 32 <= c; i += 32) {
+            float v[32];
+#pragma unroll
+            for (int k = 0; k < 32; k++) v[k] = f[(size_t)(i + k) * hw];
+#pragma unroll
+            for (int k = 0; k < 32; k += 4) { a0 += (double)wl[i + k] * v[k]; a1 += (double)wl[i + k + 1] * v[k + 1]; a2 += (double)wl[i + k + 2] * v[k + 2]; a3 += (double)wl[i + k + 3] * v[k + 3]; }
+        }
+    }
     for (; i + 4 <= c; i += 4) { a0 += (double)wl[i] * f[(size_t)i * hw]; a1 += (double)wl[i + 1] * f[(size_t)(i + 1) * hw]; a2 += (double)wl[i + 2] * f[(size_t)(i + 2) * hw]; a3 += (double)wl[i + 3] * f[(size_t)(i + 3) * hw]; }
     for (; i < c; i++) a0 += (double)wl[i] * f[(size_t)i * hw];
     const float v = (float)((a0 + a1) + (a2 + a3) + (b ? (double)b[lab] : 0.0));
@@ -169,14 +178,16 @@
 }
 
 struct RoiLevels { const float* feat[4]; int H[4], W[4]; float scale[4]; };
-template <int SR >
+template <int SR ,
+          bool SPLIT >
 __global__ __launch_bounds__(256) void k_roi_align_nhwc(RoiLevels L, int C, const float* __restrict__ rois, int roi_stride ,
-                                                        const int* __restrict__ level , int PH, int PW, int sampling, float* __restrict__ out, const int* __restrict__ n_live )
+                                                        const int* __restrict__ level , int PH, int PW, int sampling, float* __restrict__ out, const int* __restrict__ n_live ,
+                                                        int seg_bins )
 {
     extern __shared__ __attribute__((aligned(16))) float rl_tile[];
     if (n_live && (int)blockIdx.x >= *n_live) return;
     const int i = blockIdx.x, c0 = blockIdx.y * 64, lane = threadIdx.x & 63, wave = threadIdx.x >> 6;
-    const int nbin = PH * PW, pitch = nbin | 1;
+    const int nbin = PH * PW, b0 = SPLIT ? blockIdx.z * seg_bins : 0, nsb = SPLIT ? min(seg_bins, nbin - b0) : nbin, pitch = (SPLIT ? seg_bins : nbin) | 1;
     const float* r = rois + (size_t)roi_stride * i;
     const int l = level ? level[i] : 0, bi = roi_stride == 5 ? (int)r[0] : 0;
     const float* box = r + (roi_stride == 5 ? 1 : 0);
@@ -200,7 +211,7 @@
         w1 = hy * hx; w2 = hy * lx; w3 = ly * hx; w4 = ly * lx;
         return out;
     };
-    for (int bin = wave; bin < nbin; bin += 4) {
+    for (int bin = b0 + wave; bin < b0 + nsb; bin += 4) {
         const int ph = bin / PW, pw = bin - ph * PW;
         float acc = 0.f;
         if (SR == 2) {
@@ -229,12 +240,13 @@
                 }
             }
         }
-        rl_tile[lane * pitch + bin] = acc / count;
+        rl_tile[lane * pitch + (bin - b0)] = acc / count;
     }
     __syncthreads();
-    const int nc = min(64, C - c0), total = nc * nbin;
-    float* o = out + ((size_t)i * C + c0) * nbin;
-    for (int e = threadIdx.x; e < total; e += 256) { const int cc = e / nbin; o[e] = rl_tile[cc * pitch + (e - cc * nbin)]; }
+    const int nc = min(64, C - c0), total = nc * nsb;
+    float* o = out + ((size_t)i * C + c0) * nbin + b0;
+    if (SPLIT) for (int e = threadIdx.x; e < total; e += 256) { const int cc = e / nsb, k = e - cc * nsb; o[(size_t)cc * nbin + k] = rl_tile[cc * pitch + k]; }
+    else for (int e = threadIdx.x; e < total; e += 256) { const int cc = e / nbin; o[e] = rl_tile[cc * pitch + (e - cc * nbin)]; }
 }
 __global__ __launch_bounds__(256) void k_nchw_to_nhwc(const float* __restrict__ src, int C, int HW, float* __restrict__ dst)
 {
@@ -389,11 +401,12 @@
     det[i] = d;
 }
 __global__ __launch_bounds__(256) void k_paste_label(const float* __restrict__ masks , const PasteDet* __restrict__ det, int n, int M, int padding, float thresh,
-                                                     int H, int W, uint8_t* __restrict__ out)
+                                                     int H, int W, uint8_t* __restrict__ out, const int* __restrict__ n_live )
 {
     __shared__ PasteDet sd[128];
     const int x = blockIdx.x * 32 + (threadIdx.x & 31), y = blockIdx.y * 8 + (threadIdx.x >> 5);
     const int Mp = M + 2 * padding;
+    if (n_live) n = min(max(*n_live, 0), n);
     unsigned acc = 0;
     for (int d0 = 0; d0 < n; d0 += 128) {
         __syncthreads();
@@ -640,12 +653,15 @@
     out[((size_t)bc * OH + oy) * OW + ox] = acc;
 }
 
+#define ROI_SEG_BINS 16
 static int roi_lds_limit(vido_ctx* ctx, size_t lds)
 {
     static size_t have = 48 * 1024;
     if (lds <= have) return VIDO_OK;
-    HIP_TRY(ctx, hipFuncSetAttribute((const void*)k_roi_align_nhwc<2>, hipFuncAttributeMaxDynamicSharedMemorySize, (int)lds));
-    HIP_TRY(ctx, hipFuncSetAttribute((const void*)k_roi_align_nhwc<0>, hipFuncAttributeMaxDynamicSharedMemorySize, (int)lds));
+    HIP_TRY(ctx, hipFuncSetAttribute((const void*)k_roi_align_nhwc<2, false>, hipFuncAttributeMaxDynamicSharedMemorySize, (int)lds));
+    HIP_TRY(ctx, hipFuncSetAttribute((const void*)k_roi_align_nhwc<0, false>, hipFuncAttributeMaxDynamicSharedMemorySize, (int)lds));
+    HIP_TRY(ctx, hipFuncSetAttribute((const void*)k_roi_align_nhwc<2, true>, hipFuncAttributeMaxDynamicSharedMemorySize, (int)lds));
+    HIP_TRY(ctx, hipFuncSetAttribute((const void*)k_roi_align_nhwc<0, true>, hipFuncAttributeMaxDynamicSharedMemorySize, (int)lds));
     have = lds;
     return VIDO_OK;
 }
@@ -725,7 +741,8 @@
     if (!feat || !w || !labels || !out || n < 1 || c < 1 || c > 1024 || hw < 1 || classes < 1) return vido_set_error(ctx, VIDO_E_INVALID, "mask_logit_select: bad arguments");
     HIP_TRY(ctx, hipSetDevice(ctx->device));
     hipStream_t st = ctx->has_ext_stream ? ctx->ext_stream : ctx->stream;
-    hipLaunchKernelGGL(k_mask_logit_select, dim3((unsigned)((hw + 255) / 256), (unsigned)n), dim3(256), 0, st, feat, w, b, labels, out, c, hw, classes, n_live);
+    hipLaunchKernelGGL(k_mask_logit_select, dim3((unsigned)((hw + 255) / 256), (unsigned)n), dim3(256), 0, st, feat, w, b, labels, out, c, hw, classes, n_live,
+                       n_live && !vido_mask_head_coarse() ? 1 : 0);
     HIP_TRY(ctx, hipGetLastError());
     return VIDO_OK;
 }
@@ -884,8 +901,8 @@
     const size_t lds = (size_t)64 * ((pooled_h * pooled_w) | 1) * sizeof(float);
     if (lds > 150 * 1024) return vido_set_error(ctx, VIDO_E_CAPACITY, "roi_align: pooled size %d x %d too large", pooled_h, pooled_w);
     { int rc = roi_lds_limit(ctx, lds); if (rc) return rc; }
-    if (sampling_ratio == 2) hipLaunchKernelGGL(k_roi_align_nhwc<2>, dim3(n_rois, (C + 63) / 64), dim3(256), lds, st, L, C, dr, 5, (const int*)nullptr, pooled_h, pooled_w, sampling_ratio, dout, (const int*)nullptr);
-    else hipLaunchKernelGGL(k_roi_align_nhwc<0>, dim3(n_rois, (C + 63) / 64), dim3(256), lds, st, L, C, dr, 5, (const int*)nullptr, pooled_h, pooled_w, sampling_ratio, dout, (const int*)nullptr);
+    if (sampling_ratio == 2) hipLaunchKernelGGL((k_roi_align_nhwc<2, false>), dim3(n_rois, (C + 63) / 64), dim3(256), lds, st, L, C, dr, 5, (const int*)nullptr, pooled_h, pooled_w, sampling_ratio, dout, (const int*)nullptr, 0);
+    else hipLaunchKernelGGL((k_roi_align_nhwc<0, false>), dim3(n_rois, (C + 63) / 64), dim3(256), lds, st, L, C, dr, 5, (const int*)nullptr, pooled_h, pooled_w, sampling_ratio, dout, (const int*)nullptr, 0);
     HIP_TRY(ctx, hipGetLastError());
     if (!on_device) {
         HIP_TRY(ctx, hipStreamSynchronize(st));
@@ -1005,16 +1022,27 @@
     const size_t lds = (size_t)64 * ((pooled_h * pooled_w) | 1) * sizeof(float);
     if (lds > 150 * 1024) return vido_set_error(ctx, VIDO_E_CAPACITY, "roi_align_fpn: pooled size %d x %d too large", pooled_h, pooled_w);
     { int rc = roi_lds_limit(ctx, lds); if (rc) return rc; }
-    if (sampling_ratio == 2) hipLaunchKernelGGL(k_roi_align_nhwc<2>, dim3(n, (C + 63) / 64), dim3(256), lds, st, L, C, boxes, 4, level, pooled_h, pooled_w, sampling_ratio, out, n_live);
-    else hipLaunchKernelGGL(k_roi_align_nhwc<0>, dim3(n, (C + 63) / 64), dim3(256), lds, st, L, C, boxes, 4, level, pooled_h, pooled_w, sampling_ratio, out, n_live);
+    static const int seg_env = [] { const char* e = getenv("VIDO_ROI_SEG_BINS"); return e ? atoi(e) : 0; }();
+    const int nbin = pooled_h * pooled_w, sb = n_live && !vido_mask_head_coarse() ? std::min(nbin, seg_env > 0 ? seg_env : ROI_SEG_BINS) : nbin, nseg = (nbin + sb - 1) / sb;
+    const dim3 grid(n, (C + 63) / 64, nseg);
+    if (nseg > 1) {
+        if (sampling_ratio == 2) hipLaunchKernelGGL((k_roi_align_nhwc<2, true>), grid, dim3(256), lds, st, L, C, boxes, 4, level, pooled_h, pooled_w, sampling_ratio, out, n_live, sb);
+        else hipLaunchKernelGGL((k_roi_align_nhwc<0, true>), grid, dim3(256), lds, st, L, C, boxes, 4, level, pooled_h, pooled_w, sampling_ratio, out, n_live, sb);
+    } else if (sampling_ratio == 2) hipLaunchKernelGGL((k_roi_align_nhwc<2, false>), grid, dim3(256), lds, st, L, C, boxes, 4, level, pooled_h, pooled_w, sampling_ratio, out, n_live, 0);
+    else hipLaunchKernelGGL((k_roi_align_nhwc<0, false>), grid, dim3(256), lds, st, L, C, boxes, 4, level, pooled_h, pooled_w, sampling_ratio, out, n_live, 0);
     HIP_TRY(ctx, hipGetLastError());
     return VIDO_OK;
 }
 
 int vido_mask_label_image(vido_ctx* ctx, const float* masks, const float* boxes, const int64_t* labels, int n, int M, int padding, float thresh, int H, int W, uint8_t* out)
 {
-    if (!ctx) return VIDO_E_INVALID;
-    if (!out || H < 1 || W < 1 || n < 0 || M < 1 || padding < 0 || (n && (!masks || !boxes || !labels))) return vido_set_error(ctx, VIDO_E_INVALID, "mask_label_image: bad arguments");
+    return vido_mask_label_image_n(ctx, masks, boxes, labels, n, M, padding, thresh, H, W, out, nullptr);
+}
+int vido_mask_label_image_n(vido_ctx* ctx, const float* masks, const float* boxes, const int64_t* labels, int n, int M, int padding, float thresh, int H, int W, uint8_t* out,
+                            const int32_t* n_live)
+{
+    if (!ctx) return VIDO_E_INVALID;
+    if (!out || H < 1 || W < 1 || n < 0 || M < 1 || padding < 0 || (n && (!masks || !boxes || !labels)) || ((uintptr_t)n_live & 3)) return vido_set_error(ctx, VIDO_E_INVALID, "mask_label_image: bad arguments");
     HIP_TRY(ctx, hipSetDevice(ctx->device));
     hipStream_t st = ctx->has_ext_stream ? ctx->ext_stream : ctx->stream;
     if (n == 0) { HIP_TRY(ctx, hipMemsetAsync(out, 0, (size_t)H * W, st)); return VIDO_OK; }
@@ -1022,7 +1050,7 @@
     int rc = net_scratch(ctx, al256((size_t)n * sizeof(PasteDet)), &S); if (rc) return rc;
     PasteDet* det = (PasteDet*)S->d;
     hipLaunchKernelGGL(k_paste_prepare, dim3((n + 255) / 256), dim3(256), 0, st, boxes, labels, n, M, padding, det);
-    hipLaunchKernelGGL(k_paste_label, dim3((W + 31) / 32, (H + 7) / 8), dim3(256), 0, st, masks, det, n, M, padding, thresh, H, W, out);
+    hipLaunchKernelGGL(k_paste_label, dim3((W + 31) / 32, (H + 7) / 8), dim3(256), 0, st, masks, det, n, M, padding, thresh, H, W, out, vido_mask_head_coarse() ? (const int*)nullptr : (const int*)n_live);
     HIP_TRY(ctx, hipGetLastError());
     return VIDO_OK;
 }
diff --git a/vido-slam_amd/nets/maskrcnn.py b/vido-slam_amd/nets/maskrcnn.py
--- a/vido-slam_amd/nets/maskrcnn.py
+++ b/vido-slam_amd/nets/maskrcnn.py
@@ -653,7 +653,7 @@
     out = dict(boxes=boxes, scores=scores, labels=labels, n_det=n_det, proposals=proposals, objectness=objectness, n_proposals=(objectness >= 0).sum())
     if confidence is not None:
         order, lab, n_live, n32 = self.rpn.ops.det_order(scores.contiguous(), labels.contiguous(), n_det.reshape(1), confidence, count32=True)
-        out.update(order=order, labels_ordered=lab, n_live=n_live,
+        out.update(order=order, labels_ordered=lab, n_live=n_live, n_live32=n32,
                    masks=mh.predictor.selected(mh.feature_extractor(maps, boxes[order], n32), lab, n32))
         return out
     out["masks"] = mh.predictor.selected(mh.feature_extractor(maps, boxes), labels)
@@ -728,7 +728,7 @@
             raise ValueError("label_mode='instance': %d slots, ids are u8" % cap)
         img = ops.mask_instance_image(masks, boxes[order], labels, H, W, id_base=id_base)
     else:
-        img = ops.mask_label_image(masks, boxes[order], labels, H, W)
+        img = ops.mask_label_image(masks, boxes[order], labels, H, W, n_live=out["n_live32"]) if "n_live32" in out else ops.mask_label_image(masks, boxes[order], labels, H, W)
     return img, labels, n_live, out["n_det"]
 
 
diff --git a/vido-slam_amd/nets/ops.py b/vido-slam_amd/nets/ops.py
--- a/vido-slam_amd/nets/ops.py
+++ b/vido-slam_amd/nets/ops.py
@@ -357,6 +357,11 @@
         self.ctx._check(self.ctx.lib.vido_conv3x3_h_bias_act_n(self.ctx.h, C.c_void_p(x.data_ptr()), C.c_void_p(w_packed.data_ptr()), C.c_void_p(bias.data_ptr()) if bias is not None else None,
                                                                C.c_void_p(out.data_ptr()), int(N), int(cin), int(cout), int(H), int(W), C.c_float(slope), self._live_ptr(n_live)))
         return out
+
+    def conv3x3_h_live_form(self, n, cout, h, w, live):
+        ch, br = C.c_int(), C.c_int()
+        fine = self.ctx.lib.vido_conv3x3_h_live_form(int(n), int(cout), int(h), int(w), int(live), C.byref(ch), C.byref(br))
+        return bool(fine), ch.value, br.value
 
     def fc_h(self, x, w_packed, bias, outs, slope=1.0):
         assert x.is_cuda and x.is_contiguous() and x.dtype == torch.float32 and x.dim() == 2
@@ -570,14 +575,14 @@
                                                                C.c_void_p(out.data_ptr()), self._live_ptr(n_live)))
         return out
 
-    def mask_label_image(self, masks, boxes, labels, H, W, thresh=0.5, padding=1):
+    def mask_label_image(self, masks, boxes, labels, H, W, thresh=0.5, padding=1, n_live=None):
         out = torch.empty((H, W), device=masks.device, dtype=torch.uint8)
         n = masks.shape[0]
         masks = masks.contiguous().float(); boxes = boxes.contiguous().float(); labels = labels.contiguous().to(torch.int64)
         self._adopt_stream()
-        self.ctx._check(self.ctx.lib.vido_mask_label_image(self.ctx.h, C.c_void_p(masks.data_ptr()) if n else None, C.c_void_p(boxes.data_ptr()) if n else None,
-                                                           C.c_void_p(labels.data_ptr()) if n else None, n, masks.shape[-1] if n else 28, padding, C.c_float(thresh), H, W,
-                                                           C.c_void_p(out.data_ptr())))
+        self.ctx._check(self.ctx.lib.vido_mask_label_image_n(self.ctx.h, C.c_void_p(masks.data_ptr()) if n else None, C.c_void_p(boxes.data_ptr()) if n else None,
+                                                             C.c_void_p(labels.data_ptr()) if n else None, n, masks.shape[-1] if n else 28, padding, C.c_float(thresh), H, W,
+                                                             C.c_void_p(out.data_ptr()), self._live_ptr(n_live)))
         return out
 
     def mask_propagate(self, mask, flow, depth=None, out=None, stats=None):
```
